# CuzImSlymi/Apertis-LLM

Hardware: NVIDIA B200
Metric: SSM+MoE block fwd+bwd tokens/sec (higher is better)
Workload: dtype bf16

## Files before the change

### apertis_llm_b200/_lib.py

```python
from __future__ import annotations

import ctypes
import os
import subprocess
import threading
from ctypes import c_char_p, c_float, c_int, c_int64, c_size_t, c_uint32, c_void_p

import torch

_HERE = os.path.dirname(os.path.abspath(__file__))
LIB_PATH = os.path.join(_HERE, "libapertis_b200.so")
CSRC = os.path.join(_HERE, "csrc")

AB_F32, AB_BF16 = 0, 1
ACT = {"gelu": 0, "relu": 1, "silu": 2, "swish": 2}
EPI_NONE, EPI_BIAS, EPI_BIAS_ACT, EPI_DACT, EPI_ADD = 0, 1, 2, 3, 4
SCAN_SINGLE_PASS, SCAN_TWO_PASS, SCAN_PIPELINED, SCAN_ROUNDS = 0, 1, 2, 3
ROW_ALIGN = 256
ROUTER_EXACT, ROUTER_BF16, ROUTER_FP16 = 0, 1, 2

P, I, I64, SZ, F, U32 = c_void_p, c_int, c_int64, c_size_t, c_float, c_uint32

SIGNATURES = {
    "ab_version": (I, []),
    "ab_device_check": (I, [I]),
    "ab_last_error": (I, [c_char_p, SZ]),
    "ab_causal_conv1d_silu_fwd": (I, [P, I64, P, P, P, I, I, I, I, I, P]),
    "ab_causal_conv1d_silu_bwd_workspace_bytes": (SZ, [I, I, I]),
    "ab_causal_conv1d_silu_bwd": (I, [P, I64, P, P, P, P, I64, P, P, P, SZ, I, I, I, I, I, P]),
    "ab_selective_scan_plan": (I, [I, I, I, I, P, P, P, P, P]),
    "ab_selective_scan_fwd": (I, [P, P, P, P, I64, P, I64, P, P, P, P, P, P, P, P, SZ, U32, I, I, I, I, I, I, P]),
    "ab_selective_scan_bwd": (I, [P, P, P, P, I64, P, I64, P, P, P, P, P, P, P, P, I64, P, P, P, P, P, SZ, U32, I,
                                  I, I, I, I, I, P]),
    "ab_ssm_scan_plan": (I, [I, I, I, I, P, P]),
    "ab_ssm_scan_tune": (I, [I, I, I, I, I]),
    "ab_ssm_scan_fwd": (I, [P, I64, P, I64, P, P, P, I64, P, I64, P, P, P, P, P, P, P, P, SZ, I, I, I, I, I, P]),
    "ab_ssm_scan_bwd": (I, [P, I64, P, P, I64, P, I64, P, P, P, P, P, P, I64, P, P, I64, P, I64, P, I64, I, P, P, P, P, SZ,
                            I, I, I, I, I, P]),
    "ab_gemm_row_tile": (I, []),
    "ab_shifted_ce_fwd": (I, [P, P, P, P, P, P, I, I, I, I64, I, P]),
    "ab_shifted_ce_bwd": (I, [P, P, P, P, P, I, I, I, I64, I, P]),
    "ab_ep_permute_ln": (I, [P, P, P, P, P, P, P, P, I, I, I64, I, I, I64, I, I, P]),
    "ab_ep_unpermute_bwd": (I, [P, P, P, P, P, P, P, I, I, I64, P, F, P, I, I, I64, I, I, I, P]),
    "ab_ep_grouped_gemm_nt": (I, [P, P, P, P, P, I, I, I64, P, P, I64, I, I, I, I, I, I, P]),
    "ab_ep_grouped_gemm_nn": (I, [P, P, P, P, P, I, I, I64, P, P, I64, I, I, I, I, I, I, P]),
    "ab_moe_router_workspace_bytes": (SZ, [I, I, I]),
    "ab_moe_router_fwd": (I, [P, P, P, F, P, P, P, P, P, P, P, P, P, P, P, P, P, P, SZ, I, I, I, I, I, I, P]),
    "ab_moe_topk_from_logits": (I, [P, P, P, P, P, P, I, I, I, P]),
    "ab_moe_max_rows": (I64, [I, I, I, I, I]),
    "ab_moe_plan_workspace_bytes": (SZ, [I, I, I]),
    "ab_moe_plan": (I, [P, P, P, I, P, P, P, P, P, P, P, P, SZ, I, I, I, I, I64, I, P]),
    "ab_moe_permute_ln": (I, [P, P, P, P, P, P, P, P, I, I, I64, I, I, P]),
    "ab_moe_unpermute": (I, [P, P, P, P, P, F, P, I, I, I, I, I, P]),
    "ab_moe_unpermute_bwd": (I, [P, P, P, P, P, P, P, P, F, P, I, I, I64, I, I, I, P]),
    "ab_moe_permute_ln_bwd_workspace_bytes": (SZ, [I, I, I64]),
    "ab_moe_permute_ln_bwd": (I, [P, P, P, P, P, P, P, P, P, P, P, SZ, I, I, I, I64, I, I, P]),
    "ab_moe_segment_colsum_workspace_bytes": (SZ, [I, I, I64]),
    "ab_moe_segment_colsum": (I, [P, P, P, P, P, SZ, I, I, I, I64, I, P]),
    "ab_moe_router_bwd_workspace_bytes": (SZ, [I, I, I]),
    "ab_moe_router_bwd": (I, [P] * 24 + [SZ, I, I, I, I, I, P]),
    "ab_grouped_gemm_nt": (I, [P, P, P, P, P, P, P, P, I64, I, I, I, I, I, I, F, P, P]),
    "ab_grouped_gemm_nn": (I, [P, P, P, P, P, P, P, P, I64, I, I, I, I, I, I, F, P, P]),
    "ab_grouped_gemm_tn_workspace_bytes": (SZ, [I, I, I, I]),
    "ab_grouped_gemm_tn": (I, [P, P, P, P, I64, I, I, I, I, I64, P, SZ, P]),
    "ab_dense_gemm_nt": (I, [P, P, P, P, P, I64, I, I, I, I, P]),
    "ab_dense_gemm_nn": (I, [P, P, P, P, P, I64, I, I, I, I, P]),
    "ab_dense_gemm_tn_workspace_bytes": (SZ, [I64, I, I]),
    "ab_dense_gemm_tn": (I, [P, P, P, P, SZ, I64, I, I, P]),
    "ab_dt_compose_fwd": (I, [P, P, P, I, I, I, I, I, P]),
    "ab_dt_compose_bwd": (I, [P, P, P, P, P, I, I, I, I, P]),
    "ab_layernorm_fwd": (I, [P, P, P, F, P, P, I, I, I, I, P]),
    "ab_layernorm_bwd_workspace_bytes": (SZ, [I, I]),
    "ab_layernorm_bwd": (I, [P, P, P, P, P, P, P, P, P, SZ, I, I, I, I, P]),
    "ab_dropout_add": (I, [P, P, P, F, P, I64, I, I, P]),
    "ab_cast_f32_to_bf16": (I, [P, P, I64, P]),
    "ab_split_f32_to_bf16x3": (I, [P, P, I64, I64, I, P]),
    "ab_split_f32_to_bf16x3_rows": (I, [P, P, P, I, I64, I64, I, P]),
}

_lib = None
_lock = threading.Lock()
_checked_devices = set()


def build(verbose: bool = False) -> str:
    cmd = ["make", "-C", CSRC, "-j", "8"]
    res = subprocess.run(cmd, capture_output=True, text=True)
    if res.returncode != 0:
        raise RuntimeError("building libapertis_b200.so failed:\n" + res.stdout[-4000:] + res.stderr[-4000:])
    if verbose:
        print(res.stdout[-2000:])
    return LIB_PATH


def load() -> ctypes.CDLL:
    global _lib
    with _lock:
        if _lib is not None:
            return _lib
        if not os.path.exists(LIB_PATH):
            build()
        lib = ctypes.CDLL(LIB_PATH)
        for name, (res, args) in SIGNATURES.items():
            fn = getattr(lib, name)
            fn.restype = res
            fn.argtypes = args
        _lib = lib
        return lib


def last_error() -> str:
    buf = ctypes.create_string_buffer(600)
    load().ab_last_error(buf, 600)
    return buf.value.decode("utf-8", "replace")


def ptr(t):
    if t is None:
        return None
    return t.data_ptr()


def dt(t_or_dtype) -> int:
    d = t_or_dtype.dtype if torch.is_tensor(t_or_dtype) else t_or_dtype
    if d == torch.float32:
        return AB_F32
    if d == torch.bfloat16:
        return AB_BF16
    raise TypeError(f"apertis_b200 kernels take float32 or bfloat16 activations, got {d}")


def stream_ptr(device=None) -> int:
    return torch.cuda.current_stream(device).cuda_stream


def ensure_device(device) -> None:
    if device.type != "cuda":
        raise RuntimeError("apertis_llm_b200: the hot path only runs on a CUDA sm_100a (B200) device; got "
                           f"device '{device}'. There is no CPU fallback.")
    idx = device.index if device.index is not None else torch.cuda.current_device()
    if idx in _checked_devices:
        return
    rc = load().ab_device_check(idx)
    if rc != 0:
        raise RuntimeError("apertis_llm_b200: " + last_error())
    _checked_devices.add(idx)


KERNELS_PER_CALL = {
    "ab_causal_conv1d_silu_fwd": 1, "ab_causal_conv1d_silu_bwd": 2,
    "ab_selective_scan_fwd": 1, "ab_selective_scan_bwd": 2,
    "ab_ssm_scan_fwd": 1, "ab_ssm_scan_bwd": 2, "ab_dense_gemm_nt": 1, "ab_dense_gemm_nn": 1, "ab_dense_gemm_tn": 2,
    "ab_dt_compose_fwd": 1, "ab_dt_compose_bwd": 2,
    "ab_moe_router_fwd": 2, "ab_moe_topk_from_logits": 1, "ab_moe_plan": 7, "ab_moe_permute_ln": 1, "ab_moe_unpermute": 1,
    "ab_moe_unpermute_bwd": 1, "ab_moe_permute_ln_bwd": 2, "ab_moe_segment_colsum": 2, "ab_moe_router_bwd": 3,
    "ab_layernorm_fwd": 1, "ab_layernorm_bwd": 3,
    "ab_grouped_gemm_nt": 1, "ab_grouped_gemm_nn": 1, "ab_grouped_gemm_tn": 1, "ab_cast_f32_to_bf16": 1,
    "ab_shifted_ce_fwd": 2, "ab_shifted_ce_bwd": 1, "ab_ep_permute_ln": 1, "ab_ep_unpermute_bwd": 1, "ab_ep_grouped_gemm_nt": 1, "ab_ep_grouped_gemm_nn": 1,
    "ab_split_f32_to_bf16x3": 1, "ab_split_f32_to_bf16x3_rows": 1,
}
launch_count = 0
_timed = None


def start_timing(names):
    global _timed
    _timed = {"names": set(names), "events": []}


def stop_timing():
    global _timed
    t, _timed = _timed, None
    out = {}
    if t is None:
        return out
    torch.cuda.synchronize()
    for name, a, b in t["events"]:
        out.setdefault(name, []).append(a.elapsed_time(b))
    return out


def call(name: str, *args):
    global launch_count
    fn = getattr(load(), name)
    if _timed is not None and name in _timed["names"]:
        a, b = torch.cuda.Event(enable_timing=True), torch.cuda.Event(enable_timing=True)
        a.record()
        rc = fn(*args)
        b.record()
        _timed["events"].append((name, a, b))
    else:
        rc = fn(*args)
    if rc != 0:
        raise RuntimeError(f"{name} failed (code {rc}): {last_error()}")
    launch_count += KERNELS_PER_CALL.get(name, 1)


def query(name: str, *args):
    return getattr(load(), name)(*args)
```

### apertis_llm_b200/csrc/grouped_gemm.cu

```cuda
#include "common.cuh"

namespace {

constexpr int BM = 128;
constexpr int PM = 2 * BM;
constexpr int BK = 64, NSTAGE = 5, NACC = 2;
constexpr int A_BYTES = BM * BK * 2;
constexpr int BH_BYTES_MAX = 128 * BK * 2;
constexpr int STAGE_BYTES = A_BYTES + BH_BYTES_MAX;
constexpr int ATOM_BYTES = 64 * BK * 2;
constexpr int EPI_WARP0 = 2, EPI_WARPS = 16, EPI_THREADS = EPI_WARPS * 32;
constexpr int NUM_THREADS = 64 + EPI_THREADS;
constexpr int GW = 64;
constexpr int MODE_NT = 0, MODE_NN = 1, MODE_TN = 2;
constexpr int WARP_STG_BYTES = 32 * 64;
constexpr int WARP_BIAS_BYTES = GW * 4;
constexpr size_t SMEM_BYTES = 1024 + (size_t)NSTAGE * STAGE_BYTES + (size_t)EPI_WARPS * (WARP_STG_BYTES + WARP_BIAS_BYTES) + 256;
static_assert(SMEM_BYTES <= 232448, "shared memory budget");
static_assert(PM == AB_GEMM_ROW_TILE, "row tile of the ABI");

struct GemmParams {
    int N, K, E, M;
    int bn;
    int num_n_tiles, num_m_tiles;
    int epi, act, c_f32;
    int tn_nsrc;
    int tn_e_real;
    int64_t tn_src_stride;
    int64_t rows_valid;
    int dense_m_tiles;
    int64_t tn_rows;
    int64_t tn_split;
    const int32_t* tile_expert;
    const int32_t* n_rows;
    const int32_t* seg_off;
    const float* bias;
    const void* aux;
    const uint32_t* drop_seed;
    uint32_t drop_thresh;
    float drop_scale;
    void* c;
    void* c2;
    float* cw;
    unsigned char* peer_base[16];
    int peer_n, peer_rows, peer_rank;
};

__device__ __forceinline__ int dense_tn_blocks(const GemmParams& p, int e) {
    const int64_t lo = (int64_t)e * p.tn_split;
    const int64_t hi = lo + p.tn_split < p.tn_rows ? lo + p.tn_split : p.tn_rows;
    return hi > lo ? (int)((hi - lo + BK - 1) / BK) : 0;
}

__device__ __forceinline__ float erf_core(float ax_s, float g) {
    const float t = ab_rcp(fmaf(0.3275911f, ax_s, 1.0f));
    float p = fmaf(1.061405429f, t, -1.453152027f);
    p = fmaf(p, t, 1.421413741f);
    p = fmaf(p, t, -0.284496736f);
    p = fmaf(p, t, 0.254829592f);
    return 1.0f - p * t * g;
}
__device__ __forceinline__ float gelu_fwd(float x) {
    const float a = fabsf(x) * 0.70710678118654752f;
    const float g = ab_ex2(x * (x * (-0.5f * AB_LOG2E)));
    const float t = ab_rcp(fmaf(0.3275911f, a, 1.0f));
    float q = fmaf(0.750526976f, t, -1.027533652f);
    q = fmaf(q, t, 1.005091295f);
    q = fmaf(q, t, -0.201169571f);
    q = fmaf(q, t, 0.180191733f);
    return fmaxf(x, 0.f) - (a * t) * (q * g);
}
__device__ __forceinline__ float act_fwd(float x, int act) {
    if (act == AB_ACT_GELU) return gelu_fwd(x);
    if (act == AB_ACT_RELU) return fmaxf(x, 0.f);
    return x * ab_sigmoid(x);
}
__device__ __forceinline__ float act_bwd(float x, int act) {
    if (act == AB_ACT_GELU) {
        const float a = fabsf(x) * 0.70710678118654752f;
        const float g = ab_ex2(-a * a * AB_LOG2E);
        const float cdf = 0.5f * (1.0f + copysignf(erf_core(a, g), x));
        return fmaf(x, 0.3989422804014327f * g, cdf);
    }
    if (act == AB_ACT_RELU) return x > 0.f ? 1.f : 0.f;
    const float s = ab_sigmoid(x);
    return s * fmaf(x, 1.f - s, 1.f);
}

__device__ __forceinline__ f2 gelu_fwd2(f2 x) {
    float x0, x1;
    f2_unpack(x, x0, x1);
    const f2 a = f2_pack(fabsf(x0) * 0.70710678118654752f, fabsf(x1) * 0.70710678118654752f);
    const f2 g = f2_ex2(f2_mul(x, f2_mul(x, f2_bcast(-0.5f * AB_LOG2E))));
    const f2 t = f2_rcp(f2_fma(f2_bcast(0.3275911f), a, f2_bcast(1.0f)));
    f2 q = f2_fma(f2_bcast(0.750526976f), t, f2_bcast(-1.027533652f));
    q = f2_fma(q, t, f2_bcast(1.005091295f));
    q = f2_fma(q, t, f2_bcast(-0.201169571f));
    q = f2_fma(q, t, f2_bcast(0.180191733f));
    const f2 h = f2_mul(f2_mul(a, t), f2_mul(q, g));
    return f2_fma(h, f2_bcast(-1.0f), f2_pack(fmaxf(x0, 0.f), fmaxf(x1, 0.f)));
}
__device__ __forceinline__ f2 gelu_bwd2(f2 x) {
    float x0, x1;
    f2_unpack(x, x0, x1);
    const f2 a = f2_pack(fabsf(x0) * 0.70710678118654752f, fabsf(x1) * 0.70710678118654752f);
    const f2 g = f2_ex2(f2_mul(f2_mul(a, a), f2_bcast(-AB_LOG2E)));
    const f2 t = f2_rcp(f2_fma(f2_bcast(0.3275911f), a, f2_bcast(1.0f)));
    f2 pl = f2_fma(f2_bcast(1.061405429f), t, f2_bcast(-1.453152027f));
    pl = f2_fma(pl, t, f2_bcast(1.421413741f));
    pl = f2_fma(pl, t, f2_bcast(-0.284496736f));
    pl = f2_fma(pl, t, f2_bcast(0.254829592f));
    const f2 erfv = f2_fma(f2_mul(pl, t), f2_mul(g, f2_bcast(-1.0f)), f2_bcast(1.0f));
    float e0, e1;
    f2_unpack(erfv, e0, e1);
    const f2 cdf = f2_fma(f2_pack(copysignf(e0, x0), copysignf(e1, x1)), f2_bcast(0.5f), f2_bcast(0.5f));
    return f2_fma(x, f2_mul(g, f2_bcast(0.3989422804014327f)), cdf);
}

#define AB_GF_C0 0.79746994f
#define AB_GF_C1 0.037015004f
#define AB_GF_C2 -3.5035629e-4f
__device__ __forceinline__ float ab_tanh(float x) { float y; asm("tanh.approx.f32 %0, %1;" : "=f"(y) : "f"(x)); return y; }
__device__ __forceinline__ f2 f2_tanh(f2 v) { float a, b; f2_unpack(v, a, b); return f2_pack(ab_tanh(a), ab_tanh(b)); }
__device__ __forceinline__ f2 gelu_fast_x2(f2 x) {
    float a, b;
    f2_unpack(f2_mul(x, x), a, b);
    return f2_pack(fminf(a, 81.f), fminf(b, 81.f));
}
__device__ __forceinline__ f2 gelu_fwd_fast2(f2 x, f2 hs) {
    const f2 x2 = gelu_fast_x2(x);
    f2 p = f2_fma(f2_bcast(AB_GF_C2), x2, f2_bcast(AB_GF_C1));
    p = f2_fma(p, x2, f2_bcast(AB_GF_C0));
    const f2 t = f2_tanh(f2_mul(p, x));
    const f2 hx = f2_mul(x, hs);
    return f2_fma(hx, t, hx);
}
__device__ __forceinline__ f2 gelu_bwd_fast2(f2 x, f2 hs) {
    const f2 x2 = gelu_fast_x2(x);
    f2 p = f2_fma(f2_bcast(AB_GF_C2), x2, f2_bcast(AB_GF_C1));
    p = f2_fma(p, x2, f2_bcast(AB_GF_C0));
    const f2 t = f2_tanh(f2_mul(p, x));
    f2 up = f2_fma(f2_bcast(5.f * AB_GF_C2), x2, f2_bcast(3.f * AB_GF_C1));
    up = f2_fma(up, x2, f2_bcast(AB_GF_C0));
    const f2 w = f2_mul(x, up);
    const f2 e = f2_fma(f2_mul(t, f2_bcast(-1.0f)), w, w);
    const f2 A = f2_fma(t, hs, hs);
    return f2_fma(A, e, A);
}

template <int U, bool F32>
__device__ __forceinline__ void act_fwd_row(float (&f)[U], int act, float scale) {
    if (act == AB_ACT_GELU && !F32) {
        const f2 hs = f2_bcast(0.5f * scale);
#pragma unroll
        for (int i = 0; i < U; i += 2) f2_unpack(gelu_fwd_fast2(f2_pack(f[i], f[i + 1]), hs), f[i], f[i + 1]);
    } else if (act == AB_ACT_GELU) {
        const f2 sc = f2_bcast(scale);
#pragma unroll
        for (int i = 0; i < U; i += 2) f2_unpack(f2_mul(gelu_fwd2(f2_pack(f[i], f[i + 1])), sc), f[i], f[i + 1]);
    } else if (act == AB_ACT_RELU) {
#pragma unroll
        for (int i = 0; i < U; ++i) f[i] = fmaxf(f[i], 0.f) * scale;
    } else {
#pragma unroll
        for (int i = 0; i < U; ++i) f[i] = act_fwd(f[i], AB_ACT_SILU) * scale;
    }
}
template <int U>
__device__ __forceinline__ void round_row_bf16(float (&f)[U]) {
#pragma unroll
    for (int i = 0; i < U; i += 2) {
        uint32_t r;
        asm("cvt.rn.bf16x2.f32 %0, %1, %2;" : "=r"(r) : "f"(f[i + 1]), "f"(f[i]));
        f[i] = __uint_as_float(r << 16);
        f[i + 1] = __uint_as_float(r & 0xffff0000u);
    }
}

__device__ __forceinline__ void drop_keep4(uint32_t xb, uint32_t grp, uint32_t s1, uint32_t thi, bool (&keep)[4]) {
    uint32_t x = xb + grp * 0x9E3779B1u;
    x ^= x >> 16; x *= 0x85EBCA6Bu;
    x = x ^ (x >> 13) ^ s1; x *= 0xC2B2AE35u;
    uint32_t y = x * 0x27D4EB2Fu + s1;
    y ^= y >> 15;
    keep[0] = (x << 16) >= thi;
    keep[1] = x >= thi;
    keep[2] = (y << 16) >= thi;
    keep[3] = y >= thi;
}
template <int U>
__device__ __forceinline__ void dropout_zero_row(float (&f)[U], uint32_t drop_thresh, uint32_t s0, uint32_t s1, uint32_t grow, int ncol, int n_cols) {
    const uint32_t xb = ((grow * (uint32_t)n_cols + (uint32_t)ncol) >> 2) * 0x9E3779B1u + s0;
    const uint32_t thi = drop_thresh << 16;
#pragma unroll
    for (int i = 0; i < U; i += 4) {
        bool keep[4];
        drop_keep4(xb, (uint32_t)(i >> 2), s1, thi, keep);
#pragma unroll
        for (int j = 0; j < 4; ++j) f[i + j] = keep[j] ? f[i + j] : 0.f;
    }
}

__device__ __forceinline__ uint64_t make_smem_desc(uint32_t smem_addr, uint32_t lbo_bytes, uint32_t sbo_bytes) {
    uint64_t d = 0;
    d |= (uint64_t)((smem_addr >> 4) & 0x3FFF);
    d |= (uint64_t)((lbo_bytes >> 4) & 0x3FFF) << 16;
    d |= (uint64_t)((sbo_bytes >> 4) & 0x3FFF) << 32;
    d |= (uint64_t)1 << 46;
    d |= (uint64_t)2 << 61;
    return d;
}
__host__ __device__ inline uint32_t make_idesc(int n, int a_mn_major, int b_mn_major) {
    uint32_t d = 0;
    d |= 1u << 4;
    d |= 1u << 7;
    d |= 1u << 10;
    d |= (uint32_t)a_mn_major << 15;
    d |= (uint32_t)b_mn_major << 16;
    d |= (uint32_t)(n >> 3) << 17;
    d |= (uint32_t)(PM >> 4) << 24;
    return d;
}

struct Tile { int m_pair, n_tile, e, k_begin, nk; };

template <int MODE>
__device__ __forceinline__ int total_tiles_of(const GemmParams& p) {
    if (MODE == MODE_TN) return p.E * p.num_m_tiles * p.num_n_tiles;
    return (p.n_rows != nullptr ? p.n_rows[0] / PM : p.dense_m_tiles) * p.num_n_tiles;
}
template <int MODE>
__device__ __forceinline__ Tile decode_tile(const GemmParams& p, int tile) {
    Tile t;
    if (MODE == MODE_TN) {
        const int per_e = p.num_m_tiles * p.num_n_tiles;
        t.e = tile / per_e;
        const int rem = tile % per_e;
        t.m_pair = rem / p.num_n_tiles; t.n_tile = rem % p.num_n_tiles;
        if (p.seg_off != nullptr) {
            const int e = p.tn_e_real > 0 ? t.e % p.tn_e_real : t.e, slice = p.tn_e_real > 0 ? t.e / p.tn_e_real : 0;
            const int s0 = p.seg_off[e];
            t.k_begin = s0 + (int)((int64_t)slice * p.tn_nsrc * p.tn_src_stride);
            t.nk = p.tn_nsrc * ((p.seg_off[e + 1] - s0) / BK);
        } else {
            t.k_begin = (int)(t.e * p.tn_split);
            t.nk = dense_tn_blocks(p, t.e);
        }
    } else {
        t.m_pair = tile / p.num_n_tiles; t.n_tile = tile % p.num_n_tiles;
        t.e = p.tile_expert != nullptr ? p.tile_expert[t.m_pair] : 0;
        t.k_begin = 0;
        t.nk = (p.K + BK - 1) / BK;
    }
    return t;
}

__device__ __forceinline__ uint32_t stg_off(int r, int j) { return (uint32_t)(r * 64 + ((j ^ ((r >> 1) & 3)) << 4)); }

template <int MODE, bool F32>
__device__ __forceinline__ void stage_and_store(const GemmParams& p, unsigned char* stg, const float (&src)[F32 ? 16 : 32],
                                                unsigned char* base, int lane, size_t row0, int ncol, int ncol_end) {
    constexpr int ES = F32 ? 4 : 2;
    constexpr int CPV = 16 / ES;
    const int N = p.N;
#pragma unroll
    for (int j = 0; j < 4; ++j) {
        uint4 q;
        if (F32) q = make_uint4(__float_as_uint(src[j * 4]), __float_as_uint(src[j * 4 + 1]), __float_as_uint(src[j * 4 + 2]), __float_as_uint(src[j * 4 + 3]));
        else q = ab_vec16<__nv_bfloat16>::pack(&src[j * 8]);
        *reinterpret_cast<uint4*>(stg + stg_off(lane, j)) = q;
    }
    __syncwarp();
#pragma unroll
    for (int it = 0; it < 4; ++it) {
        const int r = it * 8 + (lane >> 2), j = lane & 3;
        const int col = ncol + j * CPV;
        const size_t grow = row0 + r;
        const bool ok = col < ncol_end && (MODE == MODE_TN ? (int)grow < p.M : (int64_t)grow < p.rows_valid);
        const uint4 q = *reinterpret_cast<const uint4*>(stg + stg_off(r, j));
        if (ok) *reinterpret_cast<uint4*>(base + (grow * N + col) * ES) = q;
    }
    __syncwarp();
}

template <bool F32>
__device__ __forceinline__ void load_aux_unit(const GemmParams& p, uint4 (&q)[4], int lane, size_t row0, int ncol, int ncol_end) {
    constexpr int ES = F32 ? 4 : 2;
    constexpr int CPV = 16 / ES;
#pragma unroll
    for (int it = 0; it < 4; ++it) {
        const int r = it * 8 + (lane >> 2), j = lane & 3;
        const int col = ncol + j * CPV;
        const size_t grow = row0 + r;
        q[it] = make_uint4(0u, 0u, 0u, 0u);
        if (col < ncol_end && (int64_t)grow < p.rows_valid)
            q[it] = __ldg(reinterpret_cast<const uint4*>(reinterpret_cast<const unsigned char*>(p.aux) + (grow * p.N + col) * ES));
    }
}

struct EpiCtx {
    unsigned char* stg;
    float* bias_s;
    uint64_t* tfull;
    uint64_t* tempty;
    uint32_t tmem_base;
    int warp, lane;
    uint32_t rank;
    int pair_id, num_pairs;
};

template <int MODE, bool F32, int EPI>
__device__ __forceinline__ void epilogue_role(const GemmParams& p, const EpiCtx& c) {
    constexpr int U = F32 ? 16 : 32;
    constexpr int ES = F32 ? 4 : 2;
    constexpr int CPV = 16 / ES;
    constexpr bool HAS_BIAS = EPI == AB_EPI_BIAS || EPI == AB_EPI_BIAS_ACT;
    constexpr bool HAS_AUX = EPI == AB_EPI_DACT || EPI == AB_EPI_ADD;
    const int lane = c.lane;
    const int quarter = c.warp & 3;
    const int sub = (c.warp - EPI_WARP0) >> 2;
    const int N = p.N, bn = p.bn;
    const int g_col0 = sub * GW;
    const int g_cols = g_col0 < bn ? min(GW, bn - g_col0) : 0;
    const int total_tiles = total_tiles_of<MODE>(p);
    unsigned char* stg = c.stg;
    const bool has_drop = (EPI == AB_EPI_BIAS_ACT || EPI == AB_EPI_DACT) && p.drop_seed != nullptr;
    const uint32_t drop_s0 = has_drop ? __ldg(p.drop_seed) : 0u, drop_s1 = has_drop ? __ldg(p.drop_seed + 1) : 0u;
    const float dscale = has_drop ? p.drop_scale : 1.0f;
    int acc = 0; uint32_t acc_phase = 0;
    for (int tile = c.pair_id; tile < total_tiles; tile += c.num_pairs) {
        const Tile t = decode_tile<MODE>(p, tile);
        const int m_tile = 2 * t.m_pair + (int)c.rank;
        const bool have_acc = t.nk > 0;
        const int n0 = t.n_tile * bn;
        const int ncol_end = min(N, n0 + g_col0 + g_cols);
        const size_t row0 = (size_t)m_tile * BM + quarter * 32;
        if (HAS_BIAS && g_cols > 0) {
            const int col = n0 + g_col0 + 2 * lane;
            float2 b2 = make_float2(0.f, 0.f);
            if (col < ncol_end) b2 = __ldg(reinterpret_cast<const float2*>(p.bias + (size_t)t.e * N + col));
            *reinterpret_cast<float2*>(c.bias_s + 2 * lane) = b2;
            __syncwarp();
        }
        uint4 nxt[4];
        if (HAS_AUX && g_cols > 0 && n0 + g_col0 < ncol_end) {
            load_aux_unit<F32>(p, nxt, lane, row0, n0 + g_col0, ncol_end);
        }
        if (have_acc) {
            ab_mbar_wait(&c.tfull[acc], acc_phase);
            ab_tc_fence_after();
        }
        const uint32_t t_row = c.tmem_base + (uint32_t)acc * 256u + ((uint32_t)(quarter * 32) << 16);
        for (int u0 = 0; u0 < g_cols; u0 += U) {
            const int tcol = g_col0 + u0;
            const int ncol = n0 + tcol;
            if (ncol >= ncol_end) break;
            uint4 cur[4];
            if (HAS_AUX) {
#pragma unroll
                for (int it = 0; it < 4; ++it) cur[it] = nxt[it];
                if (u0 + U < g_cols && ncol + U < ncol_end) {
                    load_aux_unit<F32>(p, nxt, lane, row0, ncol + U, ncol_end);
                }
            }
            float f[U];
            {
                uint32_t v[U];
                if (have_acc) {
                    if (U == 32) ab_tmem_ld32(t_row + (uint32_t)tcol, v);
                    else ab_tmem_ld16(t_row + (uint32_t)tcol, v);
                    ab_tmem_ld_wait();
                } else {
#pragma unroll
                    for (int i = 0; i < U; ++i) v[i] = 0u;
                }
#pragma unroll
                for (int i = 0; i < U; ++i) f[i] = __uint_as_float(v[i]);
            }
            if (HAS_BIAS) {
#pragma unroll
                for (int i = 0; i < U; i += 4) {
                    const float4 b4 = *reinterpret_cast<const float4*>(c.bias_s + u0 + i);
                    f[i] += b4.x; f[i + 1] += b4.y; f[i + 2] += b4.z; f[i + 3] += b4.w;
                }
            }
            if (EPI == AB_EPI_BIAS_ACT) {
                if (!F32) round_row_bf16<U>(f);
                stage_and_store<MODE, F32>(p, stg, f, reinterpret_cast<unsigned char*>(p.c2), lane, row0, ncol, ncol_end);
                act_fwd_row<U, F32>(f, p.act, p.drop_seed ? p.drop_scale : 1.0f);
                if (p.drop_seed) dropout_zero_row<U>(f, p.drop_thresh, drop_s0, drop_s1, (uint32_t)row0 + (uint32_t)lane, ncol, N);
            } else if (HAS_AUX) {
#pragma unroll
                for (int it = 0; it < 4; ++it) *reinterpret_cast<uint4*>(stg + stg_off(it * 8 + (lane >> 2), lane & 3)) = cur[it];
                __syncwarp();
#pragma unroll
                for (int j = 0; j < 4; ++j) cur[j] = *reinterpret_cast<const uint4*>(stg + stg_off(lane, j));
                __syncwarp();
#pragma unroll
                for (int j = 0; j < 4; ++j) {
                    const uint4 q = cur[j];
                    float a[CPV];
                    if (F32) { a[0] = __uint_as_float(q.x); a[1] = __uint_as_float(q.y); a[2] = __uint_as_float(q.z); a[3] = __uint_as_float(q.w); }
                    else ab_vec16<__nv_bfloat16>::unpack(q, a);
                    if (EPI == AB_EPI_ADD) {
#pragma unroll
                        for (int i = 0; i < CPV; ++i) f[j * CPV + i] += a[i];
                    } else if (p.act == AB_ACT_GELU) {
#pragma unroll
                        for (int i = 0; i < CPV; i += 2) {
                            const f2 gp = F32 ? f2_mul(gelu_bwd2(f2_pack(a[i], a[i + 1])), f2_bcast(dscale))
                                              : gelu_bwd_fast2(f2_pack(a[i], a[i + 1]), f2_bcast(0.5f * dscale));
                            f2_unpack(f2_mul(f2_pack(f[j * CPV + i], f[j * CPV + i + 1]), gp), f[j * CPV + i], f[j * CPV + i + 1]);
                        }
                    } else {
#pragma unroll
                        for (int i = 0; i < CPV; ++i) f[j * CPV + i] *= act_bwd(a[i], p.act) * dscale;
                    }
                }
                if (EPI == AB_EPI_DACT && p.drop_seed) dropout_zero_row<U>(f, p.drop_thresh, drop_s0, drop_s1, (uint32_t)row0 + (uint32_t)lane, ncol, N);
            }
            unsigned char* base;
            if (MODE == MODE_TN) base = reinterpret_cast<unsigned char*>(p.cw) + ((size_t)t.e * p.M) * N * 4;
            else if (p.peer_n > 0) {
                const int dst = (int)(row0 / (size_t)p.peer_rows);
                base = p.peer_base[dst] + ((int64_t)(p.peer_rank - dst) * p.peer_rows) * (int64_t)N * ES;
            } else base = reinterpret_cast<unsigned char*>(p.c);
            stage_and_store<MODE, F32>(p, stg, f, base, lane, row0, ncol, ncol_end);
        }
        if (have_acc) {
            ab_tc_fence_before();
            __syncwarp();
            if (lane == 0) ab_mbar_arrive_cluster(&c.tempty[acc], 0);
            if (++acc == NACC) { acc = 0; acc_phase ^= 1; }
        }
    }
}

template <int MODE, bool F32>
__device__ __forceinline__ void epilogue_dispatch(const GemmParams& p, const EpiCtx& c) {
    if (MODE == MODE_TN) { epilogue_role<MODE, F32, AB_EPI_NONE>(p, c); return; }
    switch (p.epi) {
        case AB_EPI_BIAS: epilogue_role<MODE, F32, AB_EPI_BIAS>(p, c); break;
        case AB_EPI_BIAS_ACT: epilogue_role<MODE, F32, AB_EPI_BIAS_ACT>(p, c); break;
        case AB_EPI_DACT: epilogue_role<MODE, F32, AB_EPI_DACT>(p, c); break;
        case AB_EPI_ADD: epilogue_role<MODE, F32, AB_EPI_ADD>(p, c); break;
        default: epilogue_role<MODE, F32, AB_EPI_NONE>(p, c); break;
    }
}

template <int MODE>
__global__ void __launch_bounds__(NUM_THREADS, 1) grouped_gemm_kernel(const __grid_constant__ CUtensorMap tm_a,
                                                                      const __grid_constant__ CUtensorMap tm_b,
                                                                      const GemmParams p) {
    extern __shared__ unsigned char smem_raw[];
    const uint32_t raw = ab_smem_u32(smem_raw);
    unsigned char* smem = smem_raw + ((1024u - (raw & 1023u)) & 1023u);
    unsigned char* stg_base = smem + (size_t)NSTAGE * STAGE_BYTES;
    float* bias_base = reinterpret_cast<float*>(stg_base + (size_t)EPI_WARPS * WARP_STG_BYTES);
    uint64_t* bars = reinterpret_cast<uint64_t*>(reinterpret_cast<unsigned char*>(bias_base) + (size_t)EPI_WARPS * WARP_BIAS_BYTES);
    uint64_t* full = bars;
    uint64_t* empty = bars + NSTAGE;
    uint64_t* tfull = bars + 2 * NSTAGE;
    uint64_t* tempty = bars + 2 * NSTAGE + NACC;
    uint32_t* tmem_slot = reinterpret_cast<uint32_t*>(bars + 2 * NSTAGE + 2 * NACC);

    const int warp = threadIdx.x >> 5, lane = threadIdx.x & 31;
    const uint32_t rank = ab_cluster_ctarank();
    const int pair_id = blockIdx.x >> 1, num_pairs = gridDim.x >> 1;
    if (warp == 0 && lane == 0) {
        ab_prefetch_tmap(&tm_a);
        ab_prefetch_tmap(&tm_b);
        for (int i = 0; i < NSTAGE; ++i) { ab_mbar_init(&full[i], 1); ab_mbar_init(&empty[i], 1); }
        for (int i = 0; i < NACC; ++i) { ab_mbar_init(&tfull[i], 1); ab_mbar_init(&tempty[i], 2 * EPI_WARPS); }
        ab_fence_mbar_init();
    }
    if (warp == 1) {
        ab_tmem_alloc_pair(tmem_slot, 512);
        ab_tmem_relinquish_pair();
    }
    ab_tc_fence_before();
    ab_cluster_sync();
    ab_tc_fence_after();
    const uint32_t tmem_base = *tmem_slot;

    const int total_tiles = total_tiles_of<MODE>(p);
    const int bn = p.bn, bh = bn >> 1;
    const uint32_t bh_bytes = MODE == MODE_NT ? (uint32_t)bh * BK * 2 : (uint32_t)(bh / 64) * ATOM_BYTES;
    const uint32_t pair_tx = 2u * (A_BYTES + bh_bytes);

    if (warp == 0) {
        int stage = 0; uint32_t phase = 0;
        for (int tile = pair_id; tile < total_tiles; tile += num_pairs) {
            const Tile t = decode_tile<MODE>(p, tile);
            const int b_col0 = t.n_tile * bn + (int)rank * bh;
            const int n_src = MODE == MODE_TN ? p.tn_nsrc : 1;
            const int per_src = t.nk / n_src;
            const int m0 = MODE == MODE_TN ? t.m_pair * PM + (int)rank * BM : (2 * t.m_pair + (int)rank) * BM;
            const int b_row0 = MODE == MODE_NN ? t.e * p.K : (MODE == MODE_NT ? t.e * p.N + b_col0 : 0);
            for (int src = 0; src < n_src; ++src) {
                int r0 = MODE == MODE_TN ? (int)(src * p.tn_src_stride) + t.k_begin : 0;
                for (int kk = 0; kk < per_src; ++kk, r0 += BK) {
                    ab_mbar_wait(&empty[stage], phase ^ 1);
                    unsigned char* sa = smem + (size_t)stage * STAGE_BYTES;
                    unsigned char* sb = sa + A_BYTES;
                    if (ab_elect_one()) {
                        if (rank == 0) ab_mbar_expect_tx(&full[stage], pair_tx);
                        if (MODE == MODE_TN) {
                            ab_tma_load_2d_pair(sa, &tm_a, &full[stage], m0, r0);
                            ab_tma_load_2d_pair(sa + ATOM_BYTES, &tm_a, &full[stage], m0 + 64, r0);
                            ab_tma_load_2d_pair(sb, &tm_b, &full[stage], b_col0, r0);
                            if (bh > 64) ab_tma_load_2d_pair(sb + ATOM_BYTES, &tm_b, &full[stage], b_col0 + 64, r0);
                        } else {
                            ab_tma_load_2d_pair(sa, &tm_a, &full[stage], r0, m0);
                            if (MODE == MODE_NT) {
                                ab_tma_load_2d_pair(sb, &tm_b, &full[stage], r0, b_row0);
                            } else {
                                ab_tma_load_2d_pair(sb, &tm_b, &full[stage], b_col0, b_row0 + r0);
                                if (bh > 64) ab_tma_load_2d_pair(sb + ATOM_BYTES, &tm_b, &full[stage], b_col0 + 64, b_row0 + r0);
                            }
                        }
                    }
                    __syncwarp();
                    if (++stage == NSTAGE) { stage = 0; phase ^= 1; }
                }
            }
        }
        for (int i = 0; i < NSTAGE; ++i) {
            ab_mbar_wait(&empty[stage], phase ^ 1);
            if (++stage == NSTAGE) { stage = 0; phase ^= 1; }
        }
    } else if (warp == 1) {
        if (rank == 0) {
            const uint32_t idesc = make_idesc(bn, MODE == MODE_TN ? 1 : 0, MODE == MODE_NT ? 0 : 1);
            const uint32_t smem0 = ab_smem_u32(smem);
            const uint64_t da0 = MODE == MODE_TN ? make_smem_desc(smem0, ATOM_BYTES, 1024) : make_smem_desc(smem0, 0, 1024);
            const uint64_t db0 = MODE == MODE_NT ? make_smem_desc(smem0 + A_BYTES, 0, 1024) : make_smem_desc(smem0 + A_BYTES, ATOM_BYTES, 1024);
            constexpr uint32_t a_step = MODE == MODE_TN ? (16 * 128) >> 4 : 32 >> 4;
            constexpr uint32_t b_step = MODE == MODE_NT ? 32 >> 4 : (16 * 128) >> 4;
            int stage = 0; uint32_t phase = 0;
            int acc = 0; uint32_t acc_phase = 0;
            for (int tile = pair_id; tile < total_tiles; tile += num_pairs) {
                const Tile t = decode_tile<MODE>(p, tile);
                if (t.nk == 0) continue;
                ab_mbar_wait(&tempty[acc], acc_phase ^ 1);
                ab_tc_fence_after();
                const uint32_t d_tmem = tmem_base + (uint32_t)acc * 256u;
                for (int kb = 0; kb < t.nk; ++kb) {
                    ab_mbar_wait(&full[stage], phase);
                    ab_tc_fence_after();
                    const uint64_t soff = (uint64_t)((uint32_t)stage * (STAGE_BYTES >> 4));
                    const uint64_t da = da0 + soff, db = db0 + soff;
                    if (ab_elect_one()) {
#pragma unroll
                        for (int k = 0; k < BK / 16; ++k)
                            ab_umma_f16_pair(d_tmem, da + (uint64_t)(k * a_step), db + (uint64_t)(k * b_step), idesc, (kb > 0 || k > 0) ? 1u : 0u);
                        ab_umma_commit_pair(&empty[stage], 3);
                        if (kb == t.nk - 1) ab_umma_commit_pair(&tfull[acc], 3);
                    }
                    __syncwarp();
                    if (++stage == NSTAGE) { stage = 0; phase ^= 1; }
                }
                if (++acc == NACC) { acc = 0; acc_phase ^= 1; }
            }
        }
    } else {
        EpiCtx c;
        c.stg = stg_base + (size_t)(warp - EPI_WARP0) * WARP_STG_BYTES;
        c.bias_s = bias_base + (size_t)(warp - EPI_WARP0) * GW;
        c.tfull = tfull; c.tempty = tempty; c.tmem_base = tmem_base;
        c.warp = warp; c.lane = lane; c.rank = rank; c.pair_id = pair_id; c.num_pairs = num_pairs;
        if (p.c_f32) epilogue_dispatch<MODE, true>(p, c);
        else epilogue_dispatch<MODE, false>(p, c);
    }
    ab_tc_fence_before();
    ab_cluster_sync();
    if (warp == 1) ab_tmem_dealloc_pair(tmem_base, 512);
}

int pick_bn(int N, bool mn_major_b) {
    const int step = mn_major_b ? 128 : 16;
    int best = step, best_cost = 1 << 30;
    for (int bn = step; bn <= 256; bn += step) {
        const int cost = (int)ab_ceil_div(N, bn) * (bn + 48);
        if (cost <= best_cost) { best_cost = cost; best = bn; }
    }
    return best;
}

int make_map2(CUtensorMap* m, const void* base, uint64_t inner, uint64_t outer, uint32_t box_inner, uint32_t box_outer) {
    AB_REQUIRE(((uintptr_t)base % 16) == 0 && (inner * 2) % 16 == 0,
               "grouped_gemm: operand base must be 16-byte aligned and the contiguous dimension (%llu) a multiple of 8",
               (unsigned long long)inner);
    uint64_t dims[2] = {inner, outer};
    uint64_t strides[1] = {inner * 2};
    uint32_t box[2] = {box_inner, box_outer};
    return ab_encode_tmap(m, CU_TENSOR_MAP_DATA_TYPE_BFLOAT16, 2, base, dims, strides, box, CU_TENSOR_MAP_SWIZZLE_128B);
}

template <int MODE>
int resident_pairs(int* out) {
    static int cached[64] = {0};
    int dev = 0;
    AB_CHECK_CUDA(cudaGetDevice(&dev));
    if (dev >= 0 && dev < 64 && cached[dev] > 0) { *out = cached[dev]; return AB_OK; }
    auto k = grouped_gemm_kernel<MODE>;
    AB_CHECK_CUDA(cudaFuncSetAttribute(k, cudaFuncAttributeMaxDynamicSharedMemorySize, (int)SMEM_BYTES));
    cudaLaunchConfig_t cfg;
    memset(&cfg, 0, sizeof(cfg));
    cfg.gridDim = dim3(2 * (unsigned)(ab_num_sms() / 2), 1, 1);
    cfg.blockDim = dim3(NUM_THREADS, 1, 1);
    cfg.dynamicSmemBytes = SMEM_BYTES;
    cudaLaunchAttribute attr[1];
    attr[0].id = cudaLaunchAttributeClusterDimension;
    attr[0].val.clusterDim.x = 2; attr[0].val.clusterDim.y = 1; attr[0].val.clusterDim.z = 1;
    cfg.attrs = attr; cfg.numAttrs = 1;
    int n = 0;
    AB_CHECK_CUDA(cudaOccupancyMaxActiveClusters(&n, k, &cfg));
    if (n < 1) n = 1;
    if (n > ab_num_sms() / 2) n = ab_num_sms() / 2;
    if (dev >= 0 && dev < 64) cached[dev] = n;
    *out = n;
    return AB_OK;
}

template <int MODE>
int launch(const CUtensorMap& ta, const CUtensorMap& tb, const GemmParams& p, int64_t max_tiles, cudaStream_t stream) {
    int pairs = 0;
    if (int e = resident_pairs<MODE>(&pairs)) return e;
    if (max_tiles < pairs) pairs = (int)max_tiles;
    if (pairs < 1) pairs = 1;
    cudaLaunchConfig_t cfg;
    memset(&cfg, 0, sizeof(cfg));
    cfg.gridDim = dim3(2 * (unsigned)pairs, 1, 1);
    cfg.blockDim = dim3(NUM_THREADS, 1, 1);
    cfg.dynamicSmemBytes = SMEM_BYTES;
    cfg.stream = stream;
    cudaLaunchAttribute attr[1];
    attr[0].id = cudaLaunchAttributeClusterDimension;
    attr[0].val.clusterDim.x = 2; attr[0].val.clusterDim.y = 1; attr[0].val.clusterDim.z = 1;
    cfg.attrs = attr; cfg.numAttrs = 1;
    AB_CHECK_CUDA(cudaLaunchKernelEx(&cfg, grouped_gemm_kernel<MODE>, ta, tb, p));
    return AB_OK;
}

int gemm_rows(int mode, const void* A, const void* W, const float* bias, const void* aux, void* c, void* c2,
              const int32_t* tile_expert, const int32_t* n_rows, int64_t max_rows, int N, int K, int E, int epi, int act,
              int c_dtype, float drop_p, const uint32_t* drop_seed, cudaStream_t stream, const uint64_t* peer_c = nullptr,
              int peer_w = 0, int peer_rank = 0, int64_t peer_rows = 0) {
    AB_REQUIRE(drop_p >= 0.f && drop_p < 1.f, "grouped_gemm: dropout probability must be in [0, 1)");
    AB_REQUIRE(drop_p == 0.f || (drop_seed != nullptr && (epi == AB_EPI_BIAS_ACT || epi == AB_EPI_DACT)),
               "grouped_gemm: dropout needs a seed and the bias+act / dact epilogue");
    AB_REQUIRE(max_rows > 0 && max_rows % PM == 0, "grouped_gemm: max_rows must be a positive multiple of %d", PM);
    AB_REQUIRE(N > 0 && K > 0 && E > 0 && N % 8 == 0 && K % 8 == 0, "grouped_gemm: N (%d) and K (%d) must be multiples of 8", N, K);
    AB_REQUIRE(c_dtype == AB_F32 || c_dtype == AB_BF16, "grouped_gemm: bad output dtype");
    AB_REQUIRE(epi >= AB_EPI_NONE && epi <= AB_EPI_ADD, "grouped_gemm: bad epilogue %d", epi);
    AB_REQUIRE((epi != AB_EPI_BIAS && epi != AB_EPI_BIAS_ACT) || bias, "grouped_gemm: bias epilogue without bias");
    AB_REQUIRE(epi != AB_EPI_BIAS_ACT || c2, "grouped_gemm: bias+act epilogue needs the pre-activation output c2");
    AB_REQUIRE((epi != AB_EPI_DACT && epi != AB_EPI_ADD) || aux, "grouped_gemm: dact / add epilogue needs aux");
    AB_REQUIRE(bias == nullptr || ((uintptr_t)bias % 8) == 0, "grouped_gemm: bias must be 8-byte aligned");
    GemmParams p;
    memset(&p, 0, sizeof(p));
    p.N = N; p.K = K; p.E = E;
    p.bn = pick_bn(N, mode == MODE_NN);
    p.num_n_tiles = (int)ab_ceil_div(N, p.bn);
    p.epi = epi; p.act = act; p.c_f32 = c_dtype == AB_F32;
    p.tile_expert = tile_expert; p.n_rows = n_rows; p.bias = bias; p.aux = aux; p.c = c; p.c2 = c2;
    p.rows_valid = max_rows;
    if (peer_c != nullptr) {
        AB_REQUIRE(peer_w >= 1 && peer_w <= 16 && peer_rank >= 0 && peer_rank < peer_w && peer_rows > 0 && peer_rows % PM == 0 &&
                   (int64_t)peer_w * peer_rows == max_rows && epi != AB_EPI_BIAS_ACT,
                   "ep_grouped_gemm: bad peer table (W=%d rank=%d rows_per_peer=%lld, max_rows=%lld)", peer_w, peer_rank,
                   (long long)peer_rows, (long long)max_rows);
        for (int i = 0; i < peer_w; ++i) {
            AB_REQUIRE(peer_c[i] != 0 && peer_c[i] % 16 == 0, "ep_grouped_gemm: peer buffer %d is null or misaligned", i);
            p.peer_base[i] = reinterpret_cast<unsigned char*>(peer_c[i]);
        }
        p.peer_n = peer_w; p.peer_rows = (int)peer_rows; p.peer_rank = peer_rank;
        c = reinterpret_cast<void*>(peer_c[peer_rank]);
        p.c = c;
    }
    if (drop_p > 0.f) {
        p.drop_seed = drop_seed;
        p.drop_thresh = (uint32_t)((double)drop_p * 65536.0 + 0.5);
        p.drop_scale = 1.0f / (1.0f - drop_p);
    }
    AB_REQUIRE(((uintptr_t)c % 16) == 0 && (c2 == nullptr || ((uintptr_t)c2 % 16) == 0) && (aux == nullptr || ((uintptr_t)aux % 16) == 0),
               "grouped_gemm: output / aux pointers must be 16-byte aligned");
    CUtensorMap ta, tb;
    if (int e = make_map2(&ta, A, (uint64_t)K, (uint64_t)max_rows, BK, BM)) return e;
    const int64_t max_tiles = (max_rows / PM) * p.num_n_tiles;
    if (mode == MODE_NT) {
        if (int e = make_map2(&tb, W, (uint64_t)K, (uint64_t)E * N, BK, (uint32_t)(p.bn / 2))) return e;
        return launch<MODE_NT>(ta, tb, p, max_tiles, stream);
    }
    if (int e = make_map2(&tb, W, (uint64_t)N, (uint64_t)E * K, 64, BK)) return e;
    return launch<MODE_NN>(ta, tb, p, max_tiles, stream);
}

}

extern "C" int ab_gemm_row_tile(void) { return PM; }



extern "C" int ab_grouped_gemm_nt(const void* A, const void* W, const float* bias, const void* aux, void* c, void* c2,
                                  const int32_t* tile_expert, const int32_t* n_rows, int64_t max_rows, int N, int K, int E,
                                  int epi, int act, int c_dtype, float drop_p, const uint32_t* drop_seed, cudaStream_t stream) {
    return gemm_rows(MODE_NT, A, W, bias, aux, c, c2, tile_expert, n_rows, max_rows, N, K, E, epi, act, c_dtype, drop_p, drop_seed, stream);
}

extern "C" int ab_grouped_gemm_nn(const void* A, const void* W, const float* bias, const void* aux, void* c, void* c2,
                                  const int32_t* tile_expert, const int32_t* n_rows, int64_t max_rows, int N, int K, int E,
                                  int epi, int act, int c_dtype, float drop_p, const uint32_t* drop_seed, cudaStream_t stream) {
    return gemm_rows(MODE_NN, A, W, bias, aux, c, c2, tile_expert, n_rows, max_rows, N, K, E, epi, act, c_dtype, drop_p, drop_seed, stream);
}

extern "C" int ab_ep_grouped_gemm_nt(const void* A, const void* W, const float* bias, const void* aux, const uint64_t* peer_c, int peer_w,
                                     int rank, int64_t rows_per_peer, const int32_t* tile_expert, const int32_t* n_rows,
                                     int64_t max_rows, int N, int K, int E, int epi, int act, int c_dtype, cudaStream_t stream) {
    AB_REQUIRE(peer_c != nullptr, "ep_grouped_gemm_nt: no peer table");
    return gemm_rows(MODE_NT, A, W, bias, aux, nullptr, nullptr, tile_expert, n_rows, max_rows, N, K, E, epi, act, c_dtype, 0.f, nullptr,
                     stream, peer_c, peer_w, rank, rows_per_peer);
}

extern "C" int ab_ep_grouped_gemm_nn(const void* A, const void* W, const float* bias, const void* aux, const uint64_t* peer_c, int peer_w,
                                     int rank, int64_t rows_per_peer, const int32_t* tile_expert, const int32_t* n_rows,
                                     int64_t max_rows, int N, int K, int E, int epi, int act, int c_dtype, cudaStream_t stream) {
    AB_REQUIRE(peer_c != nullptr, "ep_grouped_gemm_nn: no peer table");
    return gemm_rows(MODE_NN, A, W, bias, aux, nullptr, nullptr, tile_expert, n_rows, max_rows, N, K, E, epi, act, c_dtype, 0.f, nullptr,
                     stream, peer_c, peer_w, rank, rows_per_peer);
}

namespace {
__global__ void splitk_reduce_kernel(const float* __restrict__ part, float* __restrict__ out, int64_t n, int nsplit);
int grouped_tn_slices(int M, int N, int E, int nsrc) {
    const int64_t tiles = (int64_t)E * ab_ceil_div(M, PM) * ab_ceil_div(N, pick_bn(N, true));
    const int pairs = ab_num_sms() / 2;
    int best = 1;
    double best_cost = (double)ab_ceil_div(tiles, pairs);
    for (int s = 2; s <= nsrc && s <= 4; ++s) {
        if (nsrc % s) continue;
        const double cost = (double)ab_ceil_div(tiles * s, pairs) / s;
        if (cost < 0.88 * best_cost) { best = s; best_cost = cost; }
    }
    return best;
}
}

extern "C" size_t ab_grouped_gemm_tn_workspace_bytes(int M, int N, int E, int nsrc) {
    const int slices = nsrc > 1 ? grouped_tn_slices(M, N, E, nsrc) : 1;
    return slices > 1 ? (size_t)slices * E * M * N * sizeof(float) : 0;
}

extern "C" int ab_grouped_gemm_tn(const void* A, const void* Bm, float* Cw, const int32_t* seg_off, int64_t max_rows, int M,
                                  int N, int E, int nsrc, int64_t src_stride, void* ws, size_t ws_bytes, cudaStream_t stream) {
    AB_REQUIRE(nsrc >= 1 && (nsrc == 1 || (src_stride > 0 && src_stride % BK == 0 && nsrc * src_stride <= max_rows)),
               "grouped_gemm_tn: bad source blocking nsrc=%d stride=%lld", nsrc, (long long)src_stride);
    AB_REQUIRE(max_rows > 0 && max_rows % BK == 0, "grouped_gemm_tn: max_rows must be a positive multiple of %d", BK);
    AB_REQUIRE(M > 0 && N > 0 && E > 0 && M % 8 == 0 && N % 8 == 0, "grouped_gemm_tn: M (%d) and N (%d) must be multiples of 8", M, N);
    GemmParams p;
    memset(&p, 0, sizeof(p));
    p.N = N; p.M = M; p.E = E; p.K = 0;
    p.bn = pick_bn(N, true);
    p.num_n_tiles = (int)ab_ceil_div(N, p.bn);
    p.num_m_tiles = (int)ab_ceil_div(M, PM);
    p.seg_off = seg_off; p.c_f32 = 1; p.epi = AB_EPI_NONE; p.cw = Cw;
    p.tn_nsrc = nsrc; p.tn_src_stride = src_stride;
    AB_REQUIRE(((uintptr_t)Cw % 16) == 0 && ((uintptr_t)ws % 16) == 0, "grouped_gemm_tn: output / workspace must be 16-byte aligned");
    int slices = nsrc > 1 ? grouped_tn_slices(M, N, E, nsrc) : 1;
    if (slices > 1 && (ws == nullptr || ws_bytes < (size_t)slices * E * M * N * sizeof(float))) slices = 1;
    if (slices > 1) {
        p.tn_e_real = E; p.E = E * slices; p.tn_nsrc = nsrc / slices;
        p.cw = reinterpret_cast<float*>(ws);
    }
    CUtensorMap ta, tb;
    if (int e = make_map2(&ta, A, (uint64_t)M, (uint64_t)max_rows, 64, BK)) return e;
    if (int e = make_map2(&tb, Bm, (uint64_t)N, (uint64_t)max_rows, 64, BK)) return e;
    if (int e = launch<MODE_TN>(ta, tb, p, (int64_t)p.E * p.num_m_tiles * p.num_n_tiles, stream)) return e;
    if (slices > 1) {
        const int64_t n = (int64_t)E * M * N;
        splitk_reduce_kernel<<<(unsigned)ab_ceil_div(n / 4, 256), 256, 0, stream>>>(reinterpret_cast<const float*>(ws), Cw, n, slices);
        AB_LAUNCH_CHECK();
    }
    return AB_OK;
}

namespace {
int dense_rows(int mode, const void* A, const void* W, const float* bias, const void* aux, void* c, int64_t S, int N, int K, int epi,
               int c_dtype, cudaStream_t stream) {
    AB_REQUIRE(S > 0 && N > 0 && K > 0 && N % 8 == 0 && K % 8 == 0, "dense_gemm: S (%lld) must be positive, N (%d) and K (%d) multiples of 8", (long long)S, N, K);
    AB_REQUIRE(c_dtype == AB_F32 || c_dtype == AB_BF16, "dense_gemm: bad output dtype");
    AB_REQUIRE(epi == AB_EPI_NONE || epi == AB_EPI_BIAS || epi == AB_EPI_ADD, "dense_gemm: epilogue must be none, bias or add");
    AB_REQUIRE(epi != AB_EPI_BIAS || bias, "dense_gemm: bias epilogue without bias");
    AB_REQUIRE(epi != AB_EPI_ADD || aux, "dense_gemm: add epilogue without addend");
    AB_REQUIRE(((uintptr_t)c % 16) == 0 && (aux == nullptr || ((uintptr_t)aux % 16) == 0), "dense_gemm: output / addend must be 16-byte aligned");
    AB_REQUIRE(bias == nullptr || ((uintptr_t)bias % 8) == 0, "dense_gemm: bias must be 8-byte aligned");
    GemmParams p;
    memset(&p, 0, sizeof(p));
    p.N = N; p.K = K; p.E = 1;
    p.bn = pick_bn(N, mode == MODE_NN);
    p.num_n_tiles = (int)ab_ceil_div(N, p.bn);
    p.epi = epi; p.c_f32 = c_dtype == AB_F32;
    p.bias = bias; p.aux = aux; p.c = c;
    p.rows_valid = S;
    p.dense_m_tiles = (int)ab_ceil_div(S, PM);
    CUtensorMap ta, tb;
    if (int e = make_map2(&ta, A, (uint64_t)K, (uint64_t)S, BK, BM)) return e;
    const int64_t tiles = (int64_t)p.dense_m_tiles * p.num_n_tiles;
    if (mode == MODE_NT) {
        if (int e = make_map2(&tb, W, (uint64_t)K, (uint64_t)N, BK, (uint32_t)(p.bn / 2))) return e;
        return launch<MODE_NT>(ta, tb, p, tiles, stream);
    }
    if (int e = make_map2(&tb, W, (uint64_t)N, (uint64_t)K, 64, BK)) return e;
    return launch<MODE_NN>(ta, tb, p, tiles, stream);
}
}

extern "C" int ab_dense_gemm_nt(const void* A, const void* W, const float* bias, const void* aux, void* C, int64_t S, int N, int K,
                                int epi, int c_dtype, cudaStream_t stream) {
    return dense_rows(MODE_NT, A, W, bias, aux, C, S, N, K, epi, c_dtype, stream);
}

extern "C" int ab_dense_gemm_nn(const void* A, const void* W, const float* bias, const void* aux, void* C, int64_t S, int N, int K,
                                int epi, int c_dtype, cudaStream_t stream) {
    return dense_rows(MODE_NN, A, W, bias, aux, C, S, N, K, epi, c_dtype, stream);
}

namespace {
__global__ void splitk_reduce_kernel(const float* __restrict__ part, float* __restrict__ out, int64_t n, int nsplit) {
    const int64_t i = ((int64_t)blockIdx.x * blockDim.x + threadIdx.x) * 4;
    if (i >= n) return;
    float4 acc = *reinterpret_cast<const float4*>(part + i);
    for (int s = 1; s < nsplit; ++s) {
        const float4 v = *reinterpret_cast<const float4*>(part + (size_t)s * n + i);
        acc.x += v.x; acc.y += v.y; acc.z += v.z; acc.w += v.w;
    }
    *reinterpret_cast<float4*>(out + i) = acc;
}

int dense_tn_nsplit(int64_t S, int M, int N) {
    const int tiles = (int)(ab_ceil_div(M, PM) * ab_ceil_div(N, pick_bn(N, true)));
    int nsplit = tiles > 0 ? (ab_num_sms() / 2) / tiles : 1;
    const int64_t kblocks = ab_ceil_div(S, BK);
    if (nsplit > kblocks / 4) nsplit = (int)(kblocks / 4);
    return nsplit < 2 ? 1 : nsplit;
}
}

extern "C" size_t ab_dense_gemm_tn_workspace_bytes(int64_t S, int M, int N) {
    const int nsplit = dense_tn_nsplit(S, M, N);
    return nsplit < 2 ? 0 : (size_t)nsplit * M * N * sizeof(float);
}

extern "C" int ab_dense_gemm_tn(const void* A, const void* Bm, float* Cw, void* ws, size_t ws_bytes, int64_t S, int M, int N,
                                cudaStream_t stream) {
    AB_REQUIRE(S > 0 && M > 0 && N > 0 && M % 8 == 0 && N % 8 == 0, "dense_gemm_tn: S (%lld) must be positive, M (%d) and N (%d) multiples of 8", (long long)S, M, N);
    AB_REQUIRE(((uintptr_t)Cw % 16) == 0 && ((uintptr_t)ws % 16) == 0, "dense_gemm_tn: output / workspace must be 16-byte aligned");
    GemmParams p;
    memset(&p, 0, sizeof(p));
    p.N = N; p.M = M; p.K = 0;
    p.bn = pick_bn(N, true);
    p.num_n_tiles = (int)ab_ceil_div(N, p.bn);
    p.num_m_tiles = (int)ab_ceil_div(M, PM);
    p.c_f32 = 1; p.epi = AB_EPI_NONE;
    p.tn_nsrc = 1; p.tn_rows = S;
    int nsplit = dense_tn_nsplit(S, M, N);
    if (nsplit >= 2 && (ws == nullptr || ws_bytes < (size_t)nsplit * M * N * sizeof(float))) nsplit = 1;
    const int64_t kblocks = ab_ceil_div(S, BK);
    p.E = nsplit;
    p.tn_split = ab_ceil_div(kblocks, nsplit) * BK;
    p.cw = nsplit > 1 ? reinterpret_cast<float*>(ws) : Cw;
    CUtensorMap ta, tb;
    if (int e = make_map2(&ta, A, (uint64_t)M, (uint64_t)S, 64, BK)) return e;
    if (int e = make_map2(&tb, Bm, (uint64_t)N, (uint64_t)S, 64, BK)) return e;
    if (int e = launch<MODE_TN>(ta, tb, p, (int64_t)nsplit * p.num_m_tiles * p.num_n_tiles, stream)) return e;
    if (nsplit > 1) {
        const int64_t n = (int64_t)M * N;
        splitk_reduce_kernel<<<(unsigned)ab_ceil_div(n / 4, 256), 256, 0, stream>>>(reinterpret_cast<const float*>(ws), Cw, n, nsplit);
        AB_LAUNCH_CHECK();
    }
    return AB_OK;
}
```

### apertis_llm_b200/ep.py

```python
from __future__ import annotations

import os
from typing import List

import ctypes

import torch
import torch.distributed as dist

from . import _lib, ops
from ._lib import ROW_ALIGN, call, dt, ptr, query, stream_ptr


def segment_rows(cap: int) -> int:
    return (int(cap) + ROW_ALIGN - 1) // ROW_ALIGN * ROW_ALIGN


def recv_tile_expert(W: int, El: int, seg: int, device=None) -> torch.Tensor:
    tiles_per_seg = seg // ROW_ALIGN
    return torch.arange(El, dtype=torch.int32, device=device).repeat_interleave(tiles_per_seg).repeat(W)


def local_seg_off(El: int, seg: int, device=None) -> torch.Tensor:
    return torch.arange(El + 1, dtype=torch.int32, device=device) * seg


def all_to_all_equal(send: torch.Tensor, group) -> torch.Tensor:
    W = dist.get_world_size(group)
    assert send.shape[0] == W and send.is_contiguous()
    recv = torch.empty_like(send)
    if dist.get_backend(group) == "nccl":
        dist.all_to_all_single(recv.view(-1), send.view(-1), group=group)
        return recv
    rank = dist.get_rank(group)
    recv[rank].copy_(send[rank])
    ops_ = []
    for peer in range(W):
        if peer == rank:
            continue
        ops_.append(dist.P2POp(dist.isend, send[peer], dist.get_global_rank(group, peer), group))
        ops_.append(dist.P2POp(dist.irecv, recv[peer], dist.get_global_rank(group, peer), group))
    for w in dist.batch_isend_irecv(ops_):
        w.wait()
    return recv


def all_to_all_equal_start(send: torch.Tensor, group):
    if dist.get_backend(group) != "nccl":
        return all_to_all_equal(send, group), (lambda: None)
    assert send.shape[0] == dist.get_world_size(group) and send.is_contiguous()
    recv = torch.empty_like(send)
    work = dist.all_to_all_single(recv.view(-1), send.view(-1), group=group, async_op=True)
    return recv, work.wait


def all_gather_cat(t: torch.Tensor, group) -> torch.Tensor:
    W = dist.get_world_size(group)
    out = torch.empty((W,) + tuple(t.shape), dtype=t.dtype, device=t.device)
    dist.all_gather_into_tensor(out.view(-1), t.contiguous().view(-1), group=group) if dist.get_backend(group) == "nccl" else \
        dist.all_gather(list(out.unbind(0)), t.contiguous(), group=group)
    return out.view((-1,) + tuple(t.shape[1:]))


_EP_MODE = os.environ.get("APERTIS_B200_EP", "auto")

_peer_cache = {}
_peer_failed = False
_warned_reuse = False


class _PeerState:

    def __init__(self, group, rows: int, Dm: int, device):
        import torch.distributed._symmetric_memory as symm_mem
        self.W = dist.get_world_size(group)
        self.rank = dist.get_rank(group)
        self.rows, self.Dm = rows, Dm
        names = ("xn", "y", "dy", "dxn")
        self.buf, self.hdl, self.ptrs = {}, {}, {}
        for n in names:
            t = symm_mem.empty(rows, Dm, dtype=torch.bfloat16, device=device)
            h = symm_mem.rendezvous(t, group)
            self.buf[n], self.hdl[n] = t, h
            self.ptrs[n] = (ctypes.c_uint64 * self.W)(*[int(p) for p in h.buffer_ptrs])
        self.sync = self.hdl["xn"]
        self.version = 0
        self.side = torch.cuda.Stream(device=device)

    def barrier(self, channel: int = 0):
        self.sync.barrier(channel=channel)


_uniform_checked = set()
_recv_plans = {}


def _recv_plan(W: int, El: int, seg: int, device):
    key = (W, El, seg, device.index)
    p = _recv_plans.get(key)
    if p is None:
        p = dict(tile_expert=recv_tile_expert(W, El, seg, device),
                 n_rows=torch.full((2,), W * El * seg, dtype=torch.int32, device=device),
                 seg_off=local_seg_off(El, seg, device))
        if not torch.cuda.is_current_stream_capturing():
            _recv_plans[key] = p
    return p


def _check_uniform(group, S: int, cap: int, training: bool, device):
    key = (id(group), S, cap, training)
    if key in _uniform_checked:
        return
    mine = torch.tensor([S, cap, int(training)], dtype=torch.int64, device=device)
    allv = [torch.empty_like(mine) for _ in range(dist.get_world_size(group))]
    dist.all_gather(allv, mine, group=group)
    vals = torch.stack(allv).cpu()
    if not bool((vals == vals[0]).all()):
        raise RuntimeError("apertis_b200 EP: every rank of the expert-parallel group must process the same number of tokens with the "
                           f"same capacity and mode; got (tokens, capacity, training) per rank = {vals.tolist()}")
    _uniform_checked.add(key)


def _peer_state(group, rows: int, Dm: int, device, owner=0):
    global _peer_failed
    if _EP_MODE == "nccl" or _peer_failed or dist.get_backend(group) != "nccl":
        return None
    key = (id(group), dist.get_rank(group), rows, Dm, device.index, owner)
    st = _peer_cache.get(key)
    if st is None:
        if torch.cuda.is_current_stream_capturing():
            return None
        try:
            st = _PeerState(group, rows, Dm, device)
        except Exception as ex:
            if _EP_MODE == "peer":
                raise
            _peer_failed = True
            import warnings
            warnings.warn(f"apertis_b200 EP: peer-memory transport unavailable ({type(ex).__name__}: {ex}); using NCCL all-to-all")
            return None
        _peer_cache[key] = st
    return st


class _MoEExpertsEP(torch.autograd.Function):

    @staticmethod
    @ops._on_tensor_device
    def forward(ctx, x2, rn_w, rn_b, Wr, br, noise, noise_scale, ln_w, ln_b, W1, b1, W2, b2, res, cfg, group):
        _lib.ensure_device(x2.device)
        dev = x2.device
        W = dist.get_world_size(group)
        S, Dm = x2.shape
        El, I, _ = W1.shape
        E = El * W
        K, act, training, precise = cfg["K"], cfg["act"], cfg["training"], cfg["precise"]
        x2 = x2.contiguous()
        f = lambda t: t.float().contiguous()
        rn_w, rn_b, Wr, br, b1, b2, W1, W2 = map(f, (rn_w, rn_b, Wr, br, b1, b2, W1, W2))
        ln_key = (ln_w._version, ln_b._version, ln_w.data_ptr(), ln_b.data_ptr(), E, Dm)
        ln_cache = cfg.get("_ln_cache")
        if ln_cache is not None and ln_cache.get("key") == ln_key:
            ln_w_full, ln_b_full = ln_cache["val"]
        else:
            ln_wb = all_gather_cat(torch.stack([f(ln_w), f(ln_b)]).unsqueeze(0), group)
            ln_w_full = ln_wb[:, 0].reshape(E, Dm).contiguous()
            ln_b_full = ln_wb[:, 1].reshape(E, Dm).contiguous()
            if ln_cache is not None:
                ln_cache["key"], ln_cache["val"] = ln_key, (ln_w_full, ln_b_full)
        use_noise = noise is not None and noise_scale is not None
        r = ops.moe_route(x2, rn_w, rn_b, cfg["eps"], Wr, br, f(noise) if use_noise else None,
                          f(noise_scale) if use_noise else None, K, cfg.get("quant", _lib.ROUTER_EXACT))
        _check_uniform(group, S, cfg["cap"], training, dev)
        if cfg["cap"] >= S:
            cnt = torch.bincount(r["idx"].reshape(-1).long(), minlength=E)[:E]
            if cfg["active"] is not None:
                cnt = cnt * cfg["active"].to(cnt.dtype)
            mx = cnt.max().reshape(1)
            dist.all_reduce(mx, op=dist.ReduceOp.MAX, group=group)
            seg = segment_rows(max(1, int(mx.item())))
        else:
            seg = segment_rows(min(cfg["cap"], S))
        plan = ops.moe_plan(r["idx"], r["w"], E, cfg["cap"], cfg["active"], fixed_seg=seg)
        rows_local = E * seg
        cdt = torch.float32 if precise else torch.bfloat16
        peer = None if precise else _peer_state(group, rows_local, Dm, dev, cfg.get("_owner", 0))
        rank = dist.get_rank(group)
        rplan = _recv_plan(W, El, seg, dev)
        if peer is not None:
            peer.version += 1
            peer.barrier(0)
            call("ab_ep_permute_ln", ptr(x2), ptr(r["stats"]), ptr(ln_w_full), ptr(ln_b_full), ptr(plan["tok_of_row"]),
                 ptr(plan["tile_expert"]), ptr(plan["n_rows"]), peer.ptrs["xn"], W, rank, El * seg, Dm, ROW_ALIGN, rows_local,
                 dt(x2), dt(cdt), stream_ptr())
            w1, w2 = ops._cast_bf16(W1), ops._cast_bf16(W2)
            peer.barrier(1)
            xr = peer.buf["xn"]
        else:
            xn = torch.empty(rows_local, Dm, dtype=cdt, device=dev)
            call("ab_moe_permute_ln", ptr(x2), ptr(r["stats"]), ptr(ln_w_full), ptr(ln_b_full), ptr(plan["tok_of_row"]),
                 ptr(plan["tile_expert"]), ptr(plan["n_rows"]), ptr(xn), Dm, ROW_ALIGN, rows_local, dt(x2), dt(cdt), stream_ptr())
            xr_w, xr_wait = all_to_all_equal_start(xn.view(W, El * seg, Dm), group)
            w1 = ops._split_cols(W1.view(El * I, Dm), 1) if precise else ops._cast_bf16(W1)
            w2 = ops._split_cols(W2.view(El * Dm, I), 1) if precise else ops._cast_bf16(W2)
            xr_wait()
            xr = xr_w.view(rows_local, Dm)
        if precise:
            a1, k1 = ops._split_cols(xr, 0), 3 * Dm
        else:
            a1, k1 = xr, Dm
        drop_p = float(cfg.get("drop_p", 0.0)) if training else 0.0
        drop_seed = torch.randint(0, 2 ** 31 - 1, (2,), device=dev, dtype=torch.int32) if drop_p > 0.0 else None
        h, hpre = ops.grouped_gemm("nt", a1, w1, rplan, I, k1, El, bias=b1, epi=_lib.EPI_BIAS_ACT, act=act, out_dtype=cdt, want_c2=True,
                                   drop_p=drop_p, drop_seed=drop_seed)
        if precise:
            a2, k2 = ops._split_cols(h, 0), 3 * I
        else:
            a2, k2 = h, I
        out_p = float(cfg.get("out_drop_p", 0.0)) if training else 0.0
        out_seed = torch.randint(0, 2 ** 31 - 1, (2,), device=dev, dtype=torch.int32) if out_p > 0.0 else None
        resc = res.reshape(S, Dm).float().contiguous() if res is not None else None
        out = torch.empty(S, Dm, dtype=x2.dtype if res is None else torch.float32, device=dev)
        if peer is not None:
            call("ab_ep_grouped_gemm_nt", ptr(a2), ptr(w2), ptr(b2), None, peer.ptrs["y"], W, rank, El * seg, ptr(rplan["tile_expert"]),
                 ptr(rplan["n_rows"]), rows_local, Dm, k2, El, _lib.EPI_BIAS, act, dt(cdt), stream_ptr())
            peer.barrier(2)
            y = peer.buf["y"]
            call("ab_moe_unpermute", ptr(y), ptr(plan["row_of"]), ptr(r["w"]), ptr(resc), ptr(out), out_p, ptr(out_seed), S, K, Dm, dt(y), dt(out),
                 stream_ptr())
        else:
            yr = ops.grouped_gemm("nt", a2, w2, rplan, Dm, k2, El, bias=b2, epi=_lib.EPI_BIAS, out_dtype=cdt)
            y = all_to_all_equal(yr.view(W, El * seg, Dm), group).view(rows_local, Dm)
            call("ab_moe_unpermute", ptr(y), ptr(plan["row_of"]), ptr(r["w"]), ptr(resc), ptr(out), out_p, ptr(out_seed), S, K, Dm, dt(y), dt(out),
                 stream_ptr())
        aux = r["aux"]
        zero = torch.zeros((), dtype=x2.dtype, device=dev)
        lb = (cfg["lb_coef"] * E / (S * S)) * (aux[:E] * aux[E:2 * E]).sum() if (training and cfg["lb_coef"] > 0) else zero
        rz = (cfg["rz_coef"] / S) * aux[2 * E] if (training and cfg["rz_coef"] > 0) else zero
        ctx.cfg = dict(cfg, S=S, Dm=Dm, E=E, El=El, I=I, W=W, seg=seg, use_noise=use_noise, rows=rows_local, cdt=cdt, drop_p=drop_p,
                       out_p=out_p, has_res=res is not None, res_shape=res.shape if res is not None else None,
                       res_dtype=res.dtype if res is not None else None)
        ctx.drop_seed = drop_seed
        ctx.out_seed = out_seed
        ctx.shadows = None if precise else (w1, w2)
        ctx.group = group
        ctx.peer = peer
        ctx.peer_version = peer.version if peer is not None else 0
        ctx.plan = {k: v for k, v in plan.items() if torch.is_tensor(v)}
        ctx.rplan = rplan
        ctx.save_for_backward(x2, rn_w, rn_b, Wr, br, ln_w_full, W1, W2, noise if use_noise else None, r["stats"], r["gates"],
                              r["idx"], r["probs"], r["lse"], r["lclean"], r["w"], aux, xr, h, hpre, y)
        counts = plan["counts"]
        ctx.mark_non_differentiable(counts)
        cfg["_routing"] = (r["idx"], plan["row_of"])
        return out, lb.to(x2.dtype), rz.to(x2.dtype), counts

    @staticmethod
    @ops._on_tensor_device
    def backward(ctx, dout, dlb, drz, _dcounts):
        (x2, rn_w, rn_b, Wr, br, ln_w_full, W1, W2, noise, stats, gates, idx, probs, lse, lclean, w, aux, xr, h, hpre, y) = ctx.saved_tensors
        cfg, plan, rplan, group = ctx.cfg, ctx.plan, ctx.rplan, ctx.group
        S, Dm, E, El, I, K, W, seg = (cfg[k] for k in ("S", "Dm", "E", "El", "I", "K", "W", "seg"))
        act, precise, rows, cdt = cfg["act"], cfg["precise"], cfg["rows"], cfg["cdt"]
        dev = x2.device
        f32 = dict(dtype=torch.float32, device=dev)
        dout = dout.contiguous()
        peer = ctx.peer
        rank = dist.get_rank(group)
        dw_row = torch.empty(rows, **f32)
        if peer is not None and ctx.peer_version != peer.version:
            msg = ("apertis_b200 EP (peer transport): a later forward of this layer ran before this backward.  Expected under "
                   "activation checkpointing (the recomputation rewrites identical rows); any other schedule that keeps two "
                   "forwards of one layer in flight needs APERTIS_B200_EP=nccl.")
            if os.environ.get("APERTIS_B200_EP_STRICT", "0") == "1":
                raise RuntimeError(msg)
            global _warned_reuse
            if not _warned_reuse:
                _warned_reuse = True
                import warnings
                warnings.warn(msg)
        if peer is not None:
            call("ab_ep_unpermute_bwd", ptr(dout), ptr(y), ptr(w), ptr(plan["tok_of_row"]), ptr(plan["slot_of_row"]), ptr(plan["n_rows"]),
                 peer.ptrs["dy"], W, rank, El * seg, ptr(dw_row), cfg["out_p"], ptr(ctx.out_seed), K, Dm, rows, dt(dout), dt(y), dt(cdt),
                 stream_ptr())
            peer.barrier(3)
            dyr = peer.buf["dy"]
        else:
            dy = torch.empty(rows, Dm, dtype=cdt, device=dev)
            call("ab_moe_unpermute_bwd", ptr(dout), ptr(y), ptr(w), ptr(plan["tok_of_row"]), ptr(plan["slot_of_row"]), ptr(plan["n_rows"]),
                 ptr(dy), ptr(dw_row), cfg["out_p"], ptr(ctx.out_seed), K, Dm, rows, dt(dout), dt(y), dt(cdt), stream_ptr())
            dyr = all_to_all_equal(dy.view(W, El * seg, Dm), group).view(rows, Dm)
        lseg = rplan["seg_off"]
        stride = El * seg
        cmain, cside = torch.cuda.current_stream(dev), ops._side_stream(dev)
        db2 = torch.empty(El, Dm, **f32)
        db1 = torch.empty(El, I, **f32)
        ws_b2 = ops._u8(query("ab_moe_segment_colsum_workspace_bytes", Dm, ROW_ALIGN, rows), dev)
        ws_b1 = ops._u8(query("ab_moe_segment_colsum_workspace_bytes", I, ROW_ALIGN, rows), dev)
        if precise:
            G = W * El
            lseg3 = (lseg * 3).contiguous()
            w2r = ops._split_rows(W2.view(El * Dm, I), 1, None, El, Dm)
            dhpre = ops.grouped_gemm("nn", ops._split_cols(dyr, 0), w2r, rplan, I, 3 * Dm, El, aux=hpre, epi=_lib.EPI_DACT, act=act, out_dtype=cdt,
                                     drop_p=cfg["drop_p"], drop_seed=ctx.drop_seed)
            sr = lambda t, which: ops._split_rows(t, which, None, G, seg)
            w1r = ops._split_rows(W1.view(El * I, Dm), 1, None, El, I)
            dxnr = ops.grouped_gemm("nn", ops._split_cols(dhpre, 0), w1r, rplan, Dm, 3 * I, El, out_dtype=torch.float32)
            dxn_w, dxn_wait = all_to_all_equal_start(dxnr.view(W, El * seg, Dm), group)
            dW2 = ops.grouped_gemm_tn(sr(dyr, 0), sr(h, 1), lseg3, Dm, I, El, nsrc=W, src_stride=3 * stride)
            dW1 = ops.grouped_gemm_tn(sr(dhpre, 0), sr(xr, 1), lseg3, I, Dm, El, nsrc=W, src_stride=3 * stride)
        else:
            w1b, w2b = ctx.shadows
            dhpre = ops.grouped_gemm("nn", dyr, w2b, rplan, I, Dm, El, aux=hpre, epi=_lib.EPI_DACT, act=act, out_dtype=cdt,
                                     drop_p=cfg["drop_p"], drop_seed=ctx.drop_seed)
            if peer is not None:
                call("ab_ep_grouped_gemm_nn", ptr(dhpre), ptr(w1b), None, None, peer.ptrs["dxn"], W, rank, El * seg, ptr(rplan["tile_expert"]),
                     ptr(rplan["n_rows"]), rows, Dm, I, El, _lib.EPI_NONE, act, dt(torch.bfloat16), stream_ptr())
                main = torch.cuda.current_stream(dev)
                peer.side.wait_stream(main)
                with torch.cuda.stream(peer.side):
                    peer.barrier(4)
                dxn_w = peer.buf["dxn"]
                dxn_wait = lambda: main.wait_stream(peer.side)
            else:
                dxnr = ops.grouped_gemm("nn", dhpre, w1b, rplan, Dm, I, El, out_dtype=torch.bfloat16)
                dxn_w, dxn_wait = all_to_all_equal_start(dxnr.view(W, El * seg, Dm), group)
            dW2 = ops.grouped_gemm_tn(dyr, h, lseg, Dm, I, El, nsrc=W, src_stride=stride)
            dW1 = ops.grouped_gemm_tn(dhpre, xr, lseg, I, Dm, El, nsrc=W, src_stride=stride)
        ops._colsum_side(cside, cmain, dyr, rplan, db2, ws_b2, Dm, El, rows, dev)
        ops._colsum_side(cside, cmain, dhpre, rplan, db1, ws_b1, I, El, rows, dev)
        ws = ops._u8(query("ab_moe_permute_ln_bwd_workspace_bytes", Dm, ROW_ALIGN, rows), dev)
        dxn_wait()
        dxn = dxn_w.view(rows, Dm)
        dxrow = torch.empty(rows, Dm, **f32)
        dln_w = torch.empty(E, Dm, **f32)
        dln_b = torch.empty(E, Dm, **f32)
        call("ab_moe_permute_ln_bwd", ptr(dxn), ptr(x2), ptr(stats), ptr(ln_w_full), ptr(plan["tok_of_row"]), ptr(plan["tile_expert"]),
             ptr(plan["n_rows"]), ptr(dxrow), ptr(dln_w), ptr(dln_b), ptr(ws), ws.numel(), Dm, E, ROW_ALIGN, rows, dt(x2), dt(dxn),
             stream_ptr())
        dln = torch.stack([dln_w, dln_b])
        dln_work = dist.all_reduce(dln, group=group, async_op=True)
        inv = 1.0 / W
        training = cfg["training"]
        g_lb = (dlb.float() * (cfg["lb_coef"] * E / S)) if (training and cfg["lb_coef"] > 0) else torch.zeros((), **f32)
        g_rz = (drz.float() * (cfg["rz_coef"] / S)) if (training and cfg["rz_coef"] > 0) else torch.zeros((), **f32)
        scal = torch.stack([g_lb.reshape(()), g_rz.reshape(())]).contiguous()
        fvec = (aux[E:2 * E] / S).contiguous()
        dx = torch.empty_like(x2)
        dWr, dbr = torch.empty(E, Dm, **f32), torch.empty(E, **f32)
        drn_w, drn_b = torch.empty(Dm, **f32), torch.empty(Dm, **f32)
        dns = torch.empty(E, **f32) if cfg["use_noise"] else None
        nws = query("ab_moe_router_bwd_workspace_bytes", S, Dm, E)
        ws2 = ops._u8(nws, dev)
        call("ab_moe_router_bwd", ptr(x2), ptr(stats), ptr(rn_w), ptr(rn_b), ptr(Wr), ptr(br), ptr(gates), ptr(idx), ptr(probs),
             ptr(lse), ptr(lclean), ptr(noise.float().contiguous()) if cfg["use_noise"] else None, ptr(fvec), ptr(scal), ptr(dw_row),
             ptr(dxrow), ptr(plan["row_of"]), ptr(dx), ptr(dWr), ptr(dbr), ptr(drn_w), ptr(drn_b), ptr(dns), ptr(ws2), ws2.numel(),
             S, Dm, E, K, dt(x2), stream_ptr())
        dln_work.wait()
        dln_w_l = dln[0, rank * El:(rank + 1) * El] * inv
        dln_b_l = dln[1, rank * El:(rank + 1) * El] * inv
        dres = dout.reshape(cfg["res_shape"]).to(cfg["res_dtype"]) if cfg["has_res"] else None
        cmain.wait_stream(cside)
        return (dx, drn_w, drn_b, dWr, dbr, None, dns, dln_w_l, dln_b_l, dW1 * inv, db1 * inv, dW2 * inv, db2 * inv, dres, None, None)


def moe_experts_ep(module, x2, noise, noise_scale, cfg, res=None):
    cfg["_owner"] = id(module)
    cfg["_ln_cache"] = module.__dict__.setdefault("_ep_ln_cache", {})
    return _MoEExpertsEP.apply(x2, module.router_norm.weight, module.router_norm.bias, module.router.weight, module.router.bias,
                               noise, noise_scale, module.expert_ln_weight, module.expert_ln_bias, module.expert_w1,
                               module.expert_b1, module.expert_w2, module.expert_b2, res, cfg, module.ep_group)


def replicated_parameters(layer: torch.nn.Module) -> List[torch.nn.Parameter]:
    return [p for n, p in layer.named_parameters() if ".expert_" not in n and not n.startswith("expert_")]
```

### apertis_llm_b200/ops.py

```python
from __future__ import annotations

import ctypes
import math
import os
from typing import Optional

import torch

from . import _lib
from ._lib import AB_BF16, AB_F32, ROW_ALIGN, call, dt, ptr, query, stream_ptr

def _on_tensor_device(fn):
    def wrapper(ctx, *args):
        dev = next((a.device for a in args if torch.is_tensor(a) and a.is_cuda), None)
        if dev is None:
            return fn(ctx, *args)
        with torch.cuda.device(dev):
            return fn(ctx, *args)
    wrapper.__name__, wrapper.__doc__ = fn.__name__, fn.__doc__
    return wrapper


_scan_ws = {}
_SCAN_ENV = os.environ.get("APERTIS_B200_SCAN", "auto")
SCAN_MODE = {"two_pass": _lib.SCAN_TWO_PASS, "single": _lib.SCAN_SINGLE_PASS, "pipelined": _lib.SCAN_PIPELINED,
             "rounds": _lib.SCAN_ROUNDS}.get(_SCAN_ENV)


def default_scan_mode(dtype: torch.dtype, Di: int, L: int = 1 << 20) -> int:
    if SCAN_MODE is not None:
        return SCAN_MODE
    return _lib.SCAN_ROUNDS


def _scan_workspace(device, nbytes: int, mode: int = _lib.SCAN_SINGLE_PASS):
    key = (device.index, torch.cuda.current_stream(device).cuda_stream, mode == _lib.SCAN_PIPELINED)
    ent = _scan_ws.get(key)
    if ent is None or ent[0].numel() < nbytes:
        epoch = ent[1] if ent is not None else 0
        ent = [torch.zeros(max(nbytes, 1 << 20), dtype=torch.uint8, device=device), epoch]
        _scan_ws[key] = ent
    ent[1] += 1
    if ent[1] >= (1 << 30) - 1:
        ent[0].zero_()
        ent[1] = 1
    return ent[0], ent[1]


_SCAN_CHECK = os.environ.get("APERTIS_B200_SCAN_CHECK", "0") == "1"


def _scan_check(ws: torch.Tensor, what: str):
    if _SCAN_CHECK and not torch.cuda.is_current_stream_capturing() and int(ws[64:68].view(torch.int32).item()) != 0:
        ws[64:68].zero_()
        raise RuntimeError(f"{what}: a hand-shake wait of the selective scan timed out (protocol error)")


def scan_plan(B: int, L: int, Di: int, dtype: torch.dtype, mode: int = _lib.SCAN_SINGLE_PASS):
    t, s, n, m = ctypes.c_int(), ctypes.c_int(), ctypes.c_int(), ctypes.c_int(mode)
    ws = ctypes.c_size_t()
    call("ab_selective_scan_plan", B, L, Di, dt(dtype), ctypes.byref(m), ctypes.byref(t), ctypes.byref(s), ctypes.byref(n), ctypes.byref(ws))
    return t.value, s.value, n.value, ws.value, m.value


def _row_stride(t: torch.Tensor) -> int:
    B, L, C = t.shape
    assert t.stride(2) == 1 and (B == 1 or t.stride(0) == L * t.stride(1)), "unsupported layout"
    return t.stride(1)


def _rows(t: torch.Tensor) -> torch.Tensor:
    B, L, C = t.shape
    if t.stride(2) == 1 and (B == 1 or t.stride(0) == L * t.stride(1)) and (L == 1 or t.stride(1) >= C):
        return t
    return t.contiguous()


class _LayerNorm(torch.autograd.Function):
    @staticmethod
    @_on_tensor_device
    def forward(ctx, x, weight, bias, eps, out_dtype):
        _lib.ensure_device(x.device)
        shape = x.shape
        Dm = shape[-1]
        x2 = x.reshape(-1, Dm).contiguous()
        S = x2.shape[0]
        w, b = weight.float().contiguous(), bias.float().contiguous()
        y = torch.empty(S, Dm, dtype=out_dtype, device=x.device)
        stats = torch.empty(S, 2, dtype=torch.float32, device=x.device)
        call("ab_layernorm_fwd", ptr(x2), ptr(w), ptr(b), float(eps), ptr(y), ptr(stats), S, Dm, dt(x2), dt(out_dtype), stream_ptr())
        ctx.save_for_backward(x2, stats, w)
        ctx.shape = shape
        return y.view(shape)

    @staticmethod
    @_on_tensor_device
    def backward(ctx, dy):
        x2, stats, w = ctx.saved_tensors
        S, Dm = x2.shape
        dy2 = dy.reshape(S, Dm).contiguous()
        dx = torch.empty_like(x2)
        dw = torch.empty(Dm, dtype=torch.float32, device=x2.device)
        db = torch.empty(Dm, dtype=torch.float32, device=x2.device)
        nws = query("ab_layernorm_bwd_workspace_bytes", S, Dm)
        ws = torch.empty(max(nws, 16), dtype=torch.uint8, device=x2.device)
        call("ab_layernorm_bwd", ptr(dy2), ptr(x2), ptr(stats), ptr(w), None, ptr(dx), ptr(dw), ptr(db), ptr(ws), ws.numel(), S, Dm,
             dt(x2), dt(dy2), stream_ptr())
        return dx.view(ctx.shape), dw, db, None, None


class _LayerNormSkip(torch.autograd.Function):

    @staticmethod
    @_on_tensor_device
    def forward(ctx, x, weight, bias, eps, out_dtype):
        _lib.ensure_device(x.device)
        shape = x.shape
        Dm = shape[-1]
        x2 = x.reshape(-1, Dm).contiguous()
        S = x2.shape[0]
        w, b = weight.float().contiguous(), bias.float().contiguous()
        y = torch.empty(S, Dm, dtype=out_dtype, device=x.device)
        stats = torch.empty(S, 2, dtype=torch.float32, device=x.device)
        call("ab_layernorm_fwd", ptr(x2), ptr(w), ptr(b), float(eps), ptr(y), ptr(stats), S, Dm, dt(x2), dt(out_dtype), stream_ptr())
        ctx.save_for_backward(x2, stats, w)
        ctx.shape = shape
        return y.view(shape), x.view_as(x)

    @staticmethod
    @_on_tensor_device
    def backward(ctx, dy, dskip):
        x2, stats, w = ctx.saved_tensors
        S, Dm = x2.shape
        if dy is None:
            return dskip, None, None, None, None
        dy2 = dy.reshape(S, Dm).contiguous()
        dres = dskip.reshape(S, Dm).to(x2.dtype).contiguous() if dskip is not None else None
        dx = torch.empty_like(x2)
        dw = torch.empty(Dm, dtype=torch.float32, device=x2.device)
        db = torch.empty(Dm, dtype=torch.float32, device=x2.device)
        nws = query("ab_layernorm_bwd_workspace_bytes", S, Dm)
        ws = torch.empty(max(nws, 16), dtype=torch.uint8, device=x2.device)
        call("ab_layernorm_bwd", ptr(dy2), ptr(x2), ptr(stats), ptr(w), ptr(dres), ptr(dx), ptr(dw), ptr(db), ptr(ws), ws.numel(), S, Dm,
             dt(x2), dt(dy2), stream_ptr())
        return dx.view(ctx.shape), dw, db, None, None


class _DropoutAdd(torch.autograd.Function):
    @staticmethod
    @_on_tensor_device
    def forward(ctx, sub, res, p):
        _lib.ensure_device(sub.device)
        sub = sub.contiguous()
        res = res.contiguous()
        out = torch.empty_like(res)
        seed = torch.randint(0, 2 ** 31 - 1, (2,), device=sub.device, dtype=torch.int32) if p > 0 else None
        call("ab_dropout_add", ptr(sub), ptr(res), ptr(out), float(p), ptr(seed), sub.numel(), dt(sub), dt(out), stream_ptr())
        ctx.p, ctx.seed, ctx.sub_dtype = p, seed, sub.dtype
        return out

    @staticmethod
    @_on_tensor_device
    def backward(ctx, dout):
        if ctx.p == 0:
            return dout.to(ctx.sub_dtype), dout, None
        dout = dout.contiguous()
        dsub = torch.empty(dout.shape, dtype=ctx.sub_dtype, device=dout.device)
        call("ab_dropout_add", ptr(dout), None, ptr(dsub), float(ctx.p), ptr(ctx.seed), dout.numel(), dt(dout), dt(dsub), stream_ptr())
        return dsub, dout, None


def dropout_add(sub, res, p: float, training: bool):
    return _DropoutAdd.apply(sub, res, float(p) if training else 0.0)


def layer_norm(x, weight, bias, eps, out_dtype=None):
    return _LayerNorm.apply(x, weight, bias, eps, out_dtype if out_dtype is not None else x.dtype)


def layer_norm_skip(x, weight, bias, eps, out_dtype=None):
    return _LayerNormSkip.apply(x, weight, bias, eps, out_dtype if out_dtype is not None else x.dtype)


class _CausalConv1dSiLU(torch.autograd.Function):
    @staticmethod
    @_on_tensor_device
    def forward(ctx, xp, weight, bias):
        _lib.ensure_device(xp.device)
        xp = _rows(xp)
        B, L, Di = xp.shape
        Kc = weight.shape[-1]
        w = weight.reshape(Di, Kc).float().contiguous()
        b = bias.float().contiguous()
        xa = torch.empty(B, L, Di, dtype=xp.dtype, device=xp.device)
        call("ab_causal_conv1d_silu_fwd", ptr(xp), _row_stride(xp), ptr(w), ptr(b), ptr(xa), B, L, Di, Kc, dt(xp), stream_ptr())
        ctx.save_for_backward(xp, w, b)
        ctx.wshape = weight.shape
        ctx.wdtype, ctx.bdtype = weight.dtype, bias.dtype
        return xa

    @staticmethod
    @_on_tensor_device
    def backward(ctx, dxa):
        xp, w, b = ctx.saved_tensors
        B, L, Di = xp.shape
        Kc = w.shape[-1]
        dxa = dxa.contiguous()
        dxp = torch.empty(B, L, Di, dtype=xp.dtype, device=xp.device)
        dw = torch.empty(Di, Kc, dtype=torch.float32, device=xp.device)
        db = torch.empty(Di, dtype=torch.float32, device=xp.device)
        nws = query("ab_causal_conv1d_silu_bwd_workspace_bytes", B, L, Di)
        ws = torch.empty(nws, dtype=torch.uint8, device=xp.device)
        call("ab_causal_conv1d_silu_bwd", ptr(xp), _row_stride(xp), ptr(dxa), ptr(w), ptr(b), ptr(dxp), Di, ptr(dw), ptr(db),
             ptr(ws), nws, B, L, Di, Kc, dt(xp), stream_ptr())
        return dxp, dw.reshape(ctx.wshape).to(ctx.wdtype), db.to(ctx.bdtype)


def causal_conv1d_silu(xp: torch.Tensor, weight: torch.Tensor, bias: torch.Tensor) -> torch.Tensor:
    return _CausalConv1dSiLU.apply(xp, weight, bias)


class _SelectiveScan(torch.autograd.Function):
    @staticmethod
    @_on_tensor_device
    def forward(ctx, xa, dlog, BC, z, A_log, D, h0, want_yssm, want_hlast, mode):
        _lib.ensure_device(xa.device)
        xa = xa.contiguous()
        dlog = dlog.contiguous()
        BC, z = BC.contiguous(), _rows(z)
        B, L, Di = xa.shape
        H = dlog.shape[-1]
        assert BC.shape == (B, L, 2 * Di)
        Bm, Cm = BC[..., :Di], BC[..., Di:]
        dev = xa.device
        A = A_log.reshape(-1).float().contiguous()
        Dv = D.float().contiguous()
        if want_yssm and mode == _lib.SCAN_PIPELINED:
            mode = _lib.SCAN_SINGLE_PASS
        T, Cs, nchunks, nws, mode = scan_plan(B, L, Di, xa.dtype, mode)
        if mode != _lib.SCAN_PIPELINED and torch.cuda.is_current_stream_capturing():
            mode = _lib.SCAN_TWO_PASS
        ws, epoch = _scan_workspace(dev, nws, mode)
        y = torch.empty_like(xa)
        y_ssm = torch.empty_like(xa) if want_yssm else None
        h_last = torch.empty(B, Di, dtype=torch.float32, device=dev) if want_hlast else None
        hstart = torch.empty(B, nchunks, Di, dtype=torch.float32, device=dev)
        h0c = h0.reshape(B, Di).float().contiguous() if h0 is not None else None
        call("ab_selective_scan_fwd", ptr(xa), ptr(dlog), ptr(Bm), ptr(Cm), 2 * Di, ptr(z), _row_stride(z), ptr(A),
             ptr(Dv), ptr(h0c), ptr(y), ptr(y_ssm), ptr(h_last), ptr(hstart), ptr(ws), ws.numel(), epoch, mode,
             B, L, Di, H, dt(xa), stream_ptr())
        _scan_check(ws, "ab_selective_scan_fwd")
        ctx.save_for_backward(xa, dlog, BC, z, A, Dv, hstart)
        ctx.mode = mode
        ctx.a_shape, ctx.want_yssm = A_log.shape, want_yssm
        if h_last is not None:
            ctx.mark_non_differentiable(h_last)
        return y, y_ssm, h_last

    @staticmethod
    @_on_tensor_device
    def backward(ctx, dy, dyssm, _dh):
        xa, dlog, BC, z, A, Dv, hstart = ctx.saved_tensors
        B, L, Di = xa.shape
        H = dlog.shape[-1]
        dev = xa.device
        Bm, Cm = BC[..., :Di], BC[..., Di:]
        dy = dy.contiguous()
        dys = dyssm.contiguous() if (dyssm is not None and ctx.want_yssm) else None
        T, Cs, nchunks, nws, _ = scan_plan(B, L, Di, xa.dtype, ctx.mode)
        ws, epoch = _scan_workspace(dev, nws, ctx.mode)
        dxa = torch.empty_like(xa)
        dz = torch.empty_like(xa)
        dbc = torch.empty(B, L, 2 * Di, dtype=xa.dtype, device=dev)
        parts = H if ctx.mode == _lib.SCAN_PIPELINED else Di // 4
        ddl = torch.empty(B, L, parts, dtype=torch.float32, device=dev)
        dA = torch.empty(Di, dtype=torch.float32, device=dev)
        dD = torch.empty(Di, dtype=torch.float32, device=dev)
        dB, dC = dbc[..., :Di], dbc[..., Di:]
        call("ab_selective_scan_bwd", ptr(xa), ptr(dlog), ptr(Bm), ptr(Cm), 2 * Di, ptr(z), _row_stride(z), ptr(dy),
             ptr(dys), ptr(A), ptr(Dv), ptr(hstart), ptr(dxa), ptr(dB), ptr(dC), 2 * Di, ptr(dz), ptr(ddl), ptr(dA), ptr(dD),
             ptr(ws), ws.numel(), epoch, ctx.mode, B, L, Di, H, dt(xa), stream_ptr())
        _scan_check(ws, "ab_selective_scan_bwd")
        ddlog = (ddl if parts == H else ddl.view(B, L, H, parts // H).sum(-1)).to(dlog.dtype)
        return dxa, ddlog, dbc, dz, dA.reshape(ctx.a_shape), dD, None, None, None, None


def selective_scan(xa, dlog, BC, z, A_log, D, h0=None, want_yssm=False, want_hlast=False, mode: Optional[int] = None):
    mode = default_scan_mode(xa.dtype, xa.shape[-1], xa.shape[1]) if mode is None else mode
    if mode == _lib.SCAN_ROUNDS:
        return _SelectiveScanRounds.apply(xa, dlog, None, BC, z, A_log, D, h0, want_yssm, want_hlast, dlog.shape[-1])
    return _SelectiveScan.apply(xa, dlog, BC, z, A_log, D, h0, want_yssm, want_hlast, mode)


_rounds_ws = {}


def _rounds_plan(B, L, Di, dtype):
    n, ws = ctypes.c_int64(), ctypes.c_size_t()
    call("ab_ssm_scan_plan", B, L, Di, dt(dtype), ctypes.byref(n), ctypes.byref(ws))
    return n.value, ws.value


def _rounds_workspace(device, nbytes):
    key = (device.index, torch.cuda.current_stream(device).cuda_stream)
    t = _rounds_ws.get(key)
    if t is None or t.numel() < nbytes:
        t = torch.zeros(max(nbytes, 2 << 20), dtype=torch.uint8, device=device)
        _rounds_ws[key] = t
    return t


def _cols(t, lo, hi):
    return t[..., lo:hi]


class _SelectiveScanRounds(torch.autograd.Function):

    @staticmethod
    def forward(ctx, xa, dlog, dt_bias, prm, z, A_log, D, h0, want_yssm, want_hlast, H):
        _lib.ensure_device(xa.device)
        with torch.cuda.device(xa.device):
            xa, z, prm = _rows(xa), _rows(z), _rows(prm)
            B, L, Di = xa.shape
            dev = xa.device
            fused = dlog is None
            W = prm.shape[-1]
            Hp = W - 2 * Di
            assert Hp >= (H if fused else 0) and (fused or Hp == 0), "bad [dt | B | C] layout"
            dl = prm if fused else dlog.contiguous()
            dl_stride = _row_stride(prm) if fused else H
            Bm, Cm = _cols(prm, Hp, Hp + Di), _cols(prm, Hp + Di, Hp + 2 * Di)
            A = A_log.reshape(-1).float().contiguous()
            Dv = D.float().contiguous()
            bias = dt_bias.float().contiguous() if dt_bias is not None else None
            nstate, nws = _rounds_plan(B, L, Di, xa.dtype)
            ws = _rounds_workspace(dev, nws)
            y = torch.empty(B, L, Di, dtype=xa.dtype, device=dev)
            y_ssm = torch.empty(B, L, Di, dtype=xa.dtype, device=dev) if want_yssm else None
            h_last = torch.empty(B, Di, dtype=torch.float32, device=dev) if want_hlast else None
            state = torch.empty(nstate, dtype=torch.float32, device=dev)
            h0c = h0.reshape(B, Di).float().contiguous() if h0 is not None else None
            call("ab_ssm_scan_fwd", ptr(xa), _row_stride(xa), ptr(dl), dl_stride, ptr(bias), ptr(Bm), ptr(Cm), _row_stride(prm),
                 ptr(z), _row_stride(z), ptr(A), ptr(Dv), ptr(h0c), ptr(y), ptr(y_ssm), ptr(h_last), ptr(state), ptr(ws), ws.numel(),
                 B, L, Di, H, dt(xa), stream_ptr(dev))
            ctx.save_for_backward(xa, prm, z, A, Dv, state)
            ctx.meta = (fused, H, Hp, want_yssm, A_log.shape, dlog.dtype if dlog is not None else None,
                        dt_bias is not None, dt_bias.dtype if dt_bias is not None else None)
            if h_last is not None:
                ctx.mark_non_differentiable(h_last)
            return y, y_ssm, h_last

    @staticmethod
    def backward(ctx, dy, dyssm, _dh):
        xa, prm, z, A, Dv, state = ctx.saved_tensors
        fused, H, Hp, want_yssm, a_shape, dlog_dtype, has_bias, bias_dtype = ctx.meta
        with torch.cuda.device(xa.device):
            B, L, Di = xa.shape
            dev = xa.device
            W = prm.shape[-1]
            Bm, Cm = _cols(prm, Hp, Hp + Di), _cols(prm, Hp + Di, Hp + 2 * Di)
            dy = dy.contiguous()
            dys = dyssm.contiguous() if (dyssm is not None and want_yssm) else None
            nstate, nws = _rounds_plan(B, L, Di, xa.dtype)
            ws = _rounds_workspace(dev, nws)
            dxa = torch.empty(B, L, Di, dtype=xa.dtype, device=dev)
            dz = torch.empty(B, L, Di, dtype=xa.dtype, device=dev)
            dprm = torch.empty(B, L, W, dtype=xa.dtype, device=dev)
            ddl = dprm if fused else torch.empty(B, L, H, dtype=xa.dtype, device=dev)
            dA = torch.empty(Di, dtype=torch.float32, device=dev)
            dD = torch.empty(Di, dtype=torch.float32, device=dev)
            dbias = torch.empty(H, dtype=torch.float32, device=dev) if has_bias else None
            dB, dC = _cols(dprm, Hp, Hp + Di), _cols(dprm, Hp + Di, Hp + 2 * Di)
            call("ab_ssm_scan_bwd", ptr(xa), _row_stride(xa), ptr(Bm), ptr(Cm), _row_stride(prm), ptr(z), _row_stride(z), ptr(dy),
                 ptr(dys), ptr(A), ptr(Dv), ptr(state), ptr(dxa), Di, ptr(dB), ptr(dC), W, ptr(dz), Di, ptr(ddl),
                 W if fused else H, Hp if fused else H, ptr(dbias), ptr(dA), ptr(dD), ptr(ws), ws.numel(), B, L, Di, H, dt(xa),
                 stream_ptr(dev))
            ddlog = None if fused else ddl.to(dlog_dtype)
            return (dxa, ddlog, dbias.to(bias_dtype) if has_bias else None, dprm, dz, dA.reshape(a_shape), dD,
                    None, None, None, None)


def selective_scan_fused(xa, prm, dt_bias, z, A_log, D, H, h0=None, want_yssm=False, want_hlast=False):
    return _SelectiveScanRounds.apply(xa, None, dt_bias, prm, z, A_log, D, h0, want_yssm, want_hlast, H)



def _as_bf16(t):
    if t.dtype == torch.bfloat16:
        return t.contiguous()
    if t.dtype == torch.float32 and t.is_contiguous() and t.numel() % 4 == 0:
        return _cast_bf16(t)
    return t.to(torch.bfloat16).contiguous()


def dense_nt(x2, w, precise, bias=None, out_dtype=None):
    S, K = x2.shape
    N = w.shape[0]
    dev = x2.device
    if precise:
        a, b, kk, od = _split_cols(x2.float().contiguous(), 0), _split_cols(w.float().contiguous(), 1), 3 * K, torch.float32
    else:
        a, b, kk, od = _as_bf16(x2), _as_bf16(w), K, (out_dtype or torch.bfloat16)
    c = torch.empty(S, N, dtype=od, device=dev)
    call("ab_dense_gemm_nt", ptr(a), ptr(b), ptr(bias), None, ptr(c), S, N, kk, _lib.EPI_BIAS if bias is not None else _lib.EPI_NONE,
         dt(od), stream_ptr(dev))
    return c


def dense_nn(dy2, w, precise, add=None, out_dtype=None):
    S, N = dy2.shape
    K = w.shape[1]
    dev = dy2.device
    if precise:
        a, b, nn_, od = _split_cols(dy2.float().contiguous(), 0), _split_rows(w.float().contiguous(), 1, None, 1, N), 3 * N, torch.float32
    else:
        a, b, nn_, od = _as_bf16(dy2), _as_bf16(w), N, (out_dtype or torch.bfloat16)
    if add is not None:
        add = add.to(od).contiguous()
    c = torch.empty(S, K, dtype=od, device=dev)
    call("ab_dense_gemm_nn", ptr(a), ptr(b), None, ptr(add), ptr(c), S, K, nn_, _lib.EPI_ADD if add is not None else _lib.EPI_NONE,
         dt(od), stream_ptr(dev))
    return c


def dense_tn(dy2, x2, precise):
    S, N = dy2.shape
    K = x2.shape[1]
    dev = dy2.device
    if precise:
        a, b, ss = _split_rows(dy2.float().contiguous(), 0, None, 1, S), _split_rows(x2.float().contiguous(), 1, None, 1, S), 3 * S
    else:
        a, b, ss = _as_bf16(dy2), _as_bf16(x2), S
    c = torch.empty(N, K, dtype=torch.float32, device=dev)
    nws = query("ab_dense_gemm_tn_workspace_bytes", ss, N, K)
    ws = torch.empty(nws, dtype=torch.uint8, device=dev) if nws else None
    call("ab_dense_gemm_tn", ptr(a), ptr(b), ptr(c), ptr(ws), nws, ss, N, K, stream_ptr(dev))
    return c


class _Linear(torch.autograd.Function):

    @staticmethod
    def forward(ctx, x, bias, precise, *weights):
        _lib.ensure_device(x.device)
        with torch.cuda.device(x.device):
            K = x.shape[-1]
            x2 = x.reshape(-1, K)
            w = weights[0] if len(weights) == 1 else torch.cat([wi.reshape(-1, K) for wi in weights], 0)
            wb = w.float().contiguous() if precise else _as_bf16(w)
            xb = x2.float().contiguous() if precise else _as_bf16(x2)
            y = dense_nt(xb, wb, precise, bias=bias.float().contiguous() if bias is not None else None)
            ctx.save_for_backward(xb, wb)
            ctx.meta = (precise, x.shape, x.dtype, [wi.shape[0] for wi in weights], [wi.dtype for wi in weights],
                        bias.dtype if bias is not None else None)
            return y.view(*x.shape[:-1], w.shape[0])

    @staticmethod
    def backward(ctx, dy):
        xb, wb = ctx.saved_tensors
        precise, xshape, xdtype, splits, wdtypes, bdtype = ctx.meta
        with torch.cuda.device(dy.device):
            N = wb.shape[0]
            dy2 = dy.reshape(-1, N)
            dyb = dy2.float().contiguous() if precise else _as_bf16(dy2)
            dx = dense_nn(dyb, wb, precise).view(xshape) if ctx.needs_input_grad[0] else None
            dw = dense_tn(dyb, xb, precise)
            db = dy2.float().sum(0).to(bdtype) if bdtype is not None else None
            dws = [g.to(d) for g, d in zip(dw.split(splits, 0), wdtypes)]
            if dx is not None and dx.dtype != xdtype:
                dx = dx.to(xdtype)
            return (dx, db, None, *dws)


def linear(x, weights, bias=None, precise=False):
    if torch.is_tensor(weights):
        weights = [weights]
    return _Linear.apply(x, bias, precise, *weights)


class _SSMCore(torch.autograd.Function):

    @staticmethod
    def forward(ctx, xz, conv_w, conv_b, Wp, Wdt, dt_bias, A_log, D, precise):
        _lib.ensure_device(xz.device)
        with torch.cuda.device(xz.device):
            dev = xz.device
            B, L, Di2 = xz.shape
            Di = Di2 // 2
            H, R = Wdt.shape
            Hp = (H + 7) // 8 * 8
            Kc = conv_w.shape[-1]
            W = Hp + 2 * Di
            cdt = torch.float32 if precise else torch.bfloat16
            xz = xz.to(cdt).contiguous()
            cw, cb = conv_w.reshape(Di, Kc).float().contiguous(), conv_b.float().contiguous()
            xp, z = xz[..., :Di], xz[..., Di:]
            xa = torch.empty(B, L, Di, dtype=cdt, device=dev)
            call("ab_causal_conv1d_silu_fwd", ptr(xp), Di2, ptr(cw), ptr(cb), ptr(xa), B, L, Di, Kc, dt(cdt), stream_ptr(dev))
            Wp32, Wdt32 = Wp.float().contiguous(), Wdt.float().contiguous()
            wcat = torch.empty(W, Di, dtype=cdt, device=dev)
            call("ab_dt_compose_fwd", ptr(Wp32), ptr(Wdt32), ptr(wcat), H, Hp, R, Di, dt(cdt), stream_ptr(dev))
            prm = dense_nt(xa.view(B * L, Di), wcat, precise).view(B, L, W)
            A = A_log.reshape(-1).float().contiguous()
            Dv = D.float().contiguous()
            bias = dt_bias.float().contiguous()
            nstate, nws = _rounds_plan(B, L, Di, cdt)
            ws = _rounds_workspace(dev, nws)
            y = torch.empty(B, L, Di, dtype=cdt, device=dev)
            state = torch.empty(nstate, dtype=torch.float32, device=dev)
            call("ab_ssm_scan_fwd", ptr(xa), Di, ptr(prm), W, ptr(bias), ptr(prm[..., Hp:]), ptr(prm[..., Hp + Di:]), W, ptr(z), Di2,
                 ptr(A), ptr(Dv), None, ptr(y), None, None, ptr(state), ptr(ws), ws.numel(), B, L, Di, H, dt(cdt), stream_ptr(dev))
            ctx.save_for_backward(xz, cw, cb, xa, wcat, prm, A, Dv, state, Wp32, Wdt32)
            ctx.meta = (precise, H, Hp, R, Kc, conv_w.shape, conv_w.dtype, conv_b.dtype, Wp.dtype, Wdt.dtype, dt_bias.dtype, A_log.shape)
            return y

    @staticmethod
    def backward(ctx, dy):
        xz, cw, cb, xa, wcat, prm, A, Dv, state, Wp32, Wdt32 = ctx.saved_tensors
        precise, H, Hp, R, Kc, cw_shape, cw_dtype, cb_dtype, wp_dtype, wdt_dtype, bias_dtype, a_shape = ctx.meta
        with torch.cuda.device(dy.device):
            dev = dy.device
            B, L, Di2 = xz.shape
            Di = Di2 // 2
            W = Hp + 2 * Di
            cdt = xz.dtype
            S = B * L
            dy = dy.to(cdt).contiguous()
            z = xz[..., Di:]
            nstate, nws = _rounds_plan(B, L, Di, cdt)
            ws = _rounds_workspace(dev, nws)
            dxz = torch.empty(B, L, Di2, dtype=cdt, device=dev)
            dxa_s = torch.empty(B, L, Di, dtype=cdt, device=dev)
            dprm = torch.empty(B, L, W, dtype=cdt, device=dev)
            dA = torch.empty(Di, dtype=torch.float32, device=dev)
            dD = torch.empty(Di, dtype=torch.float32, device=dev)
            dbias = torch.empty(H, dtype=torch.float32, device=dev)
            call("ab_ssm_scan_bwd", ptr(xa), Di, ptr(prm[..., Hp:]), ptr(prm[..., Hp + Di:]), W, ptr(z), Di2, ptr(dy), None, ptr(A),
                 ptr(Dv), ptr(state), ptr(dxa_s), Di, ptr(dprm[..., Hp:]), ptr(dprm[..., Hp + Di:]), W, ptr(dxz[..., Di:]), Di2,
                 ptr(dprm), W, Hp, ptr(dbias), ptr(dA), ptr(dD), ptr(ws), ws.numel(), B, L, Di, H, dt(cdt), stream_ptr(dev))
            dprm2, xa2 = dprm.view(S, W), xa.view(S, Di)
            dxa = dense_nn(dprm2, wcat, precise, add=dxa_s.view(S, Di), out_dtype=cdt)
            dwcat = dense_tn(dprm2, xa2, precise)
            dWp = torch.empty(R + 2 * Di, Di, dtype=torch.float32, device=dev)
            dWdt = torch.empty(H, R, dtype=torch.float32, device=dev)
            call("ab_dt_compose_bwd", ptr(dwcat), ptr(Wp32), ptr(Wdt32), ptr(dWp), ptr(dWdt), H, Hp, R, Di, stream_ptr(dev))
            dcw = torch.empty(Di, Kc, dtype=torch.float32, device=dev)
            dcb = torch.empty(Di, dtype=torch.float32, device=dev)
            ncw = query("ab_causal_conv1d_silu_bwd_workspace_bytes", B, L, Di)
            cws = torch.empty(ncw, dtype=torch.uint8, device=dev)
            call("ab_causal_conv1d_silu_bwd", ptr(xz), Di2, ptr(dxa), ptr(cw), ptr(cb), ptr(dxz), Di2, ptr(dcw), ptr(dcb), ptr(cws), ncw,
                 B, L, Di, Kc, dt(cdt), stream_ptr(dev))
            return (dxz, dcw.reshape(cw_shape).to(cw_dtype), dcb.to(cb_dtype), dWp.to(wp_dtype), dWdt.to(wdt_dtype),
                    dbias.to(bias_dtype), dA.reshape(a_shape), dD, None)


class _DtCompose(torch.autograd.Function):

    @staticmethod
    def forward(ctx, Wp, Wdt, precise):
        _lib.ensure_device(Wp.device)
        with torch.cuda.device(Wp.device):
            H, R = Wdt.shape
            Di = Wp.shape[1]
            Hp = (H + 7) // 8 * 8
            cdt = torch.float32 if precise else torch.bfloat16
            Wp32, Wdt32 = Wp.float().contiguous(), Wdt.float().contiguous()
            wcat = torch.empty(Hp + 2 * Di, Di, dtype=cdt, device=Wp.device)
            call("ab_dt_compose_fwd", ptr(Wp32), ptr(Wdt32), ptr(wcat), H, Hp, R, Di, dt(cdt), stream_ptr(Wp.device))
            ctx.save_for_backward(Wp32, Wdt32)
            ctx.meta = (H, Hp, R, Di, Wp.dtype, Wdt.dtype)
            return wcat

    @staticmethod
    def backward(ctx, dwcat):
        Wp32, Wdt32 = ctx.saved_tensors
        H, Hp, R, Di, wp_dtype, wdt_dtype = ctx.meta
        with torch.cuda.device(dwcat.device):
            dw = dwcat.float().contiguous()
            dWp = torch.empty(R + 2 * Di, Di, dtype=torch.float32, device=dw.device)
            dWdt = torch.empty(H, R, dtype=torch.float32, device=dw.device)
            call("ab_dt_compose_bwd", ptr(dw), ptr(Wp32), ptr(Wdt32), ptr(dWp), ptr(dWdt), H, Hp, R, Di, stream_ptr(dw.device))
            return dWp.to(wp_dtype), dWdt.to(wdt_dtype), None


def dt_compose(Wp, Wdt, precise=False):
    return _DtCompose.apply(Wp, Wdt, precise)


def ssm_core(xz, conv_w, conv_b, Wp, Wdt, dt_bias, A_log, D, precise):
    return _SSMCore.apply(xz, conv_w, conv_b, Wp, Wdt, dt_bias, A_log, D, precise)


class _LMHeadCE(torch.autograd.Function):

    @staticmethod
    @_on_tensor_device
    def forward(ctx, hidden, weight, labels, ignore_index, precise):
        _lib.ensure_device(hidden.device)
        dev = hidden.device
        B, L, Dm = hidden.shape
        V = weight.shape[0]
        h2 = hidden.reshape(B * L, Dm)
        hb = h2.float().contiguous() if precise else _as_bf16(h2)
        wb = weight.float().contiguous() if precise else _as_bf16(weight)
        logits = dense_nt(hb, wb, precise)
        labels = labels.to(torch.int64).contiguous()
        n = B * (L - 1)
        f32 = dict(dtype=torch.float32, device=dev)
        lse, row_loss, row_valid, sums = torch.empty(n, **f32), torch.empty(n, **f32), torch.empty(n, **f32), torch.empty(2, **f32)
        call("ab_shifted_ce_fwd", ptr(logits), ptr(labels), ptr(lse), ptr(row_loss), ptr(row_valid), ptr(sums), B, L, V, int(ignore_index),
             dt(logits), stream_ptr(dev))
        loss = sums[0] / sums[1]
        ctx.save_for_backward(hb, wb, logits, labels, lse, sums)
        ctx.meta = (B, L, V, Dm, int(ignore_index), precise, hidden.dtype, weight.dtype)
        return logits.view(B, L, V), loss

    @staticmethod
    @_on_tensor_device
    def backward(ctx, dlogits_ext, dloss):
        hb, wb, logits, labels, lse, sums = ctx.saved_tensors
        B, L, V, Dm, ignore_index, precise, hdtype, wdtype = ctx.meta
        dev = logits.device
        g = dloss.float() if dloss is not None else torch.zeros((), dtype=torch.float32, device=dev)
        scale = (g / sums[1]).reshape(1).contiguous()
        dl = torch.empty_like(logits)
        call("ab_shifted_ce_bwd", ptr(logits), ptr(labels), ptr(lse), ptr(scale), ptr(dl), B, L, V, ignore_index, dt(logits), stream_ptr(dev))
        if dlogits_ext is not None:
            dl += dlogits_ext.reshape(B * L, V).to(dl.dtype)
        dlb = dl if precise else _as_bf16(dl)
        dh = dense_nn(dlb, wb, precise).view(B, L, Dm).to(hdtype)
        dw = dense_tn(dlb, hb, precise).to(wdtype)
        return dh, dw, None, None, None


def lm_head_cross_entropy(hidden, weight, labels, ignore_index: int = -100, precise: bool = False):
    return _LMHeadCE.apply(hidden, weight, labels, ignore_index, precise)


def _u8(n, dev):
    return torch.empty(max(int(n), 16), dtype=torch.uint8, device=dev)


_side_streams = {}


def _side_stream(device) -> torch.cuda.Stream:
    st = _side_streams.get(device.index)
    if st is None:
        st = torch.cuda.Stream(device=device)
        _side_streams[device.index] = st
    return st


def moe_route(x2, ln_w, ln_b, eps, Wr, br, noise, noise_scale, K, quant=_lib.ROUTER_EXACT):
    S, Dm = x2.shape
    E = Wr.shape[0]
    dev = x2.device
    f32 = dict(dtype=torch.float32, device=dev)
    r = dict(lclean=torch.empty(S, E, **f32), logits=torch.empty(S, E, **f32), gates=torch.empty(S, E, **f32),
             idx=torch.empty(S, K, dtype=torch.int32, device=dev), probs=torch.empty(S, K, **f32),
             w=torch.empty(S, K, **f32), lse=torch.empty(S, **f32), stats=torch.empty(S, 2, **f32),
             aux=torch.empty(2 * E + 1, **f32))
    nws = query("ab_moe_router_workspace_bytes", S, Dm, E)
    ws = _u8(nws, dev)
    call("ab_moe_router_fwd", ptr(x2), ptr(ln_w), ptr(ln_b), float(eps), ptr(Wr), ptr(br), ptr(noise), ptr(noise_scale),
         ptr(r["lclean"]), ptr(r["logits"]), ptr(r["gates"]), ptr(r["idx"]), ptr(r["probs"]), ptr(r["w"]), ptr(r["lse"]),
         ptr(r["stats"]), ptr(r["aux"]), ptr(ws), ws.numel(), S, Dm, E, K, dt(x2), quant, stream_ptr())
    return r


def moe_topk_from_logits(logits, K):
    S, E = logits.shape
    dev = logits.device
    f32 = dict(dtype=torch.float32, device=dev)
    gates, probs, w, lse = torch.empty(S, E, **f32), torch.empty(S, K, **f32), torch.empty(S, K, **f32), torch.empty(S, **f32)
    idx = torch.empty(S, K, dtype=torch.int32, device=dev)
    call("ab_moe_topk_from_logits", ptr(logits.contiguous()), ptr(gates), ptr(idx), ptr(probs), ptr(w), ptr(lse), S, E, K, stream_ptr())
    return gates, idx, probs, w, lse


def moe_plan(idx, w, E, cap, active=None, fixed_seg=0):
    S, K = idx.shape
    dev = idx.device
    cap = int(min(cap, S))
    max_rows = E * fixed_seg if fixed_seg > 0 else int(query("ab_moe_max_rows", S, K, E, cap, ROW_ALIGN))
    i32 = dict(dtype=torch.int32, device=dev)
    p = dict(counts=torch.empty(E, **i32), seg_off=torch.empty(E + 1, **i32), row_of=torch.empty(S, K, **i32),
             tok_of_row=torch.empty(max_rows, **i32), slot_of_row=torch.empty(max_rows, **i32),
             tile_expert=torch.empty(max_rows // ROW_ALIGN, **i32), n_rows=torch.empty(2, **i32), max_rows=max_rows, cap=cap)
    nws = query("ab_moe_plan_workspace_bytes", S, K, E)
    ws = _u8(nws, dev)
    call("ab_moe_plan", ptr(idx), ptr(w), ptr(active), cap, ptr(p["counts"]), ptr(p["seg_off"]), ptr(p["row_of"]),
         ptr(p["tok_of_row"]), ptr(p["slot_of_row"]), ptr(p["tile_expert"]), ptr(p["n_rows"]), ptr(ws), ws.numel(),
         S, K, E, ROW_ALIGN, max_rows, fixed_seg, stream_ptr())
    return p


def _cast_bf16(t):
    out = torch.empty(t.shape, dtype=torch.bfloat16, device=t.device)
    call("ab_cast_f32_to_bf16", ptr(t), ptr(out), t.numel(), stream_ptr())
    return out


def _split_cols(t2d, which):
    rows, cols = t2d.shape
    out = torch.empty(rows, 3 * cols, dtype=torch.bfloat16, device=t2d.device)
    call("ab_split_f32_to_bf16x3", ptr(t2d), ptr(out), rows, cols, which, stream_ptr())
    return out


def _split_rows(t2d, which, seg_off=None, G=1, rows_per_group=0):
    rows, cols = t2d.shape
    out = torch.empty(3 * rows, cols, dtype=torch.bfloat16, device=t2d.device)
    call("ab_split_f32_to_bf16x3_rows", ptr(t2d), ptr(out), ptr(seg_off), G, rows_per_group, cols, which, stream_ptr())
    return out


def grouped_gemm(mode, A, W, plan, N, K, E, *, bias=None, aux=None, epi=_lib.EPI_NONE, act=0, out_dtype=torch.bfloat16,
                 want_c2=False, drop_p=0.0, drop_seed=None, out=None):
    max_rows = A.shape[0]
    if out is not None:
        assert out.shape == (max_rows, N) and out.dtype == out_dtype and out.is_contiguous()
    c = out if out is not None else torch.empty(max_rows, N, dtype=out_dtype, device=A.device)
    c2 = torch.empty(max_rows, N, dtype=out_dtype, device=A.device) if want_c2 else None
    call("ab_grouped_gemm_" + mode, ptr(A), ptr(W), ptr(bias), ptr(aux), ptr(c), ptr(c2), ptr(plan["tile_expert"]),
         ptr(plan["n_rows"]), max_rows, N, K, E, epi, act, dt(out_dtype), float(drop_p), ptr(drop_seed), stream_ptr())
    return (c, c2) if want_c2 else c


def grouped_gemm_tn(A, Bm, seg_off, M, N, E, nsrc=1, src_stride=0):
    out = torch.empty(E, M, N, dtype=torch.float32, device=A.device)
    nws = query("ab_grouped_gemm_tn_workspace_bytes", M, N, E, nsrc)
    ws = torch.empty(nws, dtype=torch.uint8, device=A.device) if nws else None
    call("ab_grouped_gemm_tn", ptr(A), ptr(Bm), ptr(out), ptr(seg_off), A.shape[0], M, N, E, nsrc, src_stride, ptr(ws), nws, stream_ptr())
    return out


def _colsum_side(side, main, a, plan, out, ws, C, E, max_rows, dev):
    side.wait_stream(main)
    with torch.cuda.stream(side):
        call("ab_moe_segment_colsum", ptr(a), ptr(plan["tile_expert"]), ptr(plan["n_rows"]), ptr(out), ptr(ws), ws.numel(), C, E,
             ROW_ALIGN, max_rows, dt(a), stream_ptr(dev))


class _MoEExperts(torch.autograd.Function):

    @staticmethod
    @_on_tensor_device
    def forward(ctx, x2, rn_w, rn_b, Wr, br, noise, noise_scale, ln_w, ln_b, W1, b1, W2, b2, res, cfg):
        _lib.ensure_device(x2.device)
        dev = x2.device
        S, Dm = x2.shape
        E, I, _ = W1.shape
        K, act, training, precise = cfg["K"], cfg["act"], cfg["training"], cfg["precise"]
        x2 = x2.contiguous()
        f = lambda t: t.float().contiguous()
        rn_w, rn_b, Wr, br, ln_w, ln_b, b1, b2 = map(f, (rn_w, rn_b, Wr, br, ln_w, ln_b, b1, b2))
        W1, W2 = f(W1), f(W2)
        use_noise = noise is not None and noise_scale is not None
        main, side = torch.cuda.current_stream(dev), _side_stream(dev)
        w1 = w2 = None
        if not precise:
            w1, w2 = torch.empty(W1.shape, dtype=torch.bfloat16, device=dev), torch.empty(W2.shape, dtype=torch.bfloat16, device=dev)
            side.wait_stream(main)
            with torch.cuda.stream(side):
                call("ab_cast_f32_to_bf16", ptr(W1), ptr(w1), W1.numel(), stream_ptr(dev))
                call("ab_cast_f32_to_bf16", ptr(W2), ptr(w2), W2.numel(), stream_ptr(dev))
        r = moe_route(x2, rn_w, rn_b, cfg["eps"], Wr, br, f(noise) if use_noise else None,
                      f(noise_scale) if use_noise else None, K, cfg.get("quant", _lib.ROUTER_EXACT))
        plan = moe_plan(r["idx"], r["w"], E, cfg["cap"], cfg["active"])
        max_rows = plan["max_rows"]
        cdt = torch.float32 if precise else torch.bfloat16
        xn = torch.empty(max_rows, Dm, dtype=cdt, device=dev)
        call("ab_moe_permute_ln", ptr(x2), ptr(r["stats"]), ptr(ln_w), ptr(ln_b), ptr(plan["tok_of_row"]), ptr(plan["tile_expert"]),
             ptr(plan["n_rows"]), ptr(xn), Dm, ROW_ALIGN, max_rows, dt(x2), dt(cdt), stream_ptr())
        if precise:
            a1 = _split_cols(xn, 0)
            w1 = _split_cols(W1.view(E * I, Dm), 1)
            k1 = 3 * Dm
        else:
            a1, k1 = xn, Dm
            main.wait_stream(side)
        drop_p = float(cfg.get("drop_p", 0.0)) if training else 0.0
        drop_seed = None
        if drop_p > 0.0:
            drop_seed = torch.randint(0, 2 ** 31 - 1, (2,), device=dev, dtype=torch.int32)
        h, hpre = grouped_gemm("nt", a1, w1, plan, I, k1, E, bias=b1, epi=_lib.EPI_BIAS_ACT, act=act, out_dtype=cdt, want_c2=True,
                               drop_p=drop_p, drop_seed=drop_seed)
        if precise:
            a2 = _split_cols(h, 0)
            w2 = _split_cols(W2.view(E * Dm, I), 1)
            k2 = 3 * I
        else:
            a2, k2 = h, I
        y = grouped_gemm("nt", a2, w2, plan, Dm, k2, E, bias=b2, epi=_lib.EPI_BIAS, out_dtype=cdt)
        out_p = float(cfg.get("out_drop_p", 0.0)) if training else 0.0
        out_seed = torch.randint(0, 2 ** 31 - 1, (2,), device=dev, dtype=torch.int32) if out_p > 0.0 else None
        resc = res.reshape(S, Dm).float().contiguous() if res is not None else None
        out = torch.empty(S, Dm, dtype=x2.dtype if res is None else torch.float32, device=dev)
        call("ab_moe_unpermute", ptr(y), ptr(plan["row_of"]), ptr(r["w"]), ptr(resc), ptr(out), out_p, ptr(out_seed), S, K, Dm, dt(y), dt(out),
             stream_ptr())
        aux = r["aux"]
        zero = torch.zeros((), dtype=x2.dtype, device=dev)
        lb = (cfg["lb_coef"] * E / (S * S)) * (aux[:E] * aux[E:2 * E]).sum() if (training and cfg["lb_coef"] > 0) else zero
        rz = (cfg["rz_coef"] / S) * aux[2 * E] if (training and cfg["rz_coef"] > 0) else zero
        ctx.cfg = dict(cfg, S=S, Dm=Dm, E=E, I=I, use_noise=use_noise, max_rows=max_rows, cdt=cdt, drop_p=drop_p, out_p=out_p,
                       has_res=res is not None, res_shape=res.shape if res is not None else None,
                       res_dtype=res.dtype if res is not None else None)
        ctx.drop_seed = drop_seed
        ctx.out_seed = out_seed
        ctx.shadows = None if precise else (w1, w2)
        ctx.plan = {k: v for k, v in plan.items() if torch.is_tensor(v)}
        ctx.save_for_backward(x2, rn_w, rn_b, Wr, br, ln_w, W1, W2, noise if use_noise else None,
                              r["stats"], r["gates"], r["idx"], r["probs"], r["lse"], r["lclean"], r["w"], aux,
                              xn, h, hpre, y)
        ctx.routing = r
        counts = plan["counts"]
        ctx.mark_non_differentiable(counts)
        cfg["_routing"] = (r["idx"], plan["row_of"])
        return out, lb.to(x2.dtype) if torch.is_tensor(lb) else lb, rz.to(x2.dtype) if torch.is_tensor(rz) else rz, counts

    @staticmethod
    @_on_tensor_device
    def backward(ctx, dout, dlb, drz, _dcounts):
        (x2, rn_w, rn_b, Wr, br, ln_w, W1, W2, noise, stats, gates, idx, probs, lse, lclean, w, aux, xn, h, hpre, y) = ctx.saved_tensors
        cfg, plan = ctx.cfg, ctx.plan
        S, Dm, E, I, K = cfg["S"], cfg["Dm"], cfg["E"], cfg["I"], cfg["K"]
        act, precise, max_rows, cdt = cfg["act"], cfg["precise"], cfg["max_rows"], cfg["cdt"]
        dev = x2.device
        f32 = dict(dtype=torch.float32, device=dev)
        dout = dout.contiguous()
        dy = torch.empty(max_rows, Dm, dtype=cdt, device=dev)
        dw_row = torch.empty(max_rows, **f32)
        call("ab_moe_unpermute_bwd", ptr(dout), ptr(y), ptr(w), ptr(plan["tok_of_row"]), ptr(plan["slot_of_row"]), ptr(plan["n_rows"]),
             ptr(dy), ptr(dw_row), cfg["out_p"], ptr(ctx.out_seed), K, Dm, max_rows, dt(dout), dt(y), dt(cdt), stream_ptr())
        seg = plan["seg_off"]
        main, side = torch.cuda.current_stream(dev), _side_stream(dev)
        db2 = torch.empty(E, Dm, **f32)
        db1 = torch.empty(E, I, **f32)
        ws_b2 = _u8(query("ab_moe_segment_colsum_workspace_bytes", Dm, ROW_ALIGN, max_rows), dev)
        ws_b1 = _u8(query("ab_moe_segment_colsum_workspace_bytes", I, ROW_ALIGN, max_rows), dev)
        if precise:
            seg3 = (seg * 3).contiguous()
            w2r = _split_rows(W2.view(E * Dm, I), 1, None, E, Dm)
            dhpre = grouped_gemm("nn", _split_cols(dy, 0), w2r, plan, I, 3 * Dm, E, aux=hpre, epi=_lib.EPI_DACT, act=act, out_dtype=cdt,
                                 drop_p=cfg["drop_p"], drop_seed=ctx.drop_seed)
            dW2 = grouped_gemm_tn(_split_rows(dy, 0, seg, E), _split_rows(h, 1, seg, E), seg3, Dm, I, E)
            dW1 = grouped_gemm_tn(_split_rows(dhpre, 0, seg, E), _split_rows(xn, 1, seg, E), seg3, I, Dm, E)
            w1r = _split_rows(W1.view(E * I, Dm), 1, None, E, I)
            dxn = grouped_gemm("nn", _split_cols(dhpre, 0), w1r, plan, Dm, 3 * I, E, out_dtype=torch.float32)
        else:
            w1b, w2b = ctx.shadows
            dhpre = grouped_gemm("nn", dy, w2b, plan, I, Dm, E, aux=hpre, epi=_lib.EPI_DACT, act=act, out_dtype=cdt,
                                 drop_p=cfg["drop_p"], drop_seed=ctx.drop_seed)
            dW2 = grouped_gemm_tn(dy, h, seg, Dm, I, E)
            dW1 = grouped_gemm_tn(dhpre, xn, seg, I, Dm, E)
            dxn = grouped_gemm("nn", dhpre, w1b, plan, Dm, I, E, out_dtype=torch.bfloat16)
        _colsum_side(side, main, dy, plan, db2, ws_b2, Dm, E, max_rows, dev)
        _colsum_side(side, main, dhpre, plan, db1, ws_b1, I, E, max_rows, dev)
        ws = _u8(query("ab_moe_permute_ln_bwd_workspace_bytes", Dm, ROW_ALIGN, max_rows), dev)
        dxrow = torch.empty(max_rows, Dm, **f32)
        dln_w = torch.empty(E, Dm, **f32)
        dln_b = torch.empty(E, Dm, **f32)
        call("ab_moe_permute_ln_bwd", ptr(dxn), ptr(x2), ptr(stats), ptr(ln_w), ptr(plan["tok_of_row"]), ptr(plan["tile_expert"]),
             ptr(plan["n_rows"]), ptr(dxrow), ptr(dln_w), ptr(dln_b), ptr(ws), ws.numel(), Dm, E, ROW_ALIGN, max_rows, dt(x2),
             dt(dxn), stream_ptr())
        training = cfg["training"]
        g_lb = (dlb.float() * (cfg["lb_coef"] * E / S)) if (training and cfg["lb_coef"] > 0) else torch.zeros((), **f32)
        g_rz = (drz.float() * (cfg["rz_coef"] / S)) if (training and cfg["rz_coef"] > 0) else torch.zeros((), **f32)
        scal = torch.stack([g_lb.reshape(()), g_rz.reshape(())]).contiguous()
        fvec = (aux[E:2 * E] / S).contiguous()
        dx = torch.empty_like(x2)
        dWr, dbr = torch.empty(E, Dm, **f32), torch.empty(E, **f32)
        drn_w, drn_b = torch.empty(Dm, **f32), torch.empty(Dm, **f32)
        dns = torch.empty(E, **f32) if cfg["use_noise"] else None
        nws = query("ab_moe_router_bwd_workspace_bytes", S, Dm, E)
        ws2 = _u8(nws, dev)
        call("ab_moe_router_bwd", ptr(x2), ptr(stats), ptr(rn_w), ptr(rn_b), ptr(Wr), ptr(br), ptr(gates), ptr(idx), ptr(probs),
             ptr(lse), ptr(lclean), ptr(noise.float().contiguous()) if cfg["use_noise"] else None, ptr(fvec), ptr(scal), ptr(dw_row),
             ptr(dxrow), ptr(plan["row_of"]), ptr(dx), ptr(dWr), ptr(dbr), ptr(drn_w), ptr(drn_b), ptr(dns), ptr(ws2), ws2.numel(),
             S, Dm, E, K, dt(x2), stream_ptr())
        dres = dout.reshape(cfg["res_shape"]).to(cfg["res_dtype"]) if cfg["has_res"] else None
        main.wait_stream(side)
        return (dx, drn_w, drn_b, dWr, dbr, None, dns, dln_w, dln_b, dW1, db1, dW2, db2, dres, None)


def moe_experts(x2, rn_w, rn_b, Wr, br, noise, noise_scale, ln_w, ln_b, W1, b1, W2, b2, cfg, res=None):
    return _MoEExperts.apply(x2, rn_w, rn_b, Wr, br, noise, noise_scale, ln_w, ln_b, W1, b1, W2, b2, res, cfg)


def moe_capacity(S: int, E: int, factor: float, training: bool, use_limit: bool) -> int:
    if use_limit and training and E > 0:
        return max(1, math.floor((S / E) * factor)) if S > 0 else 0
    return S
```

### include/apertis_b200.h

```cpp
#ifndef APERTIS_B200_H
#define APERTIS_B200_H

#include <stddef.h>
#include <stdint.h>

#ifdef __cplusplus
extern "C" {
#endif

#ifndef __CUDA_RUNTIME_H__
typedef struct CUstream_st* cudaStream_t;
#endif

#define AB_OK 0
#define AB_ERR_INVALID 1
#define AB_ERR_CUDA 2
#define AB_ERR_UNSUPPORTED 3

#define AB_F32 0
#define AB_BF16 1

#define AB_ACT_GELU 0
#define AB_ACT_RELU 1
#define AB_ACT_SILU 2

int ab_version(void);
int ab_device_check(int device);
int ab_last_error(char* buf, size_t n);

int ab_causal_conv1d_silu_fwd(const void* xp, int64_t xp_stride, const float* w, const float* bias, void* xa,
                              int B, int L, int Di, int Kc, int dtype, cudaStream_t stream);
size_t ab_causal_conv1d_silu_bwd_workspace_bytes(int B, int L, int Di);
int ab_causal_conv1d_silu_bwd(const void* xp, int64_t xp_stride, const void* dxa, const float* w, const float* bias,
                              void* dxp, int64_t dxp_stride, float* dw, float* dbias, void* ws, size_t ws_bytes,
                              int B, int L, int Di, int Kc, int dtype, cudaStream_t stream);

#define AB_SCAN_SINGLE_PASS 0
#define AB_SCAN_TWO_PASS 1
#define AB_SCAN_PIPELINED 2
int ab_selective_scan_plan(int B, int L, int Di, int dtype, int* mode, int* tile_rows, int* slab, int* n_chunks,
                           size_t* ws_bytes);
int ab_selective_scan_fwd(const void* xa, const void* dlog, const void* Bm, const void* Cm, int64_t bc_stride,
                          const void* z, int64_t z_stride, const float* A_log, const float* D, const float* h0,
                          void* y, void* y_ssm, float* h_last, float* hstart, void* ws, size_t ws_bytes,
                          uint32_t epoch, int mode, int B, int L, int Di, int H, int dtype, cudaStream_t stream);
int ab_selective_scan_bwd(const void* xa, const void* dlog, const void* Bm, const void* Cm, int64_t bc_stride,
                          const void* z, int64_t z_stride, const void* dout, const void* dyssm,
                          const float* A_log, const float* D, const float* hstart,
                          void* dxa, void* dBm, void* dCm, int64_t dbc_stride, void* dz, float* ddlog_parts,
                          float* dA_log, float* dD, void* ws, size_t ws_bytes, uint32_t epoch, int mode,
                          int B, int L, int Di, int H, int dtype, cudaStream_t stream);

int ab_dt_compose_fwd(const float* Wp, const float* Wdt, void* Wcat, int H, int Hp, int R, int Di, int out_dtype,
                      cudaStream_t stream);
int ab_dt_compose_bwd(const float* dWcat, const float* Wp, const float* Wdt, float* dWp, float* dWdt, int H, int Hp,
                      int R, int Di, cudaStream_t stream);

int ab_ssm_scan_plan(int B, int L, int Di, int dtype, int64_t* state_floats, size_t* ws_bytes);
int ab_ssm_scan_tune(int tc_fwd, int tc_bwd, int warps_per_sm, int stages_fwd, int stages_bwd);
int ab_ssm_scan_fwd(const void* xa, int64_t xa_stride, const void* dlog, int64_t dlog_stride, const float* dt_bias,
                    const void* Bm, const void* Cm, int64_t bc_stride, const void* z, int64_t z_stride,
                    const float* A_log, const float* D, const float* h0, void* y, void* y_ssm, float* h_last,
                    float* state, void* ws, size_t ws_bytes, int B, int L, int Di, int H, int dtype,
                    cudaStream_t stream);
int ab_ssm_scan_bwd(const void* xa, int64_t xa_stride, const void* Bm, const void* Cm, int64_t bc_stride,
                    const void* z, int64_t z_stride, const void* dout, const void* dyssm, const float* A_log,
                    const float* D, const float* state, void* dxa, int64_t dxa_stride, void* dBm, void* dCm,
                    int64_t dbc_stride, void* dz, int64_t dz_stride, void* ddlog, int64_t ddlog_stride, int ddlog_cols,
                    float* ddt_bias, float* dA_log, float* dD, void* ws, size_t ws_bytes, int B, int L, int Di, int H,
                    int dtype, cudaStream_t stream);

size_t ab_moe_router_workspace_bytes(int S, int Dm, int E);
#define AB_ROUTER_EXACT 0
#define AB_ROUTER_BF16 1
#define AB_ROUTER_FP16 2
int ab_moe_router_fwd(const void* x, const float* ln_w, const float* ln_b, float eps, const float* Wr, const float* br,
                      const float* noise, const float* noise_scale, float* lclean, float* logits, float* gates,
                      int32_t* idx, float* probs, float* w, float* lse, float* stats_out, float* aux, void* ws,
                      size_t ws_bytes, int S, int Dm, int E, int K, int dtype, int quant,
                      cudaStream_t stream);
int ab_moe_topk_from_logits(const float* logits, float* gates, int32_t* idx, float* probs, float* w, float* lse,
                            int S, int E, int K, cudaStream_t stream);

int64_t ab_moe_max_rows(int S, int K, int E, int cap, int row_align);
size_t ab_moe_plan_workspace_bytes(int S, int K, int E);
int ab_moe_plan(const int32_t* idx, const float* w, const int32_t* active, int cap, int32_t* counts, int32_t* seg_off,
                int32_t* row_of, int32_t* tok_of_row, int32_t* slot_of_row, int32_t* tile_expert, int32_t* n_rows,
                void* ws, size_t ws_bytes, int S, int K, int E, int row_align, int64_t max_rows, int fixed_seg,
                cudaStream_t stream);

int ab_moe_permute_ln(const void* x, const float* stats, const float* ln_w, const float* ln_b,
                      const int32_t* tok_of_row, const int32_t* tile_expert, const int32_t* n_rows, void* xn,
                      int Dm, int row_align, int64_t max_rows, int dtype, int out_dtype, cudaStream_t stream);
int ab_moe_unpermute(const void* y, const int32_t* row_of, const float* w, const float* res, void* out, float drop_p,
                     const uint32_t* drop_seed, int S, int K, int Dm, int y_dtype, int out_dtype, cudaStream_t stream);
int ab_moe_unpermute_bwd(const void* dout, const void* y, const float* w, const int32_t* tok_of_row,
                         const int32_t* slot_of_row, const int32_t* n_rows, void* dy, float* dw_row, float drop_p,
                         const uint32_t* drop_seed, int K, int Dm,
                         int64_t max_rows, int dout_dtype, int y_dtype, int dy_dtype, cudaStream_t stream);
size_t ab_moe_permute_ln_bwd_workspace_bytes(int Dm, int row_align, int64_t max_rows);
int ab_moe_permute_ln_bwd(const void* dxn, const void* x, const float* stats, const float* ln_w,
                          const int32_t* tok_of_row, const int32_t* tile_expert, const int32_t* n_rows,
                          float* dxrow, float* dln_w, float* dln_b, void* ws, size_t ws_bytes, int Dm, int E,
                          int row_align, int64_t max_rows, int dtype, int dxn_dtype, cudaStream_t stream);
size_t ab_moe_segment_colsum_workspace_bytes(int C, int row_align, int64_t max_rows);
int ab_moe_segment_colsum(const void* a, const int32_t* tile_expert, const int32_t* n_rows, float* out, void* ws,
                          size_t ws_bytes, int C, int E, int row_align, int64_t max_rows, int dtype, cudaStream_t stream);

size_t ab_moe_router_bwd_workspace_bytes(int S, int Dm, int E);
int ab_moe_router_bwd(const void* x, const float* stats, const float* ln_w, const float* ln_b, const float* Wr,
                      const float* br, const float* gates, const int32_t* idx, const float* probs, const float* lse,
                      const float* lclean, const float* noise, const float* f, const float* scal, const float* dw_row,
                      const float* dxrow, const int32_t* row_of, void* dx, float* dWr, float* dbr, float* dln_w,
                      float* dln_b, float* dnoise_scale, void* ws, size_t ws_bytes, int S, int Dm, int E, int K,
                      int dtype, cudaStream_t stream);

int ab_ep_permute_ln(const void* x, const float* stats, const float* ln_w, const float* ln_b, const int32_t* tok_of_row,
                     const int32_t* tile_expert, const int32_t* n_rows, const uint64_t* peer_xn, int W, int rank,
                     int64_t rows_per_peer, int Dm, int row_align, int64_t max_rows, int dtype, int out_dtype, cudaStream_t stream);
int ab_ep_unpermute_bwd(const void* dout, const void* y, const float* w, const int32_t* tok_of_row, const int32_t* slot_of_row,
                        const int32_t* n_rows, const uint64_t* peer_dy, int W, int rank, int64_t rows_per_peer, float* dw_row,
                        float drop_p, const uint32_t* drop_seed, int K, int Dm, int64_t max_rows, int dout_dtype, int y_dtype,
                        int dy_dtype, cudaStream_t stream);
int ab_ep_grouped_gemm_nt(const void* A, const void* W, const float* bias, const void* aux, const uint64_t* peer_c, int peer_w,
                          int rank, int64_t rows_per_peer, const int32_t* tile_expert, const int32_t* n_rows, int64_t max_rows,
                          int N, int K, int E, int epi, int act, int c_dtype, cudaStream_t stream);
int ab_ep_grouped_gemm_nn(const void* A, const void* W, const float* bias, const void* aux, const uint64_t* peer_c, int peer_w,
                          int rank, int64_t rows_per_peer, const int32_t* tile_expert, const int32_t* n_rows, int64_t max_rows,
                          int N, int K, int E, int epi, int act, int c_dtype, cudaStream_t stream);

#define AB_GEMM_ROW_TILE 256
int ab_gemm_row_tile(void);
#define AB_EPI_NONE 0
#define AB_EPI_BIAS 1
#define AB_EPI_BIAS_ACT 2
#define AB_EPI_DACT 3
#define AB_EPI_ADD 4
int ab_grouped_gemm_nt(const void* A, const void* W, const float* bias, const void* aux, void* c, void* c2,
                       const int32_t* tile_expert, const int32_t* n_rows, int64_t max_rows, int N, int K, int E,
                       int epi, int act, int c_dtype, float drop_p, const uint32_t* drop_seed, cudaStream_t stream);
int ab_grouped_gemm_nn(const void* A, const void* W, const float* bias, const void* aux, void* c, void* c2,
                       const int32_t* tile_expert, const int32_t* n_rows, int64_t max_rows, int N, int K, int E,
                       int epi, int act, int c_dtype, float drop_p, const uint32_t* drop_seed, cudaStream_t stream);
size_t ab_grouped_gemm_tn_workspace_bytes(int M, int N, int E, int nsrc);
int ab_grouped_gemm_tn(const void* A, const void* Bm, float* Cw, const int32_t* seg_off, int64_t max_rows, int M,
                       int N, int E, int nsrc, int64_t src_stride, void* ws, size_t ws_bytes, cudaStream_t stream);

int ab_dense_gemm_nt(const void* A, const void* W, const float* bias, const void* aux, void* C, int64_t S, int N, int K,
                     int epi, int c_dtype, cudaStream_t stream);
int ab_dense_gemm_nn(const void* A, const void* W, const float* bias, const void* aux, void* C, int64_t S, int N, int K,
                     int epi, int c_dtype, cudaStream_t stream);
size_t ab_dense_gemm_tn_workspace_bytes(int64_t S, int M, int N);
int ab_dense_gemm_tn(const void* A, const void* Bm, float* Cw, void* ws, size_t ws_bytes, int64_t S, int M, int N,
                     cudaStream_t stream);

int ab_shifted_ce_fwd(const void* logits, const int64_t* labels, float* lse, float* row_loss, float* row_valid, float* sums,
                      int B, int L, int V, int64_t ignore_index, int dtype, cudaStream_t stream);
int ab_shifted_ce_bwd(const void* logits, const int64_t* labels, const float* lse, const float* scale, void* dlogits, int B,
                      int L, int V, int64_t ignore_index, int dtype, cudaStream_t stream);

int ab_layernorm_fwd(const void* x, const float* w, const float* b, float eps, void* y, float* stats, int S, int Dm,
                     int x_dtype, int y_dtype, cudaStream_t stream);
size_t ab_layernorm_bwd_workspace_bytes(int S, int Dm);
int ab_layernorm_bwd(const void* dy, const void* x, const float* stats, const float* w, const void* dres, void* dx,
                     float* dw, float* db, void* ws, size_t ws_bytes, int S, int Dm, int x_dtype, int dy_dtype,
                     cudaStream_t stream);

int ab_dropout_add(const void* sub, const void* res, void* out, float p, const uint32_t* seed, int64_t n, int sub_dtype,
                   int out_dtype, cudaStream_t stream);

int ab_cast_f32_to_bf16(const float* src, void* dst, int64_t n, cudaStream_t stream);
int ab_split_f32_to_bf16x3(const float* src, void* dst, int64_t rows, int64_t cols, int which, cudaStream_t stream);
int ab_split_f32_to_bf16x3_rows(const float* src, void* dst, const int32_t* seg_off, int G, int64_t rows_per_group,
                                int64_t cols, int which, cudaStream_t stream);

#ifdef __cplusplus
}
#endif
#endif
```

Before: 14.82 million.

## Store activation gradient in expert FC1 epilogue and multiply in backward

The FC1 grouped GEMM epilogue now computes both the activation value and its derivative (with dropout mask and scale folded in). It stores the derivative as fp16 instead of the pre-activation. The backward dact GEMM then only multiplies by the stored gradient, with no GELU recomputation or dropout regeneration. The change also switches aux loading to a cross-tile double-buffered prefetch, widens the control warps to four, and adds a register split, which may shift occupancy and register pressure. Storing the gradient in fp16 changes numerics slightly compared with recomputing it from the saved pre-activation.

```diff
diff --git a/apertis_llm_b200/_lib.py b/apertis_llm_b200/_lib.py
--- a/apertis_llm_b200/_lib.py
+++ b/apertis_llm_b200/_lib.py
@@ -15,6 +15,7 @@
 AB_F32, AB_BF16 = 0, 1
 ACT = {"gelu": 0, "relu": 1, "silu": 2, "swish": 2}
 EPI_NONE, EPI_BIAS, EPI_BIAS_ACT, EPI_DACT, EPI_ADD = 0, 1, 2, 3, 4
+EPI_BIAS_ACT_G, EPI_MUL = 5, 6
 SCAN_SINGLE_PASS, SCAN_TWO_PASS, SCAN_PIPELINED, SCAN_ROUNDS = 0, 1, 2, 3
 ROW_ALIGN = 256
 ROUTER_EXACT, ROUTER_BF16, ROUTER_FP16 = 0, 1, 2
diff --git a/apertis_llm_b200/csrc/grouped_gemm.cu b/apertis_llm_b200/csrc/grouped_gemm.cu
--- a/apertis_llm_b200/csrc/grouped_gemm.cu
+++ b/apertis_llm_b200/csrc/grouped_gemm.cu
@@ -9,8 +9,10 @@
 constexpr int BH_BYTES_MAX = 128 * BK * 2;
 constexpr int STAGE_BYTES = A_BYTES + BH_BYTES_MAX;
 constexpr int ATOM_BYTES = 64 * BK * 2;
-constexpr int EPI_WARP0 = 2, EPI_WARPS = 16, EPI_THREADS = EPI_WARPS * 32;
-constexpr int NUM_THREADS = 64 + EPI_THREADS;
+constexpr int EPI_WARP0 = 4, EPI_WARPS = 16, EPI_THREADS = EPI_WARPS * 32;
+constexpr int NUM_THREADS = 128 + EPI_THREADS;
+constexpr int REGS_CTRL = 32, REGS_EPI = 112;
+static_assert(128 * REGS_CTRL + EPI_THREADS * REGS_EPI <= NUM_THREADS * 96, "register split exceeds the launch allocation");
 constexpr int GW = 64;
 constexpr int MODE_NT = 0, MODE_NN = 1, MODE_TN = 2;
 constexpr int WARP_STG_BYTES = 32 * 64;
@@ -135,11 +137,7 @@
     const f2 hx = f2_mul(x, hs);
     return f2_fma(hx, t, hx);
 }
-__device__ __forceinline__ f2 gelu_bwd_fast2(f2 x, f2 hs) {
-    const f2 x2 = gelu_fast_x2(x);
-    f2 p = f2_fma(f2_bcast(AB_GF_C2), x2, f2_bcast(AB_GF_C1));
-    p = f2_fma(p, x2, f2_bcast(AB_GF_C0));
-    const f2 t = f2_tanh(f2_mul(p, x));
+__device__ __forceinline__ f2 gelu_bwd_fast2_from(f2 x, f2 x2, f2 t, f2 hs) {
     f2 up = f2_fma(f2_bcast(5.f * AB_GF_C2), x2, f2_bcast(3.f * AB_GF_C1));
     up = f2_fma(up, x2, f2_bcast(AB_GF_C0));
     const f2 w = f2_mul(x, up);
@@ -147,6 +145,22 @@
     const f2 A = f2_fma(t, hs, hs);
     return f2_fma(A, e, A);
 }
+__device__ __forceinline__ f2 gelu_bwd_fast2(f2 x, f2 hs) {
+    const f2 x2 = gelu_fast_x2(x);
+    f2 p = f2_fma(f2_bcast(AB_GF_C2), x2, f2_bcast(AB_GF_C1));
+    p = f2_fma(p, x2, f2_bcast(AB_GF_C0));
+    const f2 t = f2_tanh(f2_mul(p, x));
+    return gelu_bwd_fast2_from(x, x2, t, hs);
+}
+__device__ __forceinline__ void gelu_fwd_bwd_fast2(f2 x, f2 hs, f2& val, f2& grad) {
+    const f2 x2 = gelu_fast_x2(x);
+    f2 p = f2_fma(f2_bcast(AB_GF_C2), x2, f2_bcast(AB_GF_C1));
+    p = f2_fma(p, x2, f2_bcast(AB_GF_C0));
+    const f2 t = f2_tanh(f2_mul(p, x));
+    const f2 hx = f2_mul(x, hs);
+    val = f2_fma(hx, t, hx);
+    grad = gelu_bwd_fast2_from(x, x2, t, hs);
+}
 
 template <int U, bool F32>
 __device__ __forceinline__ void act_fwd_row(float (&f)[U], int act, float scale) {
@@ -165,6 +179,39 @@
 #pragma unroll
         for (int i = 0; i < U; ++i) f[i] = act_fwd(f[i], AB_ACT_SILU) * scale;
     }
+}
+template <int U, bool F32>
+__device__ __forceinline__ void act_fwd_grad_row(float (&f)[U], float (&g)[U], int act, float scale) {
+    if (act == AB_ACT_GELU && !F32) {
+        const f2 hs = f2_bcast(0.5f * scale);
+#pragma unroll
+        for (int i = 0; i < U; i += 2) {
+            f2 v, d;
+            gelu_fwd_bwd_fast2(f2_pack(f[i], f[i + 1]), hs, v, d);
+            f2_unpack(v, f[i], f[i + 1]);
+            f2_unpack(d, g[i], g[i + 1]);
+        }
+    } else if (act == AB_ACT_GELU) {
+        const f2 sc = f2_bcast(scale);
+#pragma unroll
+        for (int i = 0; i < U; i += 2) {
+            const f2 x = f2_pack(f[i], f[i + 1]);
+            f2_unpack(f2_mul(gelu_bwd2(x), sc), g[i], g[i + 1]);
+            f2_unpack(f2_mul(gelu_fwd2(x), sc), f[i], f[i + 1]);
+        }
+    } else {
+#pragma unroll
+        for (int i = 0; i < U; ++i) g[i] = act_bwd(f[i], act) * scale;
+        act_fwd_row<U, F32>(f, act, scale);
+    }
+}
+__device__ __forceinline__ uint32_t pack_f16x2(float lo, float hi) {
+    uint32_t r;
+    asm("cvt.rn.f16x2.f32 %0, %1, %2;" : "=r"(r) : "f"(hi), "f"(lo));
+    return r;
+}
+__device__ __forceinline__ void unpack_f16x2(uint32_t v, float& lo, float& hi) {
+    asm("{\n\t.reg .f16 l, h;\n\tmov.b32 {l, h}, %2;\n\tcvt.f32.f16 %0, l;\n\tcvt.f32.f16 %1, h;\n\t}" : "=f"(lo), "=f"(hi) : "r"(v));
 }
 template <int U>
 __device__ __forceinline__ void round_row_bf16(float (&f)[U]) {
@@ -198,6 +245,22 @@
         drop_keep4(xb, (uint32_t)(i >> 2), s1, thi, keep);
 #pragma unroll
         for (int j = 0; j < 4; ++j) f[i + j] = keep[j] ? f[i + j] : 0.f;
+    }
+}
+template <int U>
+__device__ __forceinline__ void dropout_zero_row2(float (&f)[U], float (&g)[U], uint32_t drop_thresh, uint32_t s0, uint32_t s1, uint32_t grow,
+                                                  int ncol, int n_cols) {
+    const uint32_t xb = ((grow * (uint32_t)n_cols + (uint32_t)ncol) >> 2) * 0x9E3779B1u + s0;
+    const uint32_t thi = drop_thresh << 16;
+#pragma unroll
+    for (int i = 0; i < U; i += 4) {
+        bool keep[4];
+        drop_keep4(xb, (uint32_t)(i >> 2), s1, thi, keep);
+#pragma unroll
+        for (int j = 0; j < 4; ++j) {
+            f[i + j] = keep[j] ? f[i + j] : 0.f;
+            g[i + j] = keep[j] ? g[i + j] : 0.f;
+        }
     }
 }
 
@@ -257,19 +320,13 @@
 
 __device__ __forceinline__ uint32_t stg_off(int r, int j) { return (uint32_t)(r * 64 + ((j ^ ((r >> 1) & 3)) << 4)); }
 
-template <int MODE, bool F32>
-__device__ __forceinline__ void stage_and_store(const GemmParams& p, unsigned char* stg, const float (&src)[F32 ? 16 : 32],
-                                                unsigned char* base, int lane, size_t row0, int ncol, int ncol_end) {
-    constexpr int ES = F32 ? 4 : 2;
+template <int MODE, int ES>
+__device__ __forceinline__ void stage_and_store_vecs(const GemmParams& p, unsigned char* stg, const uint4 (&q)[4], unsigned char* base,
+                                                     int lane, size_t row0, int ncol, int ncol_end) {
     constexpr int CPV = 16 / ES;
     const int N = p.N;
 #pragma unroll
-    for (int j = 0; j < 4; ++j) {
-        uint4 q;
-        if (F32) q = make_uint4(__float_as_uint(src[j * 4]), __float_as_uint(src[j * 4 + 1]), __float_as_uint(src[j * 4 + 2]), __float_as_uint(src[j * 4 + 3]));
-        else q = ab_vec16<__nv_bfloat16>::pack(&src[j * 8]);
-        *reinterpret_cast<uint4*>(stg + stg_off(lane, j)) = q;
-    }
+    for (int j = 0; j < 4; ++j) *reinterpret_cast<uint4*>(stg + stg_off(lane, j)) = q[j];
     __syncwarp();
 #pragma unroll
     for (int it = 0; it < 4; ++it) {
@@ -277,10 +334,18 @@
         const int col = ncol + j * CPV;
         const size_t grow = row0 + r;
         const bool ok = col < ncol_end && (MODE == MODE_TN ? (int)grow < p.M : (int64_t)grow < p.rows_valid);
-        const uint4 q = *reinterpret_cast<const uint4*>(stg + stg_off(r, j));
-        if (ok) *reinterpret_cast<uint4*>(base + (grow * N + col) * ES) = q;
+        const uint4 v = *reinterpret_cast<const uint4*>(stg + stg_off(r, j));
+        if (ok) *reinterpret_cast<uint4*>(base + (grow * N + col) * ES) = v;
     }
     __syncwarp();
+}
+template <int MODE, bool F32>
+__device__ __forceinline__ void stage_and_store(const GemmParams& p, unsigned char* stg, const float (&src)[F32 ? 16 : 32],
+                                                unsigned char* base, int lane, size_t row0, int ncol, int ncol_end) {
+    uint4 q[4];
+#pragma unroll
+    for (int j = 0; j < 4; ++j) q[j] = F32 ? ab_vec16<float>::pack(&src[j * 4]) : ab_vec16<__nv_bfloat16>::pack(&src[j * 8]);
+    stage_and_store_vecs<MODE, F32 ? 4 : 2>(p, stg, q, base, lane, row0, ncol, ncol_end);
 }
 
 template <bool F32>
@@ -314,21 +379,41 @@
     constexpr int U = F32 ? 16 : 32;
     constexpr int ES = F32 ? 4 : 2;
     constexpr int CPV = 16 / ES;
-    constexpr bool HAS_BIAS = EPI == AB_EPI_BIAS || EPI == AB_EPI_BIAS_ACT;
+    constexpr bool HAS_BIAS = EPI == AB_EPI_BIAS || EPI == AB_EPI_BIAS_ACT || EPI == AB_EPI_BIAS_ACT_G;
     constexpr bool HAS_AUX = EPI == AB_EPI_DACT || EPI == AB_EPI_ADD;
+    const bool aux_mul = EPI == AB_EPI_ADD && p.epi == AB_EPI_MUL;
     const int lane = c.lane;
     const int quarter = c.warp & 3;
     const int sub = (c.warp - EPI_WARP0) >> 2;
     const int N = p.N, bn = p.bn;
     const int g_col0 = sub * GW;
     const int g_cols = g_col0 < bn ? min(GW, bn - g_col0) : 0;
-    const int total_tiles = total_tiles_of<MODE>(p);
     unsigned char* stg = c.stg;
-    const bool has_drop = (EPI == AB_EPI_BIAS_ACT || EPI == AB_EPI_DACT) && p.drop_seed != nullptr;
+    const bool has_drop = (EPI == AB_EPI_BIAS_ACT || EPI == AB_EPI_BIAS_ACT_G || EPI == AB_EPI_DACT) && p.drop_seed != nullptr;
     const uint32_t drop_s0 = has_drop ? __ldg(p.drop_seed) : 0u, drop_s1 = has_drop ? __ldg(p.drop_seed + 1) : 0u;
     const float dscale = has_drop ? p.drop_scale : 1.0f;
+    uint4 aux_a[4], aux_b[4];
+    int pf_tile = c.pair_id, pf_u = 0, unit = 0;
+    auto prefetch = [&](uint4 (&q)[4]) {
+        while (pf_tile < total_tiles_of<MODE>(p)) {
+            const int n0 = (pf_tile % p.num_n_tiles) * bn;
+            const int cend = min(N, n0 + g_col0 + g_cols);
+            const int col = n0 + g_col0 + pf_u;
+            if (pf_u < g_cols && col < cend) {
+                const size_t row0 = (size_t)(2 * (pf_tile / p.num_n_tiles) + (int)c.rank) * BM + quarter * 32;
+                load_aux_unit<F32>(p, q, lane, row0, col, cend);
+                pf_u += U;
+                return;
+            }
+            pf_tile += c.num_pairs; pf_u = 0;
+        }
+    };
+    if (HAS_AUX) {
+        prefetch(aux_a);
+        prefetch(aux_b);
+    }
     int acc = 0; uint32_t acc_phase = 0;
-    for (int tile = c.pair_id; tile < total_tiles; tile += c.num_pairs) {
+    for (int tile = c.pair_id; tile < total_tiles_of<MODE>(p); tile += c.num_pairs) {
         const Tile t = decode_tile<MODE>(p, tile);
         const int m_tile = 2 * t.m_pair + (int)c.rank;
         const bool have_acc = t.nk > 0;
@@ -342,10 +427,6 @@
             *reinterpret_cast<float2*>(c.bias_s + 2 * lane) = b2;
             __syncwarp();
         }
-        uint4 nxt[4];
-        if (HAS_AUX && g_cols > 0 && n0 + g_col0 < ncol_end) {
-            load_aux_unit<F32>(p, nxt, lane, row0, n0 + g_col0, ncol_end);
-        }
         if (have_acc) {
             ab_mbar_wait(&c.tfull[acc], acc_phase);
             ab_tc_fence_after();
@@ -355,13 +436,15 @@
             const int tcol = g_col0 + u0;
             const int ncol = n0 + tcol;
             if (ncol >= ncol_end) break;
-            uint4 cur[4];
             if (HAS_AUX) {
-#pragma unroll
-                for (int it = 0; it < 4; ++it) cur[it] = nxt[it];
-                if (u0 + U < g_cols && ncol + U < ncol_end) {
-                    load_aux_unit<F32>(p, nxt, lane, row0, ncol + U, ncol_end);
-                }
+                auto to_staging = [&](const uint4 (&q)[4]) {
+#pragma unroll
+                    for (int it = 0; it < 4; ++it) *reinterpret_cast<uint4*>(stg + stg_off(it * 8 + (lane >> 2), lane & 3)) = q[it];
+                };
+                if (unit & 1) { to_staging(aux_b); prefetch(aux_b); }
+                else { to_staging(aux_a); prefetch(aux_a); }
+                ++unit;
+                __syncwarp();
             }
             float f[U];
             {
@@ -389,20 +472,35 @@
                 stage_and_store<MODE, F32>(p, stg, f, reinterpret_cast<unsigned char*>(p.c2), lane, row0, ncol, ncol_end);
                 act_fwd_row<U, F32>(f, p.act, p.drop_seed ? p.drop_scale : 1.0f);
                 if (p.drop_seed) dropout_zero_row<U>(f, p.drop_thresh, drop_s0, drop_s1, (uint32_t)row0 + (uint32_t)lane, ncol, N);
+            } else if (EPI == AB_EPI_BIAS_ACT_G) {
+                if (!F32) round_row_bf16<U>(f);
+                float g[U];
+                act_fwd_grad_row<U, F32>(f, g, p.act, dscale);
+                if (has_drop) dropout_zero_row2<U>(f, g, p.drop_thresh, drop_s0, drop_s1, (uint32_t)row0 + (uint32_t)lane, ncol, N);
+                if constexpr (F32) {
+                    stage_and_store<MODE, F32>(p, stg, g, reinterpret_cast<unsigned char*>(p.c2), lane, row0, ncol, ncol_end);
+                } else {
+                    uint4 q[4];
+#pragma unroll
+                    for (int j = 0; j < 4; ++j)
+                        q[j] = make_uint4(pack_f16x2(g[j * 8], g[j * 8 + 1]), pack_f16x2(g[j * 8 + 2], g[j * 8 + 3]),
+                                          pack_f16x2(g[j * 8 + 4], g[j * 8 + 5]), pack_f16x2(g[j * 8 + 6], g[j * 8 + 7]));
+                    stage_and_store_vecs<MODE, 2>(p, stg, q, reinterpret_cast<unsigned char*>(p.c2), lane, row0, ncol, ncol_end);
+                }
             } else if (HAS_AUX) {
 #pragma unroll
-                for (int it = 0; it < 4; ++it) *reinterpret_cast<uint4*>(stg + stg_off(it * 8 + (lane >> 2), lane & 3)) = cur[it];
-                __syncwarp();
-#pragma unroll
-                for (int j = 0; j < 4; ++j) cur[j] = *reinterpret_cast<const uint4*>(stg + stg_off(lane, j));
-                __syncwarp();
-#pragma unroll
                 for (int j = 0; j < 4; ++j) {
-                    const uint4 q = cur[j];
+                    const uint4 q = *reinterpret_cast<const uint4*>(stg + stg_off(lane, j));
                     float a[CPV];
                     if (F32) { a[0] = __uint_as_float(q.x); a[1] = __uint_as_float(q.y); a[2] = __uint_as_float(q.z); a[3] = __uint_as_float(q.w); }
-                    else ab_vec16<__nv_bfloat16>::unpack(q, a);
-                    if (EPI == AB_EPI_ADD) {
+                    else if (aux_mul) {
+                        unpack_f16x2(q.x, a[0], a[1]); unpack_f16x2(q.y, a[2], a[3]);
+                        unpack_f16x2(q.z, a[4], a[5]); unpack_f16x2(q.w, a[6], a[7]);
+                    } else ab_vec16<__nv_bfloat16>::unpack(q, a);
+                    if (EPI == AB_EPI_ADD && aux_mul) {
+#pragma unroll
+                        for (int i = 0; i < CPV; ++i) f[j * CPV + i] *= a[i];
+                    } else if (EPI == AB_EPI_ADD) {
 #pragma unroll
                         for (int i = 0; i < CPV; ++i) f[j * CPV + i] += a[i];
                     } else if (p.act == AB_ACT_GELU) {
@@ -443,9 +541,38 @@
         case AB_EPI_BIAS: epilogue_role<MODE, F32, AB_EPI_BIAS>(p, c); break;
         case AB_EPI_BIAS_ACT: epilogue_role<MODE, F32, AB_EPI_BIAS_ACT>(p, c); break;
         case AB_EPI_DACT: epilogue_role<MODE, F32, AB_EPI_DACT>(p, c); break;
-        case AB_EPI_ADD: epilogue_role<MODE, F32, AB_EPI_ADD>(p, c); break;
+        case AB_EPI_ADD:
+        case AB_EPI_MUL: epilogue_role<MODE, F32, AB_EPI_ADD>(p, c); break;
+        case AB_EPI_BIAS_ACT_G: epilogue_role<MODE, F32, AB_EPI_BIAS_ACT_G>(p, c); break;
         default: epilogue_role<MODE, F32, AB_EPI_NONE>(p, c); break;
     }
+}
+
+constexpr size_t STG_OFF = (size_t)NSTAGE * STAGE_BYTES;
+constexpr size_t BIAS_OFF = STG_OFF + (size_t)EPI_WARPS * WARP_STG_BYTES;
+constexpr size_t BARS_OFF = BIAS_OFF + (size_t)EPI_WARPS * WARP_BIAS_BYTES;
+struct KernelCtx {
+    unsigned char* smem;
+    uint64_t *full, *empty, *tfull, *tempty;
+    uint32_t* tmem_slot;
+    int warp, lane, pair_id, num_pairs;
+    uint32_t rank;
+};
+__device__ __forceinline__ KernelCtx kernel_ctx(unsigned char* smem_raw) {
+    KernelCtx k;
+    uint32_t raw = ab_smem_u32(smem_raw), tid = threadIdx.x, bid = blockIdx.x, nb = gridDim.x;
+    asm volatile("" : "+r"(raw), "+r"(tid), "+r"(bid), "+r"(nb));
+    k.smem = smem_raw + ((1024u - (raw & 1023u)) & 1023u);
+    uint64_t* bars = reinterpret_cast<uint64_t*>(k.smem + BARS_OFF);
+    k.full = bars;
+    k.empty = bars + NSTAGE;
+    k.tfull = bars + 2 * NSTAGE;
+    k.tempty = bars + 2 * NSTAGE + NACC;
+    k.tmem_slot = reinterpret_cast<uint32_t*>(bars + 2 * NSTAGE + 2 * NACC);
+    k.warp = (int)(tid >> 5); k.lane = (int)(tid & 31);
+    k.rank = ab_cluster_ctarank();
+    k.pair_id = (int)(bid >> 1); k.num_pairs = (int)(nb >> 1);
+    return k;
 }
 
 template <int MODE>
@@ -453,128 +580,126 @@
                                                                       const __grid_constant__ CUtensorMap tm_b,
                                                                       const GemmParams p) {
     extern __shared__ unsigned char smem_raw[];
-    const uint32_t raw = ab_smem_u32(smem_raw);
-    unsigned char* smem = smem_raw + ((1024u - (raw & 1023u)) & 1023u);
-    unsigned char* stg_base = smem + (size_t)NSTAGE * STAGE_BYTES;
-    float* bias_base = reinterpret_cast<float*>(stg_base + (size_t)EPI_WARPS * WARP_STG_BYTES);
-    uint64_t* bars = reinterpret_cast<uint64_t*>(reinterpret_cast<unsigned char*>(bias_base) + (size_t)EPI_WARPS * WARP_BIAS_BYTES);
-    uint64_t* full = bars;
-    uint64_t* empty = bars + NSTAGE;
-    uint64_t* tfull = bars + 2 * NSTAGE;
-    uint64_t* tempty = bars + 2 * NSTAGE + NACC;
-    uint32_t* tmem_slot = reinterpret_cast<uint32_t*>(bars + 2 * NSTAGE + 2 * NACC);
-
-    const int warp = threadIdx.x >> 5, lane = threadIdx.x & 31;
-    const uint32_t rank = ab_cluster_ctarank();
-    const int pair_id = blockIdx.x >> 1, num_pairs = gridDim.x >> 1;
-    if (warp == 0 && lane == 0) {
+    KernelCtx k = kernel_ctx(smem_raw);
+    if (k.warp == 0 && k.lane == 0) {
         ab_prefetch_tmap(&tm_a);
         ab_prefetch_tmap(&tm_b);
-        for (int i = 0; i < NSTAGE; ++i) { ab_mbar_init(&full[i], 1); ab_mbar_init(&empty[i], 1); }
-        for (int i = 0; i < NACC; ++i) { ab_mbar_init(&tfull[i], 1); ab_mbar_init(&tempty[i], 2 * EPI_WARPS); }
+        for (int i = 0; i < NSTAGE; ++i) { ab_mbar_init(&k.full[i], 1); ab_mbar_init(&k.empty[i], 1); }
+        for (int i = 0; i < NACC; ++i) { ab_mbar_init(&k.tfull[i], 1); ab_mbar_init(&k.tempty[i], 2 * EPI_WARPS); }
         ab_fence_mbar_init();
     }
-    if (warp == 1) {
-        ab_tmem_alloc_pair(tmem_slot, 512);
+    if (k.warp == 1) {
+        ab_tmem_alloc_pair(k.tmem_slot, 512);
         ab_tmem_relinquish_pair();
     }
     ab_tc_fence_before();
     ab_cluster_sync();
     ab_tc_fence_after();
-    const uint32_t tmem_base = *tmem_slot;
-
-    const int total_tiles = total_tiles_of<MODE>(p);
-    const int bn = p.bn, bh = bn >> 1;
-    const uint32_t bh_bytes = MODE == MODE_NT ? (uint32_t)bh * BK * 2 : (uint32_t)(bh / 64) * ATOM_BYTES;
-    const uint32_t pair_tx = 2u * (A_BYTES + bh_bytes);
-
-    if (warp == 0) {
-        int stage = 0; uint32_t phase = 0;
-        for (int tile = pair_id; tile < total_tiles; tile += num_pairs) {
-            const Tile t = decode_tile<MODE>(p, tile);
-            const int b_col0 = t.n_tile * bn + (int)rank * bh;
-            const int n_src = MODE == MODE_TN ? p.tn_nsrc : 1;
-            const int per_src = t.nk / n_src;
-            const int m0 = MODE == MODE_TN ? t.m_pair * PM + (int)rank * BM : (2 * t.m_pair + (int)rank) * BM;
-            const int b_row0 = MODE == MODE_NN ? t.e * p.K : (MODE == MODE_NT ? t.e * p.N + b_col0 : 0);
-            for (int src = 0; src < n_src; ++src) {
-                int r0 = MODE == MODE_TN ? (int)(src * p.tn_src_stride) + t.k_begin : 0;
-                for (int kk = 0; kk < per_src; ++kk, r0 += BK) {
-                    ab_mbar_wait(&empty[stage], phase ^ 1);
-                    unsigned char* sa = smem + (size_t)stage * STAGE_BYTES;
-                    unsigned char* sb = sa + A_BYTES;
-                    if (ab_elect_one()) {
-                        if (rank == 0) ab_mbar_expect_tx(&full[stage], pair_tx);
-                        if (MODE == MODE_TN) {
-                            ab_tma_load_2d_pair(sa, &tm_a, &full[stage], m0, r0);
-                            ab_tma_load_2d_pair(sa + ATOM_BYTES, &tm_a, &full[stage], m0 + 64, r0);
-                            ab_tma_load_2d_pair(sb, &tm_b, &full[stage], b_col0, r0);
-                            if (bh > 64) ab_tma_load_2d_pair(sb + ATOM_BYTES, &tm_b, &full[stage], b_col0 + 64, r0);
-                        } else {
-                            ab_tma_load_2d_pair(sa, &tm_a, &full[stage], r0, m0);
-                            if (MODE == MODE_NT) {
-                                ab_tma_load_2d_pair(sb, &tm_b, &full[stage], r0, b_row0);
+
+    if (k.warp < EPI_WARP0) {
+        asm volatile("setmaxnreg.dec.sync.aligned.u32 %0;" :: "n"(REGS_CTRL));
+        const KernelCtx c = kernel_ctx(smem_raw);
+        unsigned char* smem = c.smem;
+        uint64_t *full = c.full, *empty = c.empty, *tfull = c.tfull, *tempty = c.tempty;
+        const int warp = c.warp;
+        const uint32_t rank = c.rank;
+        const int pair_id = c.pair_id, num_pairs = c.num_pairs;
+        const uint32_t tmem_base = *c.tmem_slot;
+        const int total_tiles = total_tiles_of<MODE>(p);
+        const int bn = p.bn, bh = bn >> 1;
+        const uint32_t bh_bytes = MODE == MODE_NT ? (uint32_t)bh * BK * 2 : (uint32_t)(bh / 64) * ATOM_BYTES;
+        const uint32_t pair_tx = 2u * (A_BYTES + bh_bytes);
+        if (warp == 0) {
+            int stage = 0; uint32_t phase = 0;
+            for (int tile = pair_id; tile < total_tiles; tile += num_pairs) {
+                const Tile t = decode_tile<MODE>(p, tile);
+                const int b_col0 = t.n_tile * bn + (int)rank * bh;
+                const int n_src = MODE == MODE_TN ? p.tn_nsrc : 1;
+                const int per_src = t.nk / n_src;
+                const int m0 = MODE == MODE_TN ? t.m_pair * PM + (int)rank * BM : (2 * t.m_pair + (int)rank) * BM;
+                const int b_row0 = MODE == MODE_NN ? t.e * p.K : (MODE == MODE_NT ? t.e * p.N + b_col0 : 0);
+                for (int src = 0; src < n_src; ++src) {
+                    int r0 = MODE == MODE_TN ? (int)(src * p.tn_src_stride) + t.k_begin : 0;
+                    for (int kk = 0; kk < per_src; ++kk, r0 += BK) {
+                        ab_mbar_wait(&empty[stage], phase ^ 1);
+                        unsigned char* sa = smem + (size_t)stage * STAGE_BYTES;
+                        unsigned char* sb = sa + A_BYTES;
+                        if (ab_elect_one()) {
+                            if (rank == 0) ab_mbar_expect_tx(&full[stage], pair_tx);
+                            if (MODE == MODE_TN) {
+                                ab_tma_load_2d_pair(sa, &tm_a, &full[stage], m0, r0);
+                                ab_tma_load_2d_pair(sa + ATOM_BYTES, &tm_a, &full[stage], m0 + 64, r0);
+                                ab_tma_load_2d_pair(sb, &tm_b, &full[stage], b_col0, r0);
+                                if (bh > 64) ab_tma_load_2d_pair(sb + ATOM_BYTES, &tm_b, &full[stage], b_col0 + 64, r0);
                             } else {
-                                ab_tma_load_2d_pair(sb, &tm_b, &full[stage], b_col0, b_row0 + r0);
-                                if (bh > 64) ab_tma_load_2d_pair(sb + ATOM_BYTES, &tm_b, &full[stage], b_col0 + 64, b_row0 + r0);
+                                ab_tma_load_2d_pair(sa, &tm_a, &full[stage], r0, m0);
+                                if (MODE == MODE_NT) {
+                                    ab_tma_load_2d_pair(sb, &tm_b, &full[stage], r0, b_row0);
+                                } else {
+                                    ab_tma_load_2d_pair(sb, &tm_b, &full[stage], b_col0, b_row0 + r0);
+                                    if (bh > 64) ab_tma_load_2d_pair(sb + ATOM_BYTES, &tm_b, &full[stage], b_col0 + 64, b_row0 + r0);
+                                }
                             }
                         }
+                        __syncwarp();
+                        if (++stage == NSTAGE) { stage = 0; phase ^= 1; }
                     }
-                    __syncwarp();
-                    if (++stage == NSTAGE) { stage = 0; phase ^= 1; }
+                }
+            }
+            for (int i = 0; i < NSTAGE; ++i) {
+                ab_mbar_wait(&empty[stage], phase ^ 1);
+                if (++stage == NSTAGE) { stage = 0; phase ^= 1; }
+            }
+        } else if (warp == 1) {
+            if (rank == 0) {
+                const uint32_t idesc = make_idesc(bn, MODE == MODE_TN ? 1 : 0, MODE == MODE_NT ? 0 : 1);
+                const uint32_t smem0 = ab_smem_u32(smem);
+                const uint64_t da0 = MODE == MODE_TN ? make_smem_desc(smem0, ATOM_BYTES, 1024) : make_smem_desc(smem0, 0, 1024);
+                const uint64_t db0 = MODE == MODE_NT ? make_smem_desc(smem0 + A_BYTES, 0, 1024) : make_smem_desc(smem0 + A_BYTES, ATOM_BYTES, 1024);
+                constexpr uint32_t a_step = MODE == MODE_TN ? (16 * 128) >> 4 : 32 >> 4;
+                constexpr uint32_t b_step = MODE == MODE_NT ? 32 >> 4 : (16 * 128) >> 4;
+                int stage = 0; uint32_t phase = 0;
+                int acc = 0; uint32_t acc_phase = 0;
+                for (int tile = pair_id; tile < total_tiles; tile += num_pairs) {
+                    const Tile t = decode_tile<MODE>(p, tile);
+                    if (t.nk == 0) continue;
+                    ab_mbar_wait(&tempty[acc], acc_phase ^ 1);
+                    ab_tc_fence_after();
+                    const uint32_t d_tmem = tmem_base + (uint32_t)acc * 256u;
+                    for (int kb = 0; kb < t.nk; ++kb) {
+                        ab_mbar_wait(&full[stage], phase);
+                        ab_tc_fence_after();
+                        const uint64_t soff = (uint64_t)((uint32_t)stage * (STAGE_BYTES >> 4));
+                        const uint64_t da = da0 + soff, db = db0 + soff;
+                        if (ab_elect_one()) {
+    #pragma unroll
+                            for (int k = 0; k < BK / 16; ++k)
+                                ab_umma_f16_pair(d_tmem, da + (uint64_t)(k * a_step), db + (uint64_t)(k * b_step), idesc, (kb > 0 || k > 0) ? 1u : 0u);
+                            ab_umma_commit_pair(&empty[stage], 3);
+                            if (kb == t.nk - 1) ab_umma_commit_pair(&tfull[acc], 3);
+                        }
+                        __syncwarp();
+                        if (++stage == NSTAGE) { stage = 0; phase ^= 1; }
+                    }
+                    if (++acc == NACC) { acc = 0; acc_phase ^= 1; }
                 }
             }
         }
-        for (int i = 0; i < NSTAGE; ++i) {
-            ab_mbar_wait(&empty[stage], phase ^ 1);
-            if (++stage == NSTAGE) { stage = 0; phase ^= 1; }
-        }
-    } else if (warp == 1) {
-        if (rank == 0) {
-            const uint32_t idesc = make_idesc(bn, MODE == MODE_TN ? 1 : 0, MODE == MODE_NT ? 0 : 1);
-            const uint32_t smem0 = ab_smem_u32(smem);
-            const uint64_t da0 = MODE == MODE_TN ? make_smem_desc(smem0, ATOM_BYTES, 1024) : make_smem_desc(smem0, 0, 1024);
-            const uint64_t db0 = MODE == MODE_NT ? make_smem_desc(smem0 + A_BYTES, 0, 1024) : make_smem_desc(smem0 + A_BYTES, ATOM_BYTES, 1024);
-            constexpr uint32_t a_step = MODE == MODE_TN ? (16 * 128) >> 4 : 32 >> 4;
-            constexpr uint32_t b_step = MODE == MODE_NT ? 32 >> 4 : (16 * 128) >> 4;
-            int stage = 0; uint32_t phase = 0;
-            int acc = 0; uint32_t acc_phase = 0;
-            for (int tile = pair_id; tile < total_tiles; tile += num_pairs) {
-                const Tile t = decode_tile<MODE>(p, tile);
-                if (t.nk == 0) continue;
-                ab_mbar_wait(&tempty[acc], acc_phase ^ 1);
-                ab_tc_fence_after();
-                const uint32_t d_tmem = tmem_base + (uint32_t)acc * 256u;
-                for (int kb = 0; kb < t.nk; ++kb) {
-                    ab_mbar_wait(&full[stage], phase);
-                    ab_tc_fence_after();
-                    const uint64_t soff = (uint64_t)((uint32_t)stage * (STAGE_BYTES >> 4));
-                    const uint64_t da = da0 + soff, db = db0 + soff;
-                    if (ab_elect_one()) {
-#pragma unroll
-                        for (int k = 0; k < BK / 16; ++k)
-                            ab_umma_f16_pair(d_tmem, da + (uint64_t)(k * a_step), db + (uint64_t)(k * b_step), idesc, (kb > 0 || k > 0) ? 1u : 0u);
-                        ab_umma_commit_pair(&empty[stage], 3);
-                        if (kb == t.nk - 1) ab_umma_commit_pair(&tfull[acc], 3);
-                    }
-                    __syncwarp();
-                    if (++stage == NSTAGE) { stage = 0; phase ^= 1; }
-                }
-                if (++acc == NACC) { acc = 0; acc_phase ^= 1; }
-            }
-        }
     } else {
+        asm volatile("setmaxnreg.inc.sync.aligned.u32 %0;" :: "n"(REGS_EPI));
+        const KernelCtx kc = kernel_ctx(smem_raw);
         EpiCtx c;
-        c.stg = stg_base + (size_t)(warp - EPI_WARP0) * WARP_STG_BYTES;
-        c.bias_s = bias_base + (size_t)(warp - EPI_WARP0) * GW;
-        c.tfull = tfull; c.tempty = tempty; c.tmem_base = tmem_base;
-        c.warp = warp; c.lane = lane; c.rank = rank; c.pair_id = pair_id; c.num_pairs = num_pairs;
+        c.stg = kc.smem + STG_OFF + (size_t)(kc.warp - EPI_WARP0) * WARP_STG_BYTES;
+        c.bias_s = reinterpret_cast<float*>(kc.smem + BIAS_OFF) + (size_t)(kc.warp - EPI_WARP0) * GW;
+        c.tfull = kc.tfull; c.tempty = kc.tempty; c.tmem_base = *kc.tmem_slot;
+        c.warp = kc.warp; c.lane = kc.lane; c.rank = kc.rank; c.pair_id = kc.pair_id; c.num_pairs = kc.num_pairs;
         if (p.c_f32) epilogue_dispatch<MODE, true>(p, c);
         else epilogue_dispatch<MODE, false>(p, c);
     }
     ab_tc_fence_before();
     ab_cluster_sync();
-    if (warp == 1) ab_tmem_dealloc_pair(tmem_base, 512);
+    k = kernel_ctx(smem_raw);
+    if (k.warp == 1) ab_tmem_dealloc_pair(*k.tmem_slot, 512);
 }
 
 int pick_bn(int N, bool mn_major_b) {
@@ -648,15 +773,16 @@
               int c_dtype, float drop_p, const uint32_t* drop_seed, cudaStream_t stream, const uint64_t* peer_c = nullptr,
               int peer_w = 0, int peer_rank = 0, int64_t peer_rows = 0) {
     AB_REQUIRE(drop_p >= 0.f && drop_p < 1.f, "grouped_gemm: dropout probability must be in [0, 1)");
-    AB_REQUIRE(drop_p == 0.f || (drop_seed != nullptr && (epi == AB_EPI_BIAS_ACT || epi == AB_EPI_DACT)),
+    AB_REQUIRE(drop_p == 0.f || (drop_seed != nullptr && (epi == AB_EPI_BIAS_ACT || epi == AB_EPI_BIAS_ACT_G || epi == AB_EPI_DACT)),
                "grouped_gemm: dropout needs a seed and the bias+act / dact epilogue");
     AB_REQUIRE(max_rows > 0 && max_rows % PM == 0, "grouped_gemm: max_rows must be a positive multiple of %d", PM);
     AB_REQUIRE(N > 0 && K > 0 && E > 0 && N % 8 == 0 && K % 8 == 0, "grouped_gemm: N (%d) and K (%d) must be multiples of 8", N, K);
     AB_REQUIRE(c_dtype == AB_F32 || c_dtype == AB_BF16, "grouped_gemm: bad output dtype");
-    AB_REQUIRE(epi >= AB_EPI_NONE && epi <= AB_EPI_ADD, "grouped_gemm: bad epilogue %d", epi);
-    AB_REQUIRE((epi != AB_EPI_BIAS && epi != AB_EPI_BIAS_ACT) || bias, "grouped_gemm: bias epilogue without bias");
-    AB_REQUIRE(epi != AB_EPI_BIAS_ACT || c2, "grouped_gemm: bias+act epilogue needs the pre-activation output c2");
-    AB_REQUIRE((epi != AB_EPI_DACT && epi != AB_EPI_ADD) || aux, "grouped_gemm: dact / add epilogue needs aux");
+    AB_REQUIRE(epi >= AB_EPI_NONE && epi <= AB_EPI_MUL, "grouped_gemm: bad epilogue %d", epi);
+    const bool bias_act = epi == AB_EPI_BIAS_ACT || epi == AB_EPI_BIAS_ACT_G;
+    AB_REQUIRE((epi != AB_EPI_BIAS && !bias_act) || bias, "grouped_gemm: bias epilogue without bias");
+    AB_REQUIRE(!bias_act || c2, "grouped_gemm: bias+act epilogue needs the second output c2");
+    AB_REQUIRE((epi != AB_EPI_DACT && epi != AB_EPI_ADD && epi != AB_EPI_MUL) || aux, "grouped_gemm: dact / add / mul epilogue needs aux");
     AB_REQUIRE(bias == nullptr || ((uintptr_t)bias % 8) == 0, "grouped_gemm: bias must be 8-byte aligned");
     GemmParams p;
     memset(&p, 0, sizeof(p));
@@ -668,7 +794,7 @@
     p.rows_valid = max_rows;
     if (peer_c != nullptr) {
         AB_REQUIRE(peer_w >= 1 && peer_w <= 16 && peer_rank >= 0 && peer_rank < peer_w && peer_rows > 0 && peer_rows % PM == 0 &&
-                   (int64_t)peer_w * peer_rows == max_rows && epi != AB_EPI_BIAS_ACT,
+                   (int64_t)peer_w * peer_rows == max_rows && !bias_act,
                    "ep_grouped_gemm: bad peer table (W=%d rank=%d rows_per_peer=%lld, max_rows=%lld)", peer_w, peer_rank,
                    (long long)peer_rows, (long long)max_rows);
         for (int i = 0; i < peer_w; ++i) {
diff --git a/apertis_llm_b200/ep.py b/apertis_llm_b200/ep.py
--- a/apertis_llm_b200/ep.py
+++ b/apertis_llm_b200/ep.py
@@ -211,8 +211,7 @@
             a1, k1 = xr, Dm
         drop_p = float(cfg.get("drop_p", 0.0)) if training else 0.0
         drop_seed = torch.randint(0, 2 ** 31 - 1, (2,), device=dev, dtype=torch.int32) if drop_p > 0.0 else None
-        h, hpre = ops.grouped_gemm("nt", a1, w1, rplan, I, k1, El, bias=b1, epi=_lib.EPI_BIAS_ACT, act=act, out_dtype=cdt, want_c2=True,
-                                   drop_p=drop_p, drop_seed=drop_seed)
+        h, g = ops.expert_fc1(a1, w1, rplan, I, k1, El, b1, act, cdt, drop_p, drop_seed)
         if precise:
             a2, k2 = ops._split_cols(h, 0), 3 * I
         else:
@@ -249,7 +248,7 @@
         ctx.plan = {k: v for k, v in plan.items() if torch.is_tensor(v)}
         ctx.rplan = rplan
         ctx.save_for_backward(x2, rn_w, rn_b, Wr, br, ln_w_full, W1, W2, noise if use_noise else None, r["stats"], r["gates"],
-                              r["idx"], r["probs"], r["lse"], r["lclean"], r["w"], aux, xr, h, hpre, y)
+                              r["idx"], r["probs"], r["lse"], r["lclean"], r["w"], aux, xr, h, g, y)
         counts = plan["counts"]
         ctx.mark_non_differentiable(counts)
         cfg["_routing"] = (r["idx"], plan["row_of"])
@@ -258,7 +257,7 @@
     @staticmethod
     @ops._on_tensor_device
     def backward(ctx, dout, dlb, drz, _dcounts):
-        (x2, rn_w, rn_b, Wr, br, ln_w_full, W1, W2, noise, stats, gates, idx, probs, lse, lclean, w, aux, xr, h, hpre, y) = ctx.saved_tensors
+        (x2, rn_w, rn_b, Wr, br, ln_w_full, W1, W2, noise, stats, gates, idx, probs, lse, lclean, w, aux, xr, h, g, y) = ctx.saved_tensors
         cfg, plan, rplan, group = ctx.cfg, ctx.plan, ctx.rplan, ctx.group
         S, Dm, E, El, I, K, W, seg = (cfg[k] for k in ("S", "Dm", "E", "El", "I", "K", "W", "seg"))
         act, precise, rows, cdt = cfg["act"], cfg["precise"], cfg["rows"], cfg["cdt"]
@@ -301,8 +300,7 @@
             G = W * El
             lseg3 = (lseg * 3).contiguous()
             w2r = ops._split_rows(W2.view(El * Dm, I), 1, None, El, Dm)
-            dhpre = ops.grouped_gemm("nn", ops._split_cols(dyr, 0), w2r, rplan, I, 3 * Dm, El, aux=hpre, epi=_lib.EPI_DACT, act=act, out_dtype=cdt,
-                                     drop_p=cfg["drop_p"], drop_seed=ctx.drop_seed)
+            dhpre = ops.expert_dact(ops._split_cols(dyr, 0), w2r, rplan, I, 3 * Dm, El, g, cdt)
             sr = lambda t, which: ops._split_rows(t, which, None, G, seg)
             w1r = ops._split_rows(W1.view(El * I, Dm), 1, None, El, I)
             dxnr = ops.grouped_gemm("nn", ops._split_cols(dhpre, 0), w1r, rplan, Dm, 3 * I, El, out_dtype=torch.float32)
@@ -311,8 +309,7 @@
             dW1 = ops.grouped_gemm_tn(sr(dhpre, 0), sr(xr, 1), lseg3, I, Dm, El, nsrc=W, src_stride=3 * stride)
         else:
             w1b, w2b = ctx.shadows
-            dhpre = ops.grouped_gemm("nn", dyr, w2b, rplan, I, Dm, El, aux=hpre, epi=_lib.EPI_DACT, act=act, out_dtype=cdt,
-                                     drop_p=cfg["drop_p"], drop_seed=ctx.drop_seed)
+            dhpre = ops.expert_dact(dyr, w2b, rplan, I, Dm, El, g, cdt)
             if peer is not None:
                 call("ab_ep_grouped_gemm_nn", ptr(dhpre), ptr(w1b), None, None, peer.ptrs["dxn"], W, rank, El * seg, ptr(rplan["tile_expert"]),
                      ptr(rplan["n_rows"]), rows, Dm, I, El, _lib.EPI_NONE, act, dt(torch.bfloat16), stream_ptr())
diff --git a/apertis_llm_b200/ops.py b/apertis_llm_b200/ops.py
--- a/apertis_llm_b200/ops.py
+++ b/apertis_llm_b200/ops.py
@@ -722,10 +722,25 @@
     if out is not None:
         assert out.shape == (max_rows, N) and out.dtype == out_dtype and out.is_contiguous()
     c = out if out is not None else torch.empty(max_rows, N, dtype=out_dtype, device=A.device)
-    c2 = torch.empty(max_rows, N, dtype=out_dtype, device=A.device) if want_c2 else None
+    c2_dtype = act_grad_dtype(out_dtype) if epi == _lib.EPI_BIAS_ACT_G else out_dtype
+    c2 = torch.empty(max_rows, N, dtype=c2_dtype, device=A.device) if want_c2 else None
     call("ab_grouped_gemm_" + mode, ptr(A), ptr(W), ptr(bias), ptr(aux), ptr(c), ptr(c2), ptr(plan["tile_expert"]),
          ptr(plan["n_rows"]), max_rows, N, K, E, epi, act, dt(out_dtype), float(drop_p), ptr(drop_seed), stream_ptr())
     return (c, c2) if want_c2 else c
+
+
+def act_grad_dtype(cdt):
+    return torch.float16 if cdt == torch.bfloat16 else torch.float32
+
+
+def expert_fc1(a1, w1, plan, I, k1, E, b1, act, cdt, drop_p, drop_seed):
+    return grouped_gemm("nt", a1, w1, plan, I, k1, E, bias=b1, epi=_lib.EPI_BIAS_ACT_G, act=act, out_dtype=cdt, want_c2=True,
+                        drop_p=drop_p, drop_seed=drop_seed)
+
+
+def expert_dact(a, w2, plan, I, k, E, g, cdt):
+    assert g.dtype == act_grad_dtype(cdt)
+    return grouped_gemm("nn", a, w2, plan, I, k, E, aux=g, epi=_lib.EPI_MUL, out_dtype=cdt)
 
 
 def grouped_gemm_tn(A, Bm, seg_off, M, N, E, nsrc=1, src_stride=0):
@@ -785,8 +800,7 @@
         drop_seed = None
         if drop_p > 0.0:
             drop_seed = torch.randint(0, 2 ** 31 - 1, (2,), device=dev, dtype=torch.int32)
-        h, hpre = grouped_gemm("nt", a1, w1, plan, I, k1, E, bias=b1, epi=_lib.EPI_BIAS_ACT, act=act, out_dtype=cdt, want_c2=True,
-                               drop_p=drop_p, drop_seed=drop_seed)
+        h, g = expert_fc1(a1, w1, plan, I, k1, E, b1, act, cdt, drop_p, drop_seed)
         if precise:
             a2 = _split_cols(h, 0)
             w2 = _split_cols(W2.view(E * Dm, I), 1)
@@ -813,7 +827,7 @@
         ctx.plan = {k: v for k, v in plan.items() if torch.is_tensor(v)}
         ctx.save_for_backward(x2, rn_w, rn_b, Wr, br, ln_w, W1, W2, noise if use_noise else None,
                               r["stats"], r["gates"], r["idx"], r["probs"], r["lse"], r["lclean"], r["w"], aux,
-                              xn, h, hpre, y)
+                              xn, h, g, y)
         ctx.routing = r
         counts = plan["counts"]
         ctx.mark_non_differentiable(counts)
@@ -823,7 +837,7 @@
     @staticmethod
     @_on_tensor_device
     def backward(ctx, dout, dlb, drz, _dcounts):
-        (x2, rn_w, rn_b, Wr, br, ln_w, W1, W2, noise, stats, gates, idx, probs, lse, lclean, w, aux, xn, h, hpre, y) = ctx.saved_tensors
+        (x2, rn_w, rn_b, Wr, br, ln_w, W1, W2, noise, stats, gates, idx, probs, lse, lclean, w, aux, xn, h, g, y) = ctx.saved_tensors
         cfg, plan = ctx.cfg, ctx.plan
         S, Dm, E, I, K = cfg["S"], cfg["Dm"], cfg["E"], cfg["I"], cfg["K"]
         act, precise, max_rows, cdt = cfg["act"], cfg["precise"], cfg["max_rows"], cfg["cdt"]
@@ -843,16 +857,14 @@
         if precise:
             seg3 = (seg * 3).contiguous()
             w2r = _split_rows(W2.view(E * Dm, I), 1, None, E, Dm)
-            dhpre = grouped_gemm("nn", _split_cols(dy, 0), w2r, plan, I, 3 * Dm, E, aux=hpre, epi=_lib.EPI_DACT, act=act, out_dtype=cdt,
-                                 drop_p=cfg["drop_p"], drop_seed=ctx.drop_seed)
+            dhpre = expert_dact(_split_cols(dy, 0), w2r, plan, I, 3 * Dm, E, g, cdt)
             dW2 = grouped_gemm_tn(_split_rows(dy, 0, seg, E), _split_rows(h, 1, seg, E), seg3, Dm, I, E)
             dW1 = grouped_gemm_tn(_split_rows(dhpre, 0, seg, E), _split_rows(xn, 1, seg, E), seg3, I, Dm, E)
             w1r = _split_rows(W1.view(E * I, Dm), 1, None, E, I)
             dxn = grouped_gemm("nn", _split_cols(dhpre, 0), w1r, plan, Dm, 3 * I, E, out_dtype=torch.float32)
         else:
             w1b, w2b = ctx.shadows
-            dhpre = grouped_gemm("nn", dy, w2b, plan, I, Dm, E, aux=hpre, epi=_lib.EPI_DACT, act=act, out_dtype=cdt,
-                                 drop_p=cfg["drop_p"], drop_seed=ctx.drop_seed)
+            dhpre = expert_dact(dy, w2b, plan, I, Dm, E, g, cdt)
             dW2 = grouped_gemm_tn(dy, h, seg, Dm, I, E)
             dW1 = grouped_gemm_tn(dhpre, xn, seg, I, Dm, E)
             dxn = grouped_gemm("nn", dhpre, w1b, plan, Dm, I, E, out_dtype=torch.bfloat16)
diff --git a/include/apertis_b200.h b/include/apertis_b200.h
--- a/include/apertis_b200.h
+++ b/include/apertis_b200.h
@@ -136,6 +136,8 @@
 #define AB_EPI_BIAS_ACT 2
 #define AB_EPI_DACT 3
 #define AB_EPI_ADD 4
+#define AB_EPI_BIAS_ACT_G 5
+#define AB_EPI_MUL 6
 int ab_grouped_gemm_nt(const void* A, const void* W, const float* bias, const void* aux, void* c, void* c2,
                        const int32_t* tile_expert, const int32_t* n_rows, int64_t max_rows, int N, int K, int E,
                        int epi, int act, int c_dtype, float drop_p, const uint32_t* drop_seed, cudaStream_t stream);
```

New measurement: 14.98 million (median of 6 runs). 1.1% higher.
